# Yujia-Yan/Transkun

Hardware: AMD Instinct MI355X
Metric: semi-CRF logProb+backward steps/sec at T=1024, NBatch=352 (higher is better)
Workload: dtype f32; 1 GPU; NeuralSemiCRFInterval(score, noise).logProb(intervals) fwd+bwd through the public API (Python interval lists packed inside the timed region), T=1024, NBatch=352 per GPU, fp32, exact-hash randn-like scores resident in HBM; T=1024, NBatch=352, impl=0, parallelism=chains sharded, 1 rank(s) seen by the process group, no data-path collective

## Files before the change

### include/semicrf_hip.h

```cpp
#ifndef SEMICRF_HIP_H
#define SEMICRF_HIP_H

#include <stddef.h>
#include <stdint.h>

#ifdef __cplusplus
extern "C" {
#endif

#define SEMICRF_ABI_VERSION 2

#define SEMICRF_OK 0
#define SEMICRF_EINVAL 1
#define SEMICRF_EWORKSPACE 2
#define SEMICRF_ELAUNCH 3
#define SEMICRF_ETIMEOUT 4

#define SEMICRF_OP_LOGZ_FWD 0
#define SEMICRF_OP_LOGZ_BWD 1
#define SEMICRF_OP_VITERBI 2
#define SEMICRF_OP_EVAL_PATH 3
#define SEMICRF_OP_INTERVAL_SCORE 4
#define SEMICRF_OP_SAMPLE 5
#define SEMICRF_OP_VITERBI_NBEST 6
// ... 57 lines not shown
                       float* node, float* begin, float* end, float* single, float* noiseP, float* entropy, void* ws, size_t ws_bytes,
                       semicrf_stream_t stream);

int semicrf_interval_marginals(const float* score, const float* v, const float* q, const float* logZ, int T, int B,
                               const int32_t* pairs, int64_t K, const int32_t* offsets, float* out, semicrf_stream_t stream);

int semicrf_marginal_decode(const float* score, const float* noise, const float* v, const float* q, const float* logZ, int T, int B,
                            const float* tau, int tau_stride, int32_t* pairs, float* probs, int64_t cap, int32_t* offsets,
                            void* ws, size_t ws_bytes, semicrf_stream_t stream);

int semicrf_mbr_select(const int32_t* pairs, const float* weight, const int32_t* offsets, int64_t K, int T, int B, const float* tau,
                       int tau_stride, int32_t* pairs_out, float* probs_out, int64_t cap, int32_t* offsets_out, float* gain,
                       void* ws, size_t ws_bytes, semicrf_stream_t stream);

int semicrf_interval_marginals_tol(const float* score, const float* v, const float* q, const float* logZ, int T, int B,
                                   const int32_t* pairs, int64_t K, const int32_t* offsets, int tol_begin, int tol_end, float* out,
                                   semicrf_stream_t stream);
int semicrf_marginal_decode_tol(const float* score, const float* noise, const float* v, const float* q, const float* logZ, int T, int B,
                                const float* tau, int tau_stride, int tol_begin, int tol_end, int32_t* pairs, float* probs, int64_t cap,
                                int32_t* offsets, void* ws, size_t ws_bytes, semicrf_stream_t stream);

int semicrf_expectation(const float* score, const float* noise, const float* weight, const float* noiseWeight, const float* v,
                        const float* q, int T, int B, float* E, float* H, void* ws, size_t ws_bytes, semicrf_stream_t stream);
int semicrf_covariance(const float* score, const float* noise, const float* weight, const float* noiseWeight, const float* gout, int T,
                       int B, float* C, float* Cn, const void* ws, size_t ws_bytes, semicrf_stream_t stream);

int semicrf_alpha_from(const float* score, const float* noise, const int32_t* start, int T, int B, float* v, float* logZ, void* ws,
                       size_t ws_bytes, semicrf_stream_t stream);

int semicrf_compare_paths(const int32_t* est_pairs, const int32_t* est_offsets, const int32_t* ref_pairs, const int32_t* ref_offsets,
                          int T, int B, int tol_begin, int tol_end, int32_t* stats , semicrf_stream_t stream);

int semicrf_eval_path(const float* score, const float* noise, int T, int B,
                      const int32_t* pairs, int64_t K, const int32_t* offsets, float* out,
                      void* ws, size_t ws_bytes, semicrf_stream_t stream);

int semicrf_eval_path_bwd(const float* gout, int T, int B, const int32_t* pairs, int64_t K,
                          const int32_t* offsets, float* dScore, float* dNoise, semicrf_stream_t stream);

int semicrf_logprob_fwd(const float* score, const float* noise, int T, int B, const int32_t* pairs, int64_t K,
                        const int32_t* offsets, float* logProb, float* logZ, float* v, void* ws, size_t ws_bytes,
                        semicrf_stream_t stream);
int semicrf_logprob_bwd(const float* score, const float* noise, const float* v, const float* logZ, const float* gout,
                        int gout_stride, int T, int B, const int32_t* pairs, int64_t K, const int32_t* offsets,
                        float* dScore, float* dNoise, void* ws, size_t ws_bytes, semicrf_stream_t stream);

#define SEMICRF_GRAD_UPPER_IS_ZERO 1
int semicrf_logz_bwd_f(const float* score, const float* noise, const float* v, const float* logZ,
                       const float* gout, int T, int B, float* dScore, float* dNoise, float* q_out, int flags,
                       void* ws, size_t ws_bytes, semicrf_stream_t stream);
int semicrf_logprob_bwd_f(const float* score, const float* noise, const float* v, const float* logZ, const float* gout,
                          int gout_stride, int T, int B, const int32_t* pairs, int64_t K, const int32_t* offsets,
                          float* dScore, float* dNoise, int flags, void* ws, size_t ws_bytes, semicrf_stream_t stream);

int interval_score_fwd(const float* q, const float* k, const float* diag, int C, int T, int D,
                       int64_t ldq, int64_t ldk, int64_t ldd, float qscale, int length_scaling,
                       int full_square, float* S, float* noise_out, semicrf_stream_t stream);

int interval_score_bwd(const float* dS, const float* q, const float* k, int C, int T, int D, int64_t ldq,
                       int64_t ldk, float qscale, int length_scaling, float* dq, float* dk, float* ddiag,
                       int64_t lddq, int64_t lddk, int64_t lddd, semicrf_stream_t stream);

size_t interval_score_bwd_workspace_bytes(int C, int T, int D);
int interval_score_bwd_ws(const float* dS, const float* q, const float* k, int C, int T, int D, int64_t ldq,
                          int64_t ldk, float qscale, int length_scaling, float* dq, float* dk, float* ddiag,
                          int64_t lddq, int64_t lddk, int64_t lddd, void* ws, size_t ws_bytes, semicrf_stream_t stream);

int interval_score_fwd_p(const float* q, const float* k, const float* diag, int C, int T, int D,
                         int64_t ldq, int64_t ldk, int64_t ldd, float qscale, int length_scaling,
                         int full_square, int group, int pitch, float* S, float* noise_out, semicrf_stream_t stream);
int interval_score_bwd_ws_p(const float* dS, const float* q, const float* k, int C, int T, int D, int64_t ldq,
                            int64_t ldk, float qscale, int length_scaling, int group, int pitch, float* dq, float* dk,
                            float* ddiag, int64_t lddq, int64_t lddk, int64_t lddd, void* ws, size_t ws_bytes,
                            semicrf_stream_t stream);
int interval_score_bwd_fused_ws_p(const float* S, const float* alpha, const float* beta, const float* logZ,
                                  const float* gout, const float* q, const float* k, int C, int T, int D, int64_t ldq,
                                  int64_t ldk, float qscale, int length_scaling, int group, int pitch, float* dq, float* dk,
                                  float* ddiag, int64_t lddq, int64_t lddk, int64_t lddd, void* ws, size_t ws_bytes,
                                  semicrf_stream_t stream);
int interval_score_path_bwd_p(const float* gout, const int32_t* pairs, int64_t K, const int32_t* offsets, const float* q,
                              const float* k, int C, int T, int D, int64_t ldq, int64_t ldk, float qscale, int length_scaling,
                              int group, int pitch, float* dq, float* dk, float* ddiag, int64_t lddq, int64_t lddk,
                              int64_t lddd, semicrf_stream_t stream);

int interval_score_fwd_pc(const float* q, const float* k, const float* diag, const float* rowc, int C, int T, int D,
                          int64_t ldq, int64_t ldk, int64_t ldd, int64_t ldrc, float qscale, int length_scaling,
                          int full_square, int group, int pitch, float* S, float* noise_out, semicrf_stream_t stream);
int interval_score_bwd_ws_pc(const float* dS, const float* q, const float* k, int C, int T, int D, int64_t ldq,
                             int64_t ldk, float qscale, int length_scaling, int group, int pitch, float* dq, float* dk,
                             float* ddiag, float* drowc, int64_t lddq, int64_t lddk, int64_t lddd, int64_t lddrc, void* ws,
                             size_t ws_bytes, semicrf_stream_t stream);
int interval_score_bwd_fused_ws_pc(const float* S, const float* alpha, const float* beta, const float* logZ,
                                   const float* gout, const float* q, const float* k, int C, int T, int D, int64_t ldq,
                                   int64_t ldk, float qscale, int length_scaling, int group, int pitch, float* dq, float* dk,
                                   float* ddiag, float* drowc, int64_t lddq, int64_t lddk, int64_t lddd, int64_t lddrc,
                                   void* ws, size_t ws_bytes, semicrf_stream_t stream);
int interval_score_path_bwd_pc(const float* gout, const int32_t* pairs, int64_t K, const int32_t* offsets, const float* q,
                               const float* k, int C, int T, int D, int64_t ldq, int64_t ldk, float qscale,
                               int length_scaling, int group, int pitch, float* dq, float* dk, float* ddiag, float* drowc,
                               int64_t lddq, int64_t lddk, int64_t lddd, int64_t lddrc, semicrf_stream_t stream);

int scorer_proj_nn(const float* A, int64_t lda, int64_t M, int K, const float* B, int64_t ldb, int N, float* out, int64_t ldout,
                   const float* bias, const float* w2, const float* b2, int zero_cols, int accumulate, semicrf_stream_t stream);
size_t scorer_proj_nn3_workspace_bytes(int K, int N);
int scorer_proj_nn3(const float* A, int64_t lda, int64_t M, int K, const float* B, int64_t ldb, int N, float* out, int64_t ldout,
                    const float* bias, const float* w2, const float* b2, int zero_cols, int accumulate, void* ws, size_t ws_bytes,
// ... 113 lines not shown
```

### transkun_amd/CRF/NeuralSemiCRFInterval.py

```python
from __future__ import annotations

import os
from collections import namedtuple
from typing import List, Optional, Sequence, Tuple

import numpy as np
import torch

from .. import _lib

Intervals = List[List[Tuple[int, int]]]



def _check_inputs(score: torch.Tensor, noiseScore: torch.Tensor):
    assert len(score.shape) == 3
    assert score.shape[0] == score.shape[1]
    assert len(noiseScore.shape) == 2
    T, B = score.shape[0], score.shape[2]
    assert noiseScore.shape[0] == T - 1
    assert noiseScore.shape[1] == B
    _lib.require_device(score, "score")
    _lib.require_device(noiseScore, "noiseScore")
    assert score.device == noiseScore.device
    return T, B


def _prep(t: torch.Tensor) -> torch.Tensor:
    if t.dtype != torch.float32:
        t = t.float()
    return t if t.is_contiguous() else t.contiguous()


_SIDE = {}


def _side_stream(device):
    key = torch.device(device).index if torch.device(device).index is not None else torch.cuda.current_device()
    st = _SIDE.get(key)
    if st is None:
        st = _SIDE[key] = torch.cuda.Stream(device=device)
    return st


def _ready(pairs) -> None:
    ev = getattr(pairs, "_semicrf_ready", None)
    if ev is not None:
        torch.cuda.current_stream(pairs.device).wait_event(ev)
        pairs._semicrf_ready = None


def pack_intervals(intervals: Sequence[Sequence[Tuple[int, int]]], T: int, B: int, device, overlap: bool = False, ordered: bool = True):
    assert len(intervals) == B, f"expected {B} interval lists, got {len(intervals)}"
    mm = _lib.marshal()
    K = int(mm.count(intervals))
    pin = torch.device(device).type == "cuda"
    pairs_h = torch.empty(max(K, 1), 2, dtype=torch.int32, pin_memory=pin)
    offsets_h = torch.empty(B + 1, dtype=torch.int32, pin_memory=pin)
    if K == 0:
        pairs_h.zero_()
    k = mm.pack_into(intervals, pairs_h.data_ptr(), max(K, 1), offsets_h.data_ptr(), T, bool(ordered))
    assert k == K
    if overlap and pin:
        main = torch.cuda.current_stream(device)
        side = _side_stream(device)
        with torch.cuda.stream(side):
            pairs_d = pairs_h.to(device, non_blocking=True)
            offsets_d = offsets_h.to(device, non_blocking=True)
            ev = side.record_event()
        pairs_d.record_stream(main); offsets_d.record_stream(main)
        pairs_d._semicrf_ready = ev
    else:
        pairs_d = pairs_h.to(device, non_blocking=True)
        offsets_d = offsets_h.to(device, non_blocking=True)
    pairs_d._semicrf_K = K
    return pairs_d, offsets_d


def unpack_intervals(pairs_host: torch.Tensor, offsets_host: torch.Tensor, T: int = 1 << 30) -> Intervals:
    import gc
    pairs_host = pairs_host.contiguous()
    offsets_host = offsets_host.contiguous()
    assert pairs_host.dtype == torch.int32 and offsets_host.dtype == torch.int32
    B = offsets_host.numel() - 1
    total = int(offsets_host[-1]) if B >= 0 else 0
    assert pairs_host.numel() >= 2 * total
    if T >= 1 << 30:
        T = int(pairs_host[:total].max()) + 1 if total else 1
    was = gc.isenabled()
    gc.disable()
    try:
        return _lib.marshal().unpack(pairs_host.data_ptr(), offsets_host.data_ptr(), B, T)
    finally:
        if was:
            gc.enable()



_DEBUG_WS = []


def _odd_pad(score) -> bool:
    return score.is_cuda and score.shape[2] == 1 and score.shape[0] >= 2 and _lib.get_impl() == 0


def _pad1(t):
    return torch.nn.functional.pad(t, (0, 1))


def _logz_fwd_raw(score, noise, want_v: bool):
    if _odd_pad(score):
        logz, v = _logz_fwd_raw(_pad1(score), _pad1(noise), want_v)
        return logz[:-1].contiguous(), (v[:, :-1].contiguous() if v is not None else None)
    T, B = score.shape[0], score.shape[2]
    logz = torch.empty(B, dtype=torch.float32, device=score.device)
    v = torch.empty((T, B) if want_v else (0,), dtype=torch.float32, device=score.device)
    ws = _lib.leased_workspace(_lib.OP_LOGZ_FWD, T, B, score.device)
    _lib.ops().logz_fwd(score, noise, logz, v, want_v, ws)
    if os.environ.get("SEMICRF_DEBUG_KEEP_WS"):
        _DEBUG_WS[:] = [ws]
    return logz, (v if want_v else None)


GRAD_UPPER_IS_ZERO = 1


_USE_COUNT = getattr(torch._C, "_storage_Use_Count", None)
_WARNED = set()
# ... 76 lines not shown
            for i in same[:-self.PER_KEY]:
                self.entries[i] = None
            self.entries = [e for e in self.entries if e is not None]
            total = 0
            for i in range(len(self.entries) - 1, -1, -1):
                total += self.entries[i][1].numel() * 4
                if total > max(self.max_bytes, nbytes):
                    del self.entries[:i + 1]
                    break

    def rerecord(self, dscore: torch.Tensor) -> None:
        if dscore is None:
            return
        ptr = dscore.data_ptr()
        with self.lock:
            for e in self.entries:
                if e[1].data_ptr() == ptr:
                    e[2] = e[1]._version

    def clear(self) -> None:
        with self.lock:
            self.entries.clear()


_GRAD_POOL = _GradPool()


def grad_pool_bytes() -> int:
    from .. import scorer as _sc
    return _GRAD_POOL.held_bytes() + (_sc._SCORE_POOL.held_bytes() if _sc._SCORE_POOL is not None else 0)


def grad_pool_clear() -> None:
    _GRAD_POOL.clear()
    from .. import scorer as _sc
    if _sc._SCORE_POOL is not None:
        _sc._SCORE_POOL.clear()


def _logz_bwd_raw(score, noise, v, logz, gout, want_q: bool = False):
    if _odd_pad(score):
        ds, dn, q = _logz_bwd_raw(_pad1(score), _pad1(noise), _pad1(v), _pad1(logz), _pad1(gout), want_q)
        return ds[:, :, :-1].contiguous(), dn[:, :-1].contiguous(), (q[:, :-1].contiguous() if q is not None else None)
    T, B = score.shape[0], score.shape[2]
    dscore, flags, pkey = _GRAD_POOL.take(T, B, score.device)
    dnoise = torch.empty_like(noise)
    q = torch.empty((T, B) if want_q else (0,), dtype=torch.float32, device=score.device)
    ws = _lib.leased_workspace(_lib.OP_LOGZ_BWD, T, B, score.device)
    _lib.ops().logz_bwd(score, noise, v, logz, gout, dscore, dnoise, q, want_q, flags, ws)
    _GRAD_POOL.give(pkey, dscore)
    return dscore, dnoise, (q if want_q else None)


def _logprob_fwd_raw(score, noise, pairs, offsets, want_v: bool):
    K = getattr(pairs, "_semicrf_K", pairs.shape[0])
    if _odd_pad(score):
        logz, v = _logz_fwd_raw(score, noise, want_v)
        return _eval_path_raw(score, noise, pairs, offsets) - logz, logz, v
    T, B = score.shape[0], score.shape[2]
    dev = score.device
    lp = torch.empty(B, dtype=torch.float32, device=dev)
    logz = torch.empty(B, dtype=torch.float32, device=dev)
    v = torch.empty((T, B) if want_v else (0,), dtype=torch.float32, device=dev)
    ws = _lib.leased_workspace(_lib.OP_LOGZ_FWD, T, B, dev)
    _lib.ops().logprob_fwd(score, noise, pairs, int(K), offsets, lp, logz, v, want_v, ws)
    return lp, logz, (v if want_v else None)


def _eval_path_raw(score, noise, pairs, offsets):
    T, B = score.shape[0], score.shape[2]
    out = torch.empty(B, dtype=torch.float32, device=score.device)
    ws = _lib.workspace(_lib.OP_EVAL_PATH, T, B, score.device)
    K = getattr(pairs, "_semicrf_K", pairs.shape[0])
    _lib.ops().eval_path(score, noise, pairs, int(K), offsets, out, ws)
    return out


_EMPTY = {}


def _empty(device):
    e = _EMPTY.get(device)
    if e is None:
        e = _EMPTY[device] = torch.empty(0, dtype=torch.float32, device=device)
    return e


def _eval_path_bwd_raw(gout, T, B, pairs, offsets, dscore, dnoise, K: int, pooled: bool = False):
    e = _empty(gout.device)
    _lib.ops().eval_path_bwd(gout, T, B, pairs, int(K), offsets, dscore if dscore is not None else e, dscore is not None,
                             dnoise if dnoise is not None else e, dnoise is not None)
    if pooled:
        _GRAD_POOL.rerecord(dscore)


def _gout(grad_output: torch.Tensor, B: int) -> torch.Tensor:
    assert grad_output.shape[-1] == B
    g = grad_output.reshape(B)
    if g.dtype != torch.float32:
        g = g.float()
    return g.contiguous()





def _graph_task_id() -> int:
    fn = getattr(torch._C, "_current_graph_task_id", None)
    return int(fn()) if fn is not None else -1


class _HubState:

    def __init__(self):
        self.acc = {}

    def _slot(self, tid):
        a = self.acc.get(tid)
# ... 104 lines not shown
        return dscore.to(ctx.in_dtypes[0]), dnoise.to(ctx.in_dtypes[1]), None


def computeLogZFasterGrad(score, noiseScore):
    return ComputeLogZFasterGrad.apply(score, noiseScore)


class _EvalPath(torch.autograd.Function):
    @staticmethod
    def forward(ctx, score, noiseScore, pairs, offsets, hub=None):
        score_c, noise_c = _prep(score), _prep(noiseScore)
        ctx.save_for_backward(pairs, offsets)
        ctx.shape = (score_c.shape[0], score_c.shape[2])
        ctx.K = getattr(pairs, "_semicrf_K", pairs.shape[0])
        ctx.in_dtypes = (score.dtype, noiseScore.dtype)
        ctx.hub = hub
        return _eval_path_raw(score_c, noise_c, pairs, offsets).to(score.dtype)

    @staticmethod
    def backward(ctx, grad_output):
        pairs, offsets = ctx.saved_tensors
        T, B = ctx.shape
        g = _gout(grad_output, B)
        hub = _hub_of(ctx.hub)
        if hub is not None and ctx.needs_input_grad[0] and ctx.needs_input_grad[1]:
            hub.deposit_path(_graph_task_id(), g, pairs, offsets, ctx.K, T, B)
            return None, None, None, None, None
        dscore = torch.zeros(T, T, B, dtype=torch.float32, device=g.device) if ctx.needs_input_grad[0] else None
        dnoise = torch.zeros(max(T - 1, 0), B, dtype=torch.float32, device=g.device) if ctx.needs_input_grad[1] else None
        _eval_path_bwd_raw(g, T, B, pairs, offsets, dscore, dnoise, ctx.K)
        return (dscore.to(ctx.in_dtypes[0]) if dscore is not None else None,
                dnoise.to(ctx.in_dtypes[1]) if dnoise is not None else None, None, None, None)


def _gout_strided(grad_output: torch.Tensor, B: int):
    assert grad_output.shape[-1] == B
    g = grad_output.reshape(B) if grad_output.dim() != 1 else grad_output
    if g.dtype != torch.float32:
        g = g.float()
    if B > 1 and g.stride(0) == 0:
        return g.as_strided((1,), (1,)), 0
    return g.contiguous(), 1


class _LogProb(torch.autograd.Function):

    @staticmethod
    def forward(ctx, score, noiseScore, pairs, offsets):
        score_c, noise_c = _prep(score), _prep(noiseScore)
        need = ctx.needs_input_grad[0] or ctx.needs_input_grad[1]
        T, B = score_c.shape[0], score_c.shape[2]
        K = getattr(pairs, "_semicrf_K", pairs.shape[0])
        _ready(pairs)
        lp, logz, v = _logprob_fwd_raw(score_c, noise_c, pairs, offsets, need)
        if need:
            ctx.save_for_backward(score_c, noise_c, v, logz, pairs, offsets)
            ctx.K = K
        ctx.in_dtypes = (score.dtype, noiseScore.dtype)
        return lp.to(score.dtype)

    @staticmethod
    def backward(ctx, grad_output):
        score, noise, v, logz, pairs, offsets = ctx.saved_tensors
        T, B = score.shape[0], score.shape[2]
        if _odd_pad(score):
            g = _gout(grad_output, B)
            dscore, dnoise, _ = _logz_bwd_raw(score, noise, v, logz, -g)
            _eval_path_bwd_raw(g, T, B, pairs, offsets, dscore, dnoise, ctx.K)
        else:
            g, gstride = _gout_strided(grad_output, B)
            dscore, flags, pkey = _GRAD_POOL.take(T, B, score.device)
            dnoise = torch.empty_like(noise)
            ws = _lib.leased_workspace(_lib.OP_LOGZ_BWD, T, B, score.device)
            _lib.ops().logprob_bwd(score, noise, v, logz, g, gstride, pairs, int(ctx.K), offsets, dscore, dnoise, flags, ws)
            _GRAD_POOL.give(pkey, dscore)
        return dscore.to(ctx.in_dtypes[0]), dnoise.to(ctx.in_dtypes[1]), None, None



def _viterbi_raw(score_c, noise_c, start, forward: bool):
    if _odd_pad(score_c):
        st = _pad1(start) if start is not None else None
        pairs, offsets = _viterbi_raw(_pad1(score_c), _pad1(noise_c), st, forward)
        return pairs, offsets[:-1]
    T, B = score_c.shape[0], score_c.shape[2]
    dev = score_c.device
    cap = B * 2 * T
    pairs = torch.empty(cap, 2, dtype=torch.int32, device=dev)
    offsets = torch.empty(B + 1, dtype=torch.int32, device=dev)
    ws = _lib.leased_workspace(_lib.OP_VITERBI, T, B, dev)
    has = start is not None
    _lib.ops().viterbi(score_c, noise_c, start if has else offsets, has, bool(forward), pairs, offsets, ws)
    return pairs, offsets


def _start_tensor(forcedStartPos: Optional[Sequence[int]], T: int, B: int, device):
    if forcedStartPos is None:
        return None
    assert len(forcedStartPos) == B
    st = np.asarray(forcedStartPos, dtype=np.int64)
    if (st < 0).any() or (st > T - 1).any():
        raise IndexError(f"forcedStartPos out of range for T={T}")
    return torch.from_numpy(st.astype(np.int32)).to(device, non_blocking=True)


def _decode(score, noiseScore, forcedStartPos: Optional[Sequence[int]], forward: bool, packed: bool = False):
    assert len(score.shape) == 3
    assert score.shape[0] == score.shape[1]
    T, B = _check_inputs(score, noiseScore)
    with torch.no_grad():
        score_c, noise_c = _prep(score.detach()), _prep(noiseScore.detach())
        start = _start_tensor(forcedStartPos, T, B, score_c.device)
        pairs, offsets = _viterbi_raw(score_c, noise_c, start, forward)
        off_h = offsets.cpu()
        total = int(off_h[-1])
        if total < 0:
            _lib.async_error()
            raise RuntimeError("semicrf_viterbi: a bounded hand-off wait timed out on the device (GPU shared with work that "
                               "kept part of the persistent kernel from running?); the decode result is invalid")
        pairs_h = pairs[:total].cpu()
    if packed:
        return pairs_h.numpy(), off_h.numpy()
    return unpack_intervals(pairs_h, off_h, T)



_SAMPLE_CELLS = 1 << 24
# ... 751 lines not shown
```

### transkun_amd/_lib.py

```python
from __future__ import annotations

import collections
import ctypes
import os
from typing import Optional

import torch

_HERE = os.path.dirname(os.path.abspath(__file__))
LIB_PATH = os.environ.get("SEMICRF_LIB") or os.path.join(_HERE, "libsemicrf_hip.so")

OP_LOGZ_FWD, OP_LOGZ_BWD, OP_VITERBI, OP_EVAL_PATH, OP_INTERVAL_SCORE, OP_SAMPLE, OP_VITERBI_NBEST, OP_POSTERIORS = range(8)
OP_MARGINAL_DECODE = 8
OP_EXPECTATION = 9
OP_MBR_SELECT = 10
OP_MARGINAL_DECODE_TOL = 11
OP_ATTRIBUTE_HEADS = 12
OP_ATTRIBUTE_HEADS_BWD = 13
HEADS_ROW_TILE = 64
HEADS_SLICE = 64
HEADS_BWD_ROW_CHUNK = 512
TOL_MAX = 8
LEN_MODES = {"linear": 0, "sqrt": 1, "none": 2}

_vp = ctypes.c_void_p
_i = ctypes.c_int
_i64 = ctypes.c_int64
_sz = ctypes.c_size_t

OPTIM_MAX_GROUPS = 8
SQNORM_MAX_PARTIALS = 256
HISTORY_MAX = 16384


class AdaBeliefGroup(ctypes.Structure):
    _fields_ = [("end", ctypes.c_int64), ("decay", ctypes.c_float), ("b1", ctypes.c_float), ("omb1", ctypes.c_float),
                ("b2", ctypes.c_float), ("omb2", ctypes.c_float), ("eps", ctypes.c_float), ("sqrt_bc2", ctypes.c_float),
                ("step", ctypes.c_float), ("rectified", ctypes.c_int32), ("pad_", ctypes.c_int32)]


class AdaBeliefGroups(ctypes.Structure):
    _fields_ = [("n", ctypes.c_int32), ("pad_", ctypes.c_int32), ("g", AdaBeliefGroup * OPTIM_MAX_GROUPS)]


_SIGS = {
    "semicrf_abi_version": (ctypes.c_int, []),
    "semicrf_last_error": (ctypes.c_char_p, []),
    "semicrf_workspace_bytes": (_sz, [_i, _i, _i]),
    "semicrf_workspace_register": (_i, [_vp, _sz]),
    "semicrf_workspace_unregister": (_i, [_vp]),
    "semicrf_set_impl": (None, [_i]),
    "semicrf_get_impl": (ctypes.c_int, []),
    "semicrf_debug_device_status": (ctypes.c_int, []),
    "semicrf_async_error": (ctypes.c_int, []),
    "semicrf_logz_bwd_f": (_i, [_vp, _vp, _vp, _vp, _vp, _i, _i, _vp, _vp, _vp, _i, _vp, _sz, _vp]),
    "semicrf_logprob_bwd_f": (_i, [_vp, _vp, _vp, _vp, _vp, _i, _i, _i, _vp, _i64, _vp, _vp, _vp, _i, _vp, _sz, _vp]),
    "semicrf_debug_wg_ticket": (_i, [_i, _i, _i]),
    "semicrf_debug_score_variant": (None, [_i]),
    "semicrf_logz_fwd": (_i, [_vp, _vp, _i, _i, _vp, _vp, _vp, _sz, _vp]),
    "semicrf_logz_bwd": (_i, [_vp, _vp, _vp, _vp, _vp, _i, _i, _vp, _vp, _vp, _vp, _sz, _vp]),
    "semicrf_viterbi": (_i, [_vp, _vp, _i, _i, _vp, _i, _vp, _i64, _vp, _vp, _sz, _vp]),
    "semicrf_sample": (_i, [_vp, _vp, _vp, _i, _i, _i64, _i, ctypes.c_uint64, _vp, _vp, _i64, _vp, _vp, _sz, _vp]),
    "semicrf_viterbi_nbest": (_i, [_vp, _vp, _i, _i, _i, _vp, _i, _vp, _i64, _vp, _vp, _vp, _vp, _sz, _vp]),
    "semicrf_posteriors": (_i, [_vp, _vp, _vp, _vp, _vp, _i, _i, _vp, _vp, _vp, _vp, _vp, _vp, _vp, _sz, _vp]),
    "semicrf_interval_marginals": (_i, [_vp, _vp, _vp, _vp, _i, _i, _vp, _i64, _vp, _vp, _vp]),
    "semicrf_marginal_decode": (_i, [_vp, _vp, _vp, _vp, _vp, _i, _i, _vp, _i, _vp, _vp, _i64, _vp, _vp, _sz, _vp]),
    "semicrf_interval_marginals_tol": (_i, [_vp, _vp, _vp, _vp, _i, _i, _vp, _i64, _vp, _i, _i, _vp, _vp]),
    "semicrf_marginal_decode_tol": (_i, [_vp, _vp, _vp, _vp, _vp, _i, _i, _vp, _i, _i, _i, _vp, _vp, _i64, _vp, _vp, _sz, _vp]),
    "semicrf_mbr_select": (_i, [_vp, _vp, _vp, _i64, _i, _i, _vp, _i, _vp, _vp, _i64, _vp, _vp, _vp, _sz, _vp]),
    "semicrf_compare_paths": (_i, [_vp, _vp, _vp, _vp, _i, _i, _i, _i, _vp, _vp]),
    "semicrf_expectation": (_i, [_vp, _vp, _vp, _vp, _vp, _vp, _i, _i, _vp, _vp, _vp, _sz, _vp]),
    "semicrf_alpha_from": (_i, [_vp, _vp, _vp, _i, _i, _vp, _vp, _vp, _sz, _vp]),
    "semicrf_covariance": (_i, [_vp, _vp, _vp, _vp, _vp, _i, _i, _vp, _vp, _vp, _sz, _vp]),
    "semicrf_eval_path": (_i, [_vp, _vp, _i, _i, _vp, _i64, _vp, _vp, _vp, _sz, _vp]),
    "semicrf_eval_path_bwd": (_i, [_vp, _i, _i, _vp, _i64, _vp, _vp, _vp, _vp]),
    "semicrf_logprob_fwd": (_i, [_vp, _vp, _i, _i, _vp, _i64, _vp, _vp, _vp, _vp, _vp, _sz, _vp]),
    "semicrf_logprob_bwd": (_i, [_vp, _vp, _vp, _vp, _vp, _i, _i, _i, _vp, _i64, _vp, _vp, _vp, _vp, _sz, _vp]),
    "interval_score_fwd": (_i, [_vp, _vp, _vp, _i, _i, _i, _i64, _i64, _i64, ctypes.c_float, _i, _i, _vp, _vp, _vp]),
    "interval_score_fwd_p": (_i, [_vp, _vp, _vp, _i, _i, _i, _i64, _i64, _i64, ctypes.c_float, _i, _i, _i, _i, _vp, _vp, _vp]),
    "interval_score_bwd_ws_p": (_i, [_vp, _vp, _vp, _i, _i, _i, _i64, _i64, ctypes.c_float, _i, _i, _i, _vp, _vp, _vp, _i64, _i64, _i64, _vp, ctypes.c_size_t, _vp]),
    "interval_score_bwd_fused_ws_p": (_i, [_vp, _vp, _vp, _vp, _vp, _vp, _vp, _i, _i, _i, _i64, _i64, ctypes.c_float, _i, _i, _i, _vp, _vp, _vp, _i64, _i64, _i64, _vp, ctypes.c_size_t, _vp]),
    "interval_score_path_bwd_p": (_i, [_vp, _vp, _i64, _vp, _vp, _vp, _i, _i, _i, _i64, _i64, ctypes.c_float, _i, _i, _i, _vp, _vp, _vp, _i64, _i64, _i64, _vp]),
    "interval_score_fwd_pc": (_i, [_vp, _vp, _vp, _vp, _i, _i, _i, _i64, _i64, _i64, _i64, ctypes.c_float, _i, _i, _i, _i, _vp, _vp, _vp]),
    "interval_score_bwd_ws_pc": (_i, [_vp, _vp, _vp, _i, _i, _i, _i64, _i64, ctypes.c_float, _i, _i, _i, _vp, _vp, _vp, _vp, _i64, _i64, _i64, _i64, _vp, ctypes.c_size_t, _vp]),
    "interval_score_bwd_fused_ws_pc": (_i, [_vp, _vp, _vp, _vp, _vp, _vp, _vp, _i, _i, _i, _i64, _i64, ctypes.c_float, _i, _i, _i, _vp, _vp, _vp, _vp, _i64, _i64, _i64, _i64, _vp, ctypes.c_size_t, _vp]),
    "interval_score_path_bwd_pc": (_i, [_vp, _vp, _i64, _vp, _vp, _vp, _i, _i, _i, _i64, _i64, ctypes.c_float, _i, _i, _i, _vp, _vp, _vp, _vp, _i64, _i64, _i64, _i64, _vp]),
    "semicrf_beta": (_i, [_vp, _vp, _i, _i, _vp, _vp, _sz, _vp]),
    "scorer_proj_nn": (_i, [_vp, _i64, _i64, _i, _vp, _i64, _i, _vp, _i64, _vp, _vp, _vp, _i, _i, _vp]),
    "scorer_proj_nn3": (_i, [_vp, _i64, _i64, _i, _vp, _i64, _i, _vp, _i64, _vp, _vp, _vp, _i, _i, _vp, ctypes.c_size_t, _vp]),
    "scorer_proj_nn3_workspace_bytes": (ctypes.c_size_t, [_i, _i]),
    "scorer_proj_tn_workspace_bytes": (_sz, [_i64, _i, _i]),
    "scorer_merge_weights_fwd": (_i, [_vp, _vp, _i, _i, _i, _vp, _vp, _vp, _vp]),
    "scorer_stage_linear": (_i, [_vp, _vp, _i, _i, _i, _vp, _vp, _vp, _vp, _vp]),
    "scorer_merge_weights_bwd_workspace_bytes": (_sz, [_i]),
    "scorer_merge_weights_bwd": (_i, [_vp, _vp, _vp, _vp, _i, _i, _i, _vp, _vp, _vp, _sz, _vp]),
    "scorer_proj_tn": (_i, [_vp, _i64, _i64, _i, _i, _i, _vp, _i64, _i, _vp, _i64, _vp, _vp, _sz, _vp]),
    "interval_score_bwd_fused": (_i, [_vp, _vp, _vp, _vp, _vp, _vp, _vp, _i, _i, _i, _i64, _i64, ctypes.c_float, _i, _vp, _vp, _vp, _i64, _i64, _i64, _vp]),
    "interval_score_bwd": (_i, [_vp, _vp, _vp, _i, _i, _i, _i64, _i64, ctypes.c_float, _i, _vp, _vp, _vp, _i64, _i64, _i64, _vp]),
    "interval_score_bwd_fused_ws": (_i, [_vp, _vp, _vp, _vp, _vp, _vp, _vp, _i, _i, _i, _i64, _i64, ctypes.c_float, _i, _vp, _vp, _vp, _i64, _i64, _i64, _vp, ctypes.c_size_t, _vp]),
    "interval_score_path_bwd": (_i, [_vp, _vp, _i64, _vp, _vp, _vp, _i, _i, _i, _i64, _i64, ctypes.c_float, _i, _vp, _vp, _vp, _i64, _i64, _i64, _vp]),
    "interval_features_gather": (_i, [_vp, _i, _i, _i, _i64, _vp, _i64, _vp, _i, _vp, _vp, _vp, _vp]),
    "interval_features_gather_bwd": (_i, [_vp, _vp, _i, _i, _i, _i64, _vp, _i64, _vp, _vp, _i64, _vp]),
    "semicrf_attribute_loss_fwd": (_i, [_vp, _vp, _vp, _vp, _vp, _i64, _vp, _i, _vp, _vp, _vp, _vp]),
    "semicrf_attribute_loss_bwd": (_i, [_vp, _i, _vp, _vp, _vp, _vp, _vp, _i64, _vp, _i, _vp, _vp, _vp]),
    "semicrf_attribute_decode": (_i, [_vp, _vp, _i64, _i, _vp, _vp, _vp, _vp, _vp]),
    "semicrf_attribute_heads_workspace_bytes": (_sz, [_i64, _i, _i, _i, _i]),
    "semicrf_attribute_heads": (_i, [_vp, _i, _i, _i, _i64, _vp, _i64, _vp, _i, _vp, _vp, _vp, _vp, _i, _i, _i, _i, _vp, _vp, _vp, _vp, _vp, _sz, _vp]),
    "semicrf_attribute_heads_train_fwd_workspace_bytes": (_sz, [_i64, _i, _i, _i, _i]),
    "semicrf_attribute_heads_train_fwd": (_i, [_vp, _i, _i, _i, _i64, _vp, _i64, _vp, _i, _vp, _vp, _vp, _vp, _i, _i, _i, _i, ctypes.c_uint64,
# ... 167 lines not shown
```

### transkun_amd/csrc/api.hip

```cpp
#include <stdarg.h>
#include <string.h>
#include <stdlib.h>
#include <atomic>
#include <mutex>
#include <unordered_map>
#include "common.h"

namespace semicrf {

static thread_local char g_err[512] = "";
static std::atomic<int> g_impl{0};

void set_error(const char* fmt, ...)
{
    va_list ap;
    va_start(ap, fmt);
    vsnprintf(g_err, sizeof(g_err), fmt, ap);
    va_end(ap);
}

void launch_rowseq_sweep(int mode, int dir, const float* score, const float* noise, int T, int B, float* u,
                         int* code, float* out_last, hipStream_t stream);
void launch_marginals(const float* score, const float* noise, const float* v, const float* q,
                      const float* logZ, const float* gout, int T, int B, float* dScore, float* dNoise,
// ... 83 lines not shown
void launch_merge_weights_bwd(const float* W, const float* bias, const float* dWm, const float* dbm, int D, int size, float* dW, float* dbias,
                              float* ws, hipStream_t stream);
size_t merge_weights_bwd_workspace_bytes(int size);
void launch_stage_linear(const float* W, const float* bias, int D, int size, int rows_pad, float* BT, float* Wqd, float* w2, float* b2,
                         hipStream_t stream);
int launch_proj_tn(const float* A, long long lda, long long M, int R, int extra_col0, int total_rows, const float* X, long long ldx, int N,
                   float* dW, long long lddw, float* db, void* ws, size_t ws_bytes, hipStream_t stream);
size_t persist_workspace_bytes(int T, int B);
size_t sample_workspace_bytes(int T, int nB);
size_t posterior_workspace_bytes(int T, int B);
size_t expectation_workspace_bytes(int T, int B);
void launch_alpha_from(const float* score, const float* noise, const int* start, int T, int B, float* v, float* logZ, hipStream_t stream);
void launch_expectation(const float* score, const float* noise, const float* weight, const float* nweight, const float* v, const float* q,
                        int T, int B, float* E, float* H, void* ws, hipStream_t stream);
void launch_covariance(const float* score, const float* noise, const float* weight, const float* nweight, const float* gout, int T, int B,
                       float* C, float* Cn, const void* ws, hipStream_t stream);
void launch_posteriors(const float* score, const float* noise, const float* v, const float* q, const float* logZ, int T, int B,
                       float* node, float* begin, float* end, float* single, float* noiseP, float* entropy, void* ws,
                       hipStream_t stream);
void launch_interval_marginals(const float* score, const float* v, const float* q, const float* logZ, int T, int B, const int* pairs,
                               int K, const int* offsets, float* out, hipStream_t stream);
size_t marginal_decode_workspace_bytes(int T, int B);
void launch_marginal_decode(const float* score, const float* v, const float* q, const float* logZ, int T, int B, const float* tau,
                            int tau_stride, int* pairs, float* probs, long long cap, int* offsets, void* ws, hipStream_t stream);
size_t marginal_decode_tol_workspace_bytes(int T, int B);
void launch_interval_marginals_tol(const float* score, const float* v, const float* q, const float* logZ, int T, int B, const int* pairs,
                                   int K, const int* offsets, int db, int de, float* out, hipStream_t stream);
void launch_marginal_decode_tol(const float* score, const float* v, const float* q, const float* logZ, int T, int B, const float* tau,
                                int tau_stride, int db, int de, int* pairs, float* probs, long long cap, int* offsets, void* ws,
                                hipStream_t stream);
void launch_compare_paths(const int* est_pairs, const int* est_offsets, const int* ref_pairs, const int* ref_offsets, int T, int B,
                          int tb, int te, int* stats, hipStream_t stream);
size_t mbr_select_workspace_bytes(int T, int B);
void launch_mbr_select(const int* pairs, const float* weight, const int* offsets, long long K, int T, int B, const float* tau,
                       int tau_stride, int* pairs_out, float* probs_out, long long cap, int* offsets_out, float* gain, void* ws,
                       hipStream_t stream);
size_t nbest_workspace_bytes(int T, int nB);
void launch_viterbi_nbest(const float* score, const float* noise, int T, int B, int k, const int* start, int forward, int* pairs,
                          long long cap, int* offsets, float* scores, int* npaths, void* ws, hipStream_t stream);
void launch_sample(const float* score, const float* noise, const float* v, int T, int B, long long k0, int nSample,
                   unsigned long long key, const int* end, int* pairs, long long cap, int* offsets, void* ws, hipStream_t stream);
bool persist_supported(int T, int B);
int launch_persist_sweep(int mode, int dir, const float* score, const float* noise, int T, int B, float* u_out,
                         float* last_out, int* code, void* ws, hipStream_t stream, int lease, unsigned lease_tag);
int persist_set_host_abort_word(unsigned* devptr);
int persist_wg_ticket(int nSpine, int grid, int b);
void set_score_variant(int v);

int read_and_clear_device_status();

int launch_persist_logz_bwd(const float* score, const float* noise, const float* v, const float* logZ,
                            const float* gout, int T, int B, float* dScore, float* dNoise, float* q_out, void* ws,
                            hipStream_t stream, int lease, unsigned lease_tag, int gstride = 1, float gscale = 1.0f, int keep_upper = 0,
                            float noise_add = 0.0f);
int launch_persist_logprob_fwd(const float* score, const float* noise, int T, int B, float* u_out, float* logZ, const int* pairs,
                               int K, const int* offsets, float* logProb, void* ws, hipStream_t stream, int lease, unsigned lease_tag);

static bool use_persist(int T, int B) { return g_impl.load() == 0 && persist_supported(T, B); }

struct Carver {
    char* p;
    size_t left;
    bool ok = true;
    Carver(void* ws, size_t n) : p((char*)ws), left(n) {}
    template <typename U>
    U* take(size_t count)
    {
        size_t bytes = align_up(count * sizeof(U));
        if (bytes > left) { ok = false; return nullptr; }
        U* r = (U*)p;
        p += bytes;
        left -= bytes;
        return r;
    }
};

static size_t tb(int T, int B) { return align_up((size_t)T * (size_t)B * 4); }

struct Lease { size_t bytes; int op, T, B; bool clean; unsigned count; };
static std::mutex g_lease_mu;
static std::unordered_map<void*, Lease> g_leases;
static unsigned* g_abort_word = nullptr;
static std::atomic<bool> g_abort_on_device[64];

static int ensure_abort_word(hipStream_t stream)
{
    int dev = 0;
    if (hipGetDevice(&dev) != hipSuccess || dev < 0 || dev >= 64) dev = 0;
    if (g_abort_on_device[dev].load()) return 0;
    hipStreamCaptureStatus cs = hipStreamCaptureStatusNone;
    if (hipStreamIsCapturing(stream, &cs) == hipSuccess && cs != hipStreamCaptureStatusNone) return 0;
    {
        std::lock_guard<std::mutex> lk(g_lease_mu);
        if (!g_abort_word) {
            void* p = nullptr;
            if (hipHostMalloc(&p, 64, hipHostMallocMapped | hipHostMallocPortable) != hipSuccess) return 1;
            memset(p, 0, 64);
            g_abort_word = (unsigned*)p;
        }
    }
    void* dp = nullptr;
    if (hipHostGetDevicePointer(&dp, g_abort_word, 0) != hipSuccess || persist_set_host_abort_word((unsigned*)dp)) return 1;
    g_abort_on_device[dev].store(true);
    return 0;
}

static unsigned take_async_error()
{
    if (!g_abort_word) return 0u;
// ... 60 lines not shown
int semicrf_debug_wg_ticket(int n_spine, int grid, int block) { return persist_wg_ticket(n_spine, grid, block); }
void semicrf_debug_score_variant(int variant) { set_score_variant(variant); }

int semicrf_workspace_register(void* ws, size_t ws_bytes)
{
    SEMICRF_CHECK_ARG(ws != nullptr && ws_bytes > 0, "workspace is NULL or empty");
    if (ensure_abort_word(nullptr)) { set_error("could not hand the abort word to the device"); return SEMICRF_ELAUNCH; }
    std::lock_guard<std::mutex> lk(g_lease_mu);
    g_leases[ws] = Lease{ws_bytes, -1, 0, 0, false, 0u};
    return SEMICRF_OK;
}

int semicrf_workspace_unregister(void* ws)
{
    std::lock_guard<std::mutex> lk(g_lease_mu);
    g_leases.erase(ws);
    return SEMICRF_OK;
}

size_t semicrf_workspace_bytes(int op, int T, int B)
{
    if (T <= 0 || B <= 0) return 0;
    switch (op) {
        case SEMICRF_OP_LOGZ_FWD: return tb(T, B) + persist_workspace_bytes(T, B) + 4096;
        case SEMICRF_OP_LOGZ_BWD: return tb(T, B) + persist_workspace_bytes(T, B) + 4096;
        case SEMICRF_OP_VITERBI:
            return tb(T, B) * 2 + align_up((size_t)B * 2 * T * 2 * 4) + align_up((size_t)B * 4) +
                   persist_workspace_bytes(T, B) + 4096;
        case SEMICRF_OP_EVAL_PATH: return 4096;
        case SEMICRF_OP_INTERVAL_SCORE: return 4096;
        case SEMICRF_OP_SAMPLE: return sample_workspace_bytes(T, B);
        case SEMICRF_OP_POSTERIORS: return posterior_workspace_bytes(T, B);
        case SEMICRF_OP_VITERBI_NBEST: return nbest_workspace_bytes(T, B);
        case SEMICRF_OP_MARGINAL_DECODE: return marginal_decode_workspace_bytes(T, B);
        case SEMICRF_OP_EXPECTATION: return expectation_workspace_bytes(T, B);
        case SEMICRF_OP_MBR_SELECT: return mbr_select_workspace_bytes(T, B);
        case SEMICRF_OP_MARGINAL_DECODE_TOL: return marginal_decode_tol_workspace_bytes(T, B);
        case SEMICRF_OP_ATTRIBUTE_HEADS: return attr_heads_workspace_bytes(T, 64 * ((B + 63) / 64 + 1), 1, 128, 1);
        case SEMICRF_OP_ATTRIBUTE_HEADS_BWD: return attr_heads_bwd_workspace_bytes(T, (B + 2) / 3, B, 1, 128, 128);
        default: return 0;
    }
}

static int check_common(const float* score, const float* noise, int T, int B)
{
    SEMICRF_CHECK_ARG(T >= 1 && B >= 1, "T=%d, B=%d must be >= 1", T, B);
    SEMICRF_CHECK_ARG((long long)T * T * B < (1ll << 40), "T*T*B too large");
    SEMICRF_CHECK_ARG(T < (1 << 29), "T too large");
    SEMICRF_CHECK_ARG(score != nullptr, "score is NULL");
    SEMICRF_CHECK_ARG(noise != nullptr || T == 1, "noise is NULL");
    return SEMICRF_OK;
}

struct PathFold { const int32_t* pairs; int64_t K; const int32_t* offsets; float* logProb; int folded; };

static int logz_fwd_impl(const float* score, const float* noise, int T, int B, float* logZ, float* v, void* ws,
                         size_t ws_bytes, semicrf_stream_t stream, PathFold* pf)
{
    if (int rc = check_common(score, noise, T, B)) return rc;
    SEMICRF_CHECK_ARG(logZ != nullptr, "logZ is NULL");
    if (int rc = sweep_prologue("semicrf_logz_fwd", (hipStream_t)stream)) return rc;
    Carver cv(ws, ws_bytes);
    const bool fast = use_persist(T, B);
    void* pws = fast ? cv.take<char>(persist_workspace_bytes(T, B)) : nullptr;
    float* vv = v ? v : cv.take<float>((size_t)T * B);
    if (!cv.ok || !ws) { set_error("workspace too small for logz_fwd"); return SEMICRF_EWORKSPACE; }
    hipStream_t st = (hipStream_t)stream;
    if (fast) {
        unsigned ltag = 0;
        const int lease = lease_acquire(ws, SEMICRF_OP_LOGZ_FWD, T, B, &ltag, st);
        const int rc = pf ? launch_persist_logprob_fwd(score, noise, T, B, vv, logZ, pf->pairs, (int)pf->K, pf->offsets, pf->logProb, pws, st, lease, ltag)
                          : launch_persist_sweep(0, 0, score, noise, T, B, vv, logZ, nullptr, pws, st, lease, ltag);
        if (rc) {
            lease_failed(ws);
            set_error("persistent sweep could not be enqueued (too many chain chunks for this device)"); return SEMICRF_ELAUNCH;
        }
        if (pf) pf->folded = 1;
    } else {
        lease_failed(ws);
        launch_rowseq_sweep(0, 0, score, noise, T, B, vv, nullptr, logZ, st);
    }
    SEMICRF_CHECK_LAUNCH("semicrf_logz_fwd");
    return SEMICRF_OK;
}

int semicrf_logz_fwd(const float* score, const float* noise, int T, int B, float* logZ, float* v, void* ws,
                     size_t ws_bytes, semicrf_stream_t stream)
{
    return logz_fwd_impl(score, noise, T, B, logZ, v, ws, ws_bytes, stream, nullptr);
}

static int logz_bwd_impl(const float* score, const float* noise, const float* v, const float* logZ,
                         const float* gout, int gstride, float gscale, int T, int B, float* dScore, float* dNoise, float* q_out,
                         int flags, void* ws, size_t ws_bytes, semicrf_stream_t stream, float noise_add = 0.0f, int* noise_folded = nullptr)
{
    if (int rc = check_common(score, noise, T, B)) return rc;
    SEMICRF_CHECK_ARG((flags & ~SEMICRF_GRAD_UPPER_IS_ZERO) == 0, "unknown flags %d", flags);
    if (int rc = sweep_prologue("semicrf_logz_bwd", (hipStream_t)stream)) return rc;
    const int keep_upper = (flags & SEMICRF_GRAD_UPPER_IS_ZERO) ? 1 : 0;
    SEMICRF_CHECK_ARG(v && logZ && gout && dScore, "v/logZ/gout/dScore must be non-NULL");
    SEMICRF_CHECK_ARG(dNoise != nullptr || T == 1, "dNoise is NULL");
    SEMICRF_CHECK_ARG(gstride == 0 || gstride == 1, "gout stride must be 0 (one value for all chains) or 1");
    Carver cv(ws, ws_bytes);
    const bool fast = use_persist(T, B);
    void* pws = fast ? cv.take<char>(persist_workspace_bytes(T, B)) : nullptr;
    float* q = q_out ? q_out : cv.take<float>((size_t)T * B);
    if (!cv.ok || !ws) { set_error("workspace too small for logz_bwd"); return SEMICRF_EWORKSPACE; }
    hipStream_t st = (hipStream_t)stream;
    if (fast) {
        unsigned ltag = 0;
        const int lease = lease_acquire(ws, SEMICRF_OP_LOGZ_BWD, T, B, &ltag, st);
        if (launch_persist_logz_bwd(score, noise, v, logZ, gout, T, B, dScore, dNoise, q, pws, st, lease, ltag, gstride, gscale, keep_upper, noise_add)) {
            lease_failed(ws);
            set_error("persistent sweep could not be enqueued (too many chain chunks for this device)"); return SEMICRF_ELAUNCH;
        }
        if (noise_folded) *noise_folded = 1;
    } else {
        lease_failed(ws);
        launch_rowseq_sweep(0, 1, score, noise, T, B, q, nullptr, nullptr, st);
        launch_marginals(score, noise, v, q, logZ, gout, T, B, dScore, dNoise, st, gstride, gscale);
    }
    return SEMICRF_OK;
}

int semicrf_logz_bwd_f(const float* score, const float* noise, const float* v, const float* logZ,
                       const float* gout, int T, int B, float* dScore, float* dNoise, float* q_out, int flags, void* ws,
                       size_t ws_bytes, semicrf_stream_t stream)
{
    if (int rc = logz_bwd_impl(score, noise, v, logZ, gout, 1, 1.0f, T, B, dScore, dNoise, q_out, flags, ws, ws_bytes, stream)) return rc;
    SEMICRF_CHECK_LAUNCH("semicrf_logz_bwd");
    return SEMICRF_OK;
}

int semicrf_logz_bwd(const float* score, const float* noise, const float* v, const float* logZ,
                     const float* gout, int T, int B, float* dScore, float* dNoise, float* q_out, void* ws,
                     size_t ws_bytes, semicrf_stream_t stream)
{
    return semicrf_logz_bwd_f(score, noise, v, logZ, gout, T, B, dScore, dNoise, q_out, 0, ws, ws_bytes, stream);
}

int semicrf_logprob_fwd(const float* score, const float* noise, int T, int B, const int32_t* pairs, int64_t K,
                        const int32_t* offsets, float* logProb, float* logZ, float* v, void* ws, size_t ws_bytes,
                        semicrf_stream_t stream)
{
    SEMICRF_CHECK_ARG(offsets && logProb && logZ, "offsets/logProb/logZ must be non-NULL");
    SEMICRF_CHECK_ARG(K >= 0 && K < (1ll << 31) && (K == 0 || pairs), "bad interval count");
    PathFold pf{pairs, K, offsets, logProb, 0};
    if (int rc = logz_fwd_impl(score, noise, T, B, logZ, v, ws, ws_bytes, stream, &pf)) return rc;
    if (!pf.folded) launch_eval_path(score, noise, T, B, (int)K, pairs, offsets, logProb, (hipStream_t)stream, logZ);
    SEMICRF_CHECK_LAUNCH("semicrf_logprob_fwd");
    return SEMICRF_OK;
}

int semicrf_logprob_bwd(const float* score, const float* noise, const float* v, const float* logZ, const float* gout,
                        int gout_stride, int T, int B, const int32_t* pairs, int64_t K, const int32_t* offsets, float* dScore,
                        float* dNoise, void* ws, size_t ws_bytes, semicrf_stream_t stream)
{
    return semicrf_logprob_bwd_f(score, noise, v, logZ, gout, gout_stride, T, B, pairs, K, offsets, dScore, dNoise, 0, ws, ws_bytes, stream);
}

int semicrf_logprob_bwd_f(const float* score, const float* noise, const float* v, const float* logZ, const float* gout,
                          int gout_stride, int T, int B, const int32_t* pairs, int64_t K, const int32_t* offsets, float* dScore,
                          float* dNoise, int flags, void* ws, size_t ws_bytes, semicrf_stream_t stream)
{
    SEMICRF_CHECK_ARG(offsets, "offsets must be non-NULL");
    SEMICRF_CHECK_ARG(K >= 0 && K < (1ll << 31) && (K == 0 || pairs), "bad interval count");
    int noise_folded = 0;
    if (int rc = logz_bwd_impl(score, noise, v, logZ, gout, gout_stride, -1.0f, T, B, dScore, dNoise, nullptr, flags, ws, ws_bytes, stream,
                               1.0f, &noise_folded)) return rc;
    launch_eval_path_bwd(gout, T, B, (int)K, pairs, offsets, dScore, dNoise, (hipStream_t)stream, gout_stride, 1.0f, noise_folded);
    SEMICRF_CHECK_LAUNCH("semicrf_logprob_bwd");
    return SEMICRF_OK;
}

int semicrf_beta(const float* score, const float* noise, int T, int B, float* beta, void* ws, size_t ws_bytes,
                 semicrf_stream_t stream)
{
    if (int rc = check_common(score, noise, T, B)) return rc;
    SEMICRF_CHECK_ARG(beta, "beta must be non-NULL");
    if (int rc = sweep_prologue("semicrf_beta", (hipStream_t)stream)) return rc;
    Carver cv(ws, ws_bytes);
    const bool fast = use_persist(T, B);
    void* pws = fast ? cv.take<char>(persist_workspace_bytes(T, B)) : nullptr;
    if (!cv.ok || (fast && !ws)) { set_error("workspace too small for beta"); return SEMICRF_EWORKSPACE; }
    hipStream_t st = (hipStream_t)stream;
    if (fast) {
        unsigned ltag = 0;
        const int lease = lease_acquire(ws, SEMICRF_OP_LOGZ_FWD + 100, T, B, &ltag, st);
        if (launch_persist_sweep(0, 1, score, noise, T, B, beta, nullptr, nullptr, pws, st, lease, ltag)) {
            lease_failed(ws);
            set_error("persistent sweep could not be enqueued (too many chain chunks for this device)"); return SEMICRF_ELAUNCH;
        }
    } else {
        lease_failed(ws);
        launch_rowseq_sweep(0, 1, score, noise, T, B, beta, nullptr, nullptr, st);
    }
    SEMICRF_CHECK_LAUNCH("semicrf_beta");
    return SEMICRF_OK;
}

int semicrf_viterbi(const float* score, const float* noise, int T, int B, const int32_t* start, int forward,
                    int32_t* pairs, int64_t cap, int32_t* offsets, void* ws, size_t ws_bytes,
                    semicrf_stream_t stream)
{
    if (int rc = check_common(score, noise, T, B)) return rc;
    SEMICRF_CHECK_ARG(pairs && offsets && cap >= 0, "pairs/offsets must be non-NULL");
    SEMICRF_CHECK_ARG((long long)B * 2 * T < (1ll << 31), "B*2T exceeds int32 offsets");
    if (int rc = sweep_prologue("semicrf_viterbi", (hipStream_t)stream)) return rc;
    Carver cv(ws, ws_bytes);
    float* u = cv.take<float>((size_t)T * B);
    int* code = cv.take<int>((size_t)T * B);
    int* region = cv.take<int>((size_t)B * 2 * T * 2);
    int* counts = cv.take<int>((size_t)B);
    const bool fast = use_persist(T, B);
    void* pws = fast ? cv.take<char>(persist_workspace_bytes(T, B)) : nullptr;
    if (!cv.ok || !ws) { set_error("workspace too small for viterbi"); return SEMICRF_EWORKSPACE; }
    hipStream_t st = (hipStream_t)stream;
    if (fast) {
        unsigned ltag = 0;
        const int lease = lease_acquire(ws, SEMICRF_OP_VITERBI, T, B, &ltag, st);
        if (launch_persist_sweep(1, forward ? 0 : 1, score, noise, T, B, nullptr, nullptr, code, pws, st, lease, ltag)) {
            lease_failed(ws);
            set_error("persistent sweep could not be enqueued (too many chain chunks for this device)"); return SEMICRF_ELAUNCH;
// ... 830 lines not shown
```

### transkun_amd/csrc/pathscore.h

```cpp
#pragma once
#include "common.h"

namespace semicrf {

__device__ __forceinline__ double path_score_wave(const float* __restrict__ score, const float* __restrict__ noise, int T, int B, int K,
                                                  const int* __restrict__ pairs, const int* __restrict__ offsets, int c)
{
    const int lane = threadIdx.x & 63;
    double acc = 0.0;
    for (int t = lane; t < T - 1; t += 64) acc += (double)noise[(size_t)t * B + c];
    const int k0 = offsets[c], k1 = offsets[c + 1];
    for (int k = k0 + lane; k < k1 && k < K; k += 64) {
        const int b = pairs[2 * k], e = pairs[2 * k + 1];
        double covered = 0.0;
        for (int t = b; t < e; ++t) covered += (double)noise[(size_t)t * B + c];
        acc += (double)score[((size_t)e * T + b) * B + c] - covered;
    }
#pragma unroll
    for (int d = 32; d >= 1; d >>= 1) acc += __shfl_xor(acc, d, 64);
    return acc;
}

}
```

### transkun_amd/csrc/persist.hip

```cpp
#include <atomic>
#include <stdlib.h>
#include "common.h"
#include "pathscore.h"

#ifndef SEMICRF_PANEL_PROBES
#define SEMICRF_PANEL_PROBES 0
#endif

#ifndef SEMICRF_PROBE_TASKS
#define SEMICRF_PROBE_TASKS 0
#endif
#ifndef SEMICRF_PROBE_HIST
#define SEMICRF_PROBE_HIST 0
#endif

#ifndef SEMICRF_CT_DBG
#define SEMICRF_CT_DBG -1
#endif

namespace semicrf {

constexpr int PB = 16;
#ifndef SEMICRF_RING
#define SEMICRF_RING 4
// ... 57 lines not shown
constexpr size_t CTRL_WORDS = 256;
constexpr int CTRL_EXIT = 64;
constexpr int CTRL_COPYQ = 192;
constexpr int CTRL_PATHQ = 160;
constexpr int CTRL_GEN = 96;

typedef unsigned long long u64;
typedef unsigned v4u __attribute__((ext_vector_type(4)));
typedef unsigned v4u_a4 __attribute__((ext_vector_type(4), aligned(4)));
template <int V>
struct IC { static constexpr int value = V; };

#define DBGF(P) (SEMICRF_CT_DBG >= 0 ? (unsigned)SEMICRF_CT_DBG : (P).dbg)
struct SweepParams {
    const float* score;
    const float* noise;
    int T, B, K;
    int c0, c1;
    int nSpine, nPanelGroups;
    int nTasks;
    int taskBase;
    int panelWaves;
    int hybridPanelWaves;
    int hybridStart;
    int zeroWaves;
    unsigned tag;
    int selfclean;
    unsigned expect_gen;
    unsigned dbg;
    unsigned* ctrl;
    u64* ts;
    unsigned* ug;
    unsigned* ug_other;
    int gradLazyShort;
    int bandWaves;
    u64* farg;
    float* u_out;
    float* last_out;
    int* code;
    const float* vfwd;
    const float* logZ;
    const float* gout;
    int gstride;
    float gscale;
    float* dScore;
    float* dNoise;
    const int* pathPairs;
    const int* pathOffsets;
    int pathK;
    int pathSpine;
    float* pathOut;
    u64* pathg;
    float noiseAdd;
    float* band;
    unsigned* bandFlags;
    int bandSpines;
    int bandGroups;
    int bandK0;
    int copyWaves;
    int cellNT;
    int gradNT;
    int nfarw;
};

__device__ __forceinline__ float fexp2(float x) { return __builtin_amdgcn_exp2f(x); }
__device__ __forceinline__ float flog2(float x) { return __builtin_amdgcn_logf(x); }

__device__ __forceinline__ u64 make_granule(unsigned tag, float v)
{
    return ((u64)tag << 32) | (u64)__float_as_uint(v);
}
__device__ __forceinline__ u64 make_granule_key(unsigned tag, float v, int key)
{
    return ((u64)(((tag & 0xffffu) << 16) | ((unsigned)key & 0xffffu)) << 32) | (u64)__float_as_uint(v);
}
__device__ __forceinline__ void store_granule(u64* p, u64 g)
{
    __hip_atomic_store(p, g, __ATOMIC_RELAXED, __HIP_MEMORY_SCOPE_AGENT);
}
__device__ __forceinline__ u64 load_granule(const u64* p)
{
    return __hip_atomic_load(p, __ATOMIC_RELAXED, __HIP_MEMORY_SCOPE_AGENT);
}

template <int DIR>
__device__ __forceinline__ int frame_of(int p, int T) { return DIR == 0 ? p : T - 1 - p; }

template <int DIR>
__device__ __forceinline__ size_t cell_index(int pi, int pj, int T)
{
    return DIR == 0 ? (size_t)pi * T + pj : (size_t)(T - 1 - pj) * T + (T - 1 - pi);
}
template <int DIR>
__device__ __forceinline__ int gap_of(int p, int T) { return DIR == 0 ? p - 1 : T - 1 - p; }

__device__ __forceinline__ void acc_push1(float& M, float& S, float t)
{
    const float d = t - M;
    const float e = fexp2(-fabsf(d));
    S = d > 0.0f ? fmaf(S, e, 1.0f) : S + e;
    M = fmaxf(M, t);
}
__device__ __forceinline__ void acc_merge(float& M, float& S, float M2, float S2)
{
    if (S2 == 0.0f) return;
    if (M2 > M) {
        S = S * fexp2(M - M2) + S2;
        M = M2;
    } else {
        S += S2 * fexp2(M2 - M);
    }
}
template <int DIR>
__device__ __forceinline__ void max_push_seq(float& best, int& key, float t, int k)
{
    const bool take = DIR == 0 ? t > best : t >= best;
    best = take ? t : best;
    key = take ? k : key;
}
__device__ __forceinline__ float softplus2(float x)
{
    const float x2 = x * LOG2E;
    return x > 20.0f ? x2 : flog2(1.0f + fexp2(x2));
}

__device__ unsigned g_dev_status = 0;
__shared__ int s_abort;

__device__ unsigned* g_host_abort = nullptr;

__device__ __forceinline__ void set_error(unsigned* ctrl, unsigned code)
{
    __hip_atomic_store(ctrl + 1, code, __ATOMIC_RELAXED, __HIP_MEMORY_SCOPE_AGENT);
    __hip_atomic_store(&g_dev_status, code, __ATOMIC_RELAXED, __HIP_MEMORY_SCOPE_AGENT);
    unsigned* const h = g_host_abort;
    if (h) __hip_atomic_store(h, code, __ATOMIC_RELAXED, __HIP_MEMORY_SCOPE_SYSTEM);
}

__device__ __forceinline__ bool spin_abort(unsigned* ctrl, int& spins, int limit, unsigned code)
{
    ++spins;
    if (spins > limit) { set_error(ctrl, code); s_abort = 1; return true; }
    if ((spins & 255) == 0 &&
        __hip_atomic_load(ctrl + 1, __ATOMIC_RELAXED, __HIP_MEMORY_SCOPE_AGENT) != CTRL_INIT) { s_abort = 1; return true; }
    return false;
}

#ifndef SEMICRF_NLOADER
#define SEMICRF_NLOADER 1
#endif
constexpr int NLOADER = SEMICRF_NLOADER;
#ifndef SEMICRF_NRBUF
#define SEMICRF_NRBUF 4
#endif
constexpr int NRBUF = SEMICRF_NRBUF;
constexpr int TILE_BYTES = PB * PB * RS * 4;
constexpr int NCONST = 3;
constexpr int LDS_TILES = 0;
constexpr int LDS_CONST = LDS_TILES + NRBUF * RING * TILE_BYTES;
constexpr int LDS_FAR = LDS_CONST + NRBUF * NCONST * 256;
constexpr int NFAR = 8;
constexpr int NPOS = 128;
static_assert(NFAR >= RING && NPOS >= RING * PB, "ring geometry");
constexpr int LDS_RING = LDS_FAR + NFAR * 64 * 16;
#ifndef SEMICRF_STAGGER
#define SEMICRF_STAGGER 32
#endif
#ifndef SEMICRF_GRAD_LAZY
#define SEMICRF_GRAD_LAZY 127
#endif
#ifndef SEMICRF_GRAD_HSTART
#define SEMICRF_GRAD_HSTART 12
#endif
#ifndef SEMICRF_LOADER_PACE
#define SEMICRF_LOADER_PACE 0
#endif
#ifndef SEMICRF_LOADER_AUX
#define SEMICRF_LOADER_AUX 0
#endif
#ifndef SEMICRF_SPH
#define SEMICRF_SPH 1
#endif
#ifndef SEMICRF_FAR_EARLY
#define SEMICRF_FAR_EARLY 0
#endif
#ifndef SEMICRF_FAR_PRIO
#define SEMICRF_FAR_PRIO 0
#endif
#ifndef SEMICRF_NFARW
#define SEMICRF_NFARW 2
#endif
constexpr int NFARW = SEMICRF_NFARW;
constexpr int NNSLOT = 8;
constexpr int NEAR_SLOT_BYTES = NNEAR * TILE_BYTES + 256;
constexpr int LDS_NEAR = LDS_RING + NPOS * RS * 8;
constexpr int LDS_CTL = LDS_NEAR + (NNEAR > 0 ? NNSLOT * NEAR_SLOT_BYTES : 0);
static_assert(NPOS >= (FAR0 + 1) * PB && NNSLOT >= FAR0 + 1 && NRBUF + RING + NNSLOT + NFARW <= 64 && NNSLOT % NFARW == 0, "near geometry");
constexpr int LDS_DUMMY = LDS_CTL + 256;
constexpr int LDS_SPINE_BYTES = LDS_DUMMY + (64 * 2 + PB * 8) * 4;

typedef __attribute__((address_space(3))) void lds_void_t;
typedef __attribute__((address_space(1))) const void gbl_void_t;

struct SpineBlk { float v[PB]; };

__device__ __forceinline__ int spine_row(int lane) { return lane & 15; }
__device__ __forceinline__ int spine_chain(int lane) { return lane >> 4; }

template <int N>
__device__ __forceinline__ void wait_vmcnt() { asm volatile("s_waitcnt vmcnt(%0)" ::"n"(N)); }

__device__ __forceinline__ int lds_flag_load(const int* p) { return __hip_atomic_load(p, __ATOMIC_RELAXED, __HIP_MEMORY_SCOPE_WORKGROUP); }
__device__ __forceinline__ void lds_flag_store(int* p, int v) { __hip_atomic_store(p, v, __ATOMIC_RELAXED, __HIP_MEMORY_SCOPE_WORKGROUP); }
__device__ __forceinline__ unsigned lds_addr(const void* p)
{
    return (unsigned)(uintptr_t)(__attribute__((address_space(3))) const void*)p;
}
__device__ __forceinline__ int lds_flag_load_asm(const int* p)
{
    int v;
    asm volatile("ds_read_b32 %0, %1\n\ts_waitcnt lgkmcnt(0)" : "=v"(v) : "v"(lds_addr(p)) : "memory");
    return v;
}
__device__ __forceinline__ void lds_flag_store_asm(int* p, int v)
{
    asm volatile("ds_write_b32 %0, %1" ::"v"(lds_addr(p)), "v"(v) : "memory");
}
__device__ __forceinline__ u64 lds_load64(const void* p)
{
    return __hip_atomic_load((const u64*)p, __ATOMIC_RELAXED, __HIP_MEMORY_SCOPE_WORKGROUP);
}
__device__ __forceinline__ void lds_store64(void* p, float value, int seq)
{
    __hip_atomic_store((u64*)p, ((u64)(unsigned)seq << 32) | (u64)__float_as_uint(value), __ATOMIC_RELAXED, __HIP_MEMORY_SCOPE_WORKGROUP);
}
typedef float f32x4_t __attribute__((ext_vector_type(4)));
__device__ __forceinline__ void lds_store128(void* p, float4 v)
{
    const f32x4_t w = {v.x, v.y, v.z, v.w};
    asm volatile("ds_write_b128 %0, %1" ::"v"(lds_addr(p)), "v"(w) : "memory");
}
__device__ __forceinline__ float4 lds_load128(const void* p)
{
    f32x4_t w;
    asm volatile("ds_read_b128 %0, %1\n\ts_waitcnt lgkmcnt(0)" : "=v"(w) : "v"(lds_addr(p)) : "memory");
    return make_float4(w.x, w.y, w.z, w.w);
}

template <int DIR, bool GRAD>
__device__ __forceinline__ void loader_role(const SweepParams& P, int sg, char* lds, int lid)
{
    const int T = P.T, B = P.B, K = P.K;
    unsigned* const ctrl = P.ctrl;
    const size_t Bs = (size_t)B;
    const float* const score = P.score;
    const float* const noise = P.noise;
    const float* const vfwd = P.vfwd;
    const int lane = threadIdx.x & 63;
    const int cbase = P.c0 + sg * GS;
    const size_t last4 = (size_t)T * T * Bs - 4;
    const int tu = lane >> 4, tr = lane & 15;
    const int cr = spine_row(lane), cch = spine_chain(lane);
    const int cc = cbase + cch < P.c1 ? cbase + cch : cbase;
    int* const ready = (int*)(lds + LDS_CTL);
    int* const cons = ready + NRBUF;
    int* const nready = cons + RING;
    const int* const fcons = nready + NNSLOT;
    constexpr int NL = RING * 4 + 2 + (GRAD ? 1 : 0) + NNEAR * 4 + ((GRAD && NNEAR > 0) ? 1 : 0);
    constexpr int LDEPTH = 3 * NL <= 63 ? 3 : 2;
    static_assert(2 * NL <= 63, "loader pipeline");

    const bool useband = SEMICRF_BANDX && P.band != nullptr;
    const float* const bandp = useband ? P.band + (size_t)(cbase / GS) * NBT * (TILE_BYTES / 4) + lane * 4 : nullptr;
    const size_t band_kr = (size_t)P.bandSpines * NBT * (TILE_BYTES / 4);
    typedef unsigned v16u __attribute__((ext_vector_type(16)));
    const int bKpad = K + 2;
    const unsigned* const bflags = useband ? P.bandFlags + (size_t)(cbase / GP) * bKpad * 8 : nullptr;
    const unsigned btag = P.tag;
    int ready_upto = -1;
    auto band_ready = [&](int kr) -> bool {
        const uintptr_t fa = (uintptr_t)(bflags + (size_t)kr * 8);
        const u64 fp = (u64)(unsigned)__builtin_amdgcn_readfirstlane((int)(unsigned)fa) |
                       ((u64)(unsigned)__builtin_amdgcn_readfirstlane((int)(unsigned)(fa >> 32)) << 32);
        v16u f;
        asm volatile("s_load_dwordx16 %0, %1, 0x0 glc\n\ts_waitcnt lgkmcnt(0)" : "=&s"(f) : "s"(fp) : "memory");
        const unsigned want0 = ((btag & 0xffffu) << 16) | (unsigned)kr, want1 = want0 + 1u;
        bool ok0 = true, ok1 = true;
#pragma unroll
        for (int i = 0; i < NBT; ++i) { ok0 = ok0 && f[i] == want0; ok1 = ok1 && f[8 + i] == want1; }
        if (ok0) ready_upto = ok1 ? kr + 1 : kr;
        return ok0;
    };
    auto issue = [&](int kr) {
        const int slot = kr % NRBUF;
        const int prow_t = kr * PB + tr < T ? kr * PB + tr : T - 1;
        const bool fromband = useband && kr >= P.bandK0;
        if (fromband) {
            const float* const bk = bandp + (size_t)kr * band_kr;
#pragma unroll
            for (int i = 0; i < RING; ++i)
#pragma unroll
                for (int q = 0; q < 4; ++q)
                    __builtin_amdgcn_global_load_lds((gbl_void_t*)(bk + i * (TILE_BYTES / 4) + q * 256),
                                                     (lds_void_t*)(lds + LDS_TILES + (slot * RING + i) * TILE_BYTES + q * 1024), 16, 0, SEMICRF_BAND_LOAD_AUX);
        } else
#pragma unroll
        for (int i = 0; i < RING; ++i) {
            const int kc = kr - (RING - 1) + i > 0 ? kr - (RING - 1) + i : 0;
#pragma unroll
            for (int q = 0; q < 4; ++q) {
                int pj = kc * PB + 4 * q + tu;
                pj = pj < prow_t ? pj : (prow_t > 0 ? prow_t - 1 : 0);
                size_t off = cell_index<DIR>(prow_t, pj, T) * Bs + cbase;
                off = off < last4 ? off : last4;
                __builtin_amdgcn_global_load_lds((gbl_void_t*)(score + off),
                                                 (lds_void_t*)(lds + LDS_TILES + (slot * RING + i) * TILE_BYTES + q * 1024), 16, 0, SEMICRF_LOADER_AUX);
                if (SEMICRF_LOADER_PACE > 0) __builtin_amdgcn_s_sleep(SEMICRF_LOADER_PACE);
            }
        }
        const int prow_c = kr * PB + cr < T ? kr * PB + cr : T - 1;
        const int frow = frame_of<DIR>(prow_c, T);
        char* cb = lds + LDS_CONST + slot * NCONST * 256;
        __builtin_amdgcn_global_load_lds((gbl_void_t*)(score + ((size_t)frow * T + frow) * Bs + cc), (lds_void_t*)cb, 4, 0, 0);
        __builtin_amdgcn_global_load_lds((gbl_void_t*)(noise + (size_t)gap_of<DIR>(prow_c >= 1 ? prow_c : 1, T) * Bs + cc),
                                         (lds_void_t*)(cb + 256), 4, 0, 0);
        if (GRAD)
            __builtin_amdgcn_global_load_lds((gbl_void_t*)(vfwd + (size_t)frow * Bs + cc), (lds_void_t*)(cb + 512), 4, 0, 0);
        if (NNEAR > 0) {
            char* const nb = lds + LDS_NEAR + (kr % NNSLOT) * NEAR_SLOT_BYTES;
            if (fromband) {
                const float* const bk = bandp + (size_t)kr * band_kr;
#pragma unroll
                for (int n = 0; n < NNEAR; ++n)
#pragma unroll
                    for (int q = 0; q < 4; ++q)
                        __builtin_amdgcn_global_load_lds((gbl_void_t*)(bk + (RING + n) * (TILE_BYTES / 4) + q * 256),
                                                         (lds_void_t*)(nb + n * TILE_BYTES + q * 1024), 16, 0, 16);
            } else
#pragma unroll
            for (int n = 0; n < NNEAR; ++n) {
                const int kc = kr - RING - n > 0 ? kr - RING - n : 0;
#pragma unroll
                for (int q = 0; q < 4; ++q) {
                    int pj = kc * PB + 4 * q + tu;
                    pj = pj < prow_t ? pj : (prow_t > 0 ? prow_t - 1 : 0);
                    size_t off = cell_index<DIR>(prow_t, pj, T) * Bs + cbase;
                    off = off < last4 ? off : last4;
                    __builtin_amdgcn_global_load_lds((gbl_void_t*)(score + off), (lds_void_t*)(nb + n * TILE_BYTES + q * 1024), 16, 0, SEMICRF_LOADER_AUX);
                }
            }
            if (GRAD)
                __builtin_amdgcn_global_load_lds((gbl_void_t*)(vfwd + (size_t)frow * Bs + cc), (lds_void_t*)(nb + NNEAR * TILE_BYTES), 4, 0, 0);
        }
    };
    auto publish = [&](int kr) {
        if (lane == 0) {
            lds_flag_store_asm(ready + kr % NRBUF, kr + 1);
            if (NNEAR > 0) lds_flag_store_asm(nready + kr % NNSLOT, kr + 1);
        }
    };

    int prev2 = -1, prev1 = -1;
    for (int kr = lid; kr < K; kr += NLOADER) {
        if (kr >= NRBUF) {
            const int w = (kr - NRBUF) % RING;
            int spins = 0;
            while (lds_flag_load_asm(cons + w) < kr - NRBUF + 1) {
                __builtin_amdgcn_s_sleep(2);
                if (spin_abort(ctrl, spins, SPIN_LIMIT_LDS, 6)) return;
            }
        }
        if (NNEAR > 0 && kr >= NNSLOT && !(SEMICRF_PANEL_PROBES && (DBGF(P) & 9u))) {
            int spins = 0;
            while (lds_flag_load_asm(fcons + (kr - NNSLOT - RING + NFARW * NNSLOT) % NFARW) < kr - NNSLOT + 1 && kr - NNSLOT >= RING) {
                __builtin_amdgcn_s_sleep(2);
                if (spin_abort(ctrl, spins, SPIN_LIMIT_LDS, 6)) return;
            }
        }
        if (useband && kr >= P.bandK0 && kr > ready_upto) {
            int spins = 0;
// ... 165 lines not shown
                    }
            }
        }
        if (fprobe && k < 64) P.ts[896 + k] = __builtin_amdgcn_s_memrealtime();
        const float val = MODE == 0 ? aM + flog2(aS) : aM;
        lds_store128(far + (k % NFAR) * 64 + lane, make_float4(val, __int_as_float(aK), __int_as_float(k + 1), 0.0f));
        if (SEMICRF_PANEL_PROBES && (DBGF(P) & 16u) && cbase_is_first && lane == 0) P.ts[128 + k] = __builtin_amdgcn_s_memrealtime();
    }
}


template <int J>
__device__ __forceinline__ float row_bcast(float x)
{
    return __int_as_float(__builtin_amdgcn_update_dpp(0, __float_as_int(x), 0x150 + J, 0xf, 0xf, false));
}
template <int J, int N, typename F>
__device__ __forceinline__ void static_for(F&& f)
{
    if constexpr (J < N) { f(IC<J>{}); static_for<J + 1, N>(f); }
}

template <int MODE, int DIR, bool GRAD, bool RINGBAND>
__device__ __forceinline__ void spine_role(const SweepParams& P, int sg, int ring_pos, char* lds)
{
    const int T = P.T, B = P.B, K = P.K;
    const unsigned dbg = DBGF(P);
    unsigned* const ctrl = P.ctrl;
    u64* const ts = P.ts;
    unsigned* const ug = P.ug;
    float* const u_out = P.u_out;
    float* const last_out = P.last_out;
    int* const code = P.code;
    float* const dScore = P.dScore;
    float* const dNoise = P.dNoise;
    const u64* const pathg = P.pathg;
    float* const pathOut = P.pathOut;
    const unsigned ptag = P.tag;
    const int rw = __builtin_amdgcn_readfirstlane(ring_pos);
    const int lane = threadIdx.x & 63;
    const int r = spine_row(lane), ch = spine_chain(lane);
    const int c = P.c0 + sg * GS + ch;
    const bool cvalid = c < P.c1;
    const int cc = cvalid ? c : P.c0;
    const size_t Bs = (size_t)B;
    const bool trace = (dbg & 16u) && sg == 0 && lane == 0;
    float* const ring = (float*)(lds + LDS_RING);
    const float* rd_base = ring + ch * 2;
    const int* const ready = (const int*)(lds + LDS_CTL);
    int* const cons = (int*)(lds + LDS_CTL) + NRBUF;
    const float4* const far = (const float4*)(lds + LDS_FAR);
    float gz = 0.f, lzc = 0.f;
    float nadd = 0.f;
    if (GRAD && cvalid) {
        const float go = P.gout[(size_t)c * P.gstride];
        gz = go * P.gscale; lzc = P.logZ[c]; nadd = P.noiseAdd * go;
    }
    constexpr int ringBand = GRAD && RINGBAND ? 1 : 0;
    __builtin_amdgcn_s_setprio(1);

    for (int k = rw; k < K; k += RING) {
        u64* ev = ts + T + (size_t)k * 8;
        if (trace) ev[0] = __builtin_readcyclecounter();
        const int prow = k * PB + r;
        const bool rvalid = cvalid && prow < T;
        const int prow_c = prow < T ? prow : T - 1;
        const int frow = frame_of<DIR>(prow_c, T);
        const int own0 = k * PB;
        const int slot = k % NRBUF;

        {
            int spins = 0;
            while (lds_flag_load(ready + slot) != k + 1) {
                __builtin_amdgcn_s_sleep(1);
                if (spin_abort(ctrl, spins, SPIN_LIMIT_LDS, 7)) break;
            }
        }
        const char* tb = lds + LDS_TILES + slot * RING * TILE_BYTES + (r * RS + ch) * 4;
        auto read_tile = [&](int i) -> SpineBlk {
            SpineBlk o;
#pragma unroll
            for (int u = 0; u < PB; ++u) o.v[u] = *(const float*)(tb + i * TILE_BYTES + u * (PB * RS * 4));
            return o;
        };
        SpineBlk X[RING];
#pragma unroll
        for (int i = 0; i < RING; ++i) X[i] = read_tile(i);
        const float* cst = (const float*)(lds + LDS_CONST + slot * NCONST * 256) + lane;
        const float dcell = cst[0], nzl = cst[64], vfl = cst[128];
        const float s1own = *(const float*)(lds + LDS_TILES + (slot * RING + RING - 1) * TILE_BYTES +
                                            ((((r > 0 ? r - 1 : 0) * PB) + r) * RS + ch) * 4);
        const float s1 = r == 0 ? X[RING - 2].v[PB - 1] : s1own;
        if (lane == 0) lds_flag_store(cons + rw, k + 1);

        const unsigned bvoff = DIR == 0 ? (unsigned)(((size_t)(prow_c - own0) * T * Bs + cc) * 4)
                                        : (unsigned)(((size_t)(T - 1 - prow_c) * Bs + cc) * 4);
        auto col_off = [&](int j) -> size_t {
            return DIR == 0 ? ((size_t)own0 * T + (size_t)j) * Bs : (size_t)(T - 1 - j) * T * Bs;
        };
        auto grad_store = [&](int j, float v) {
#ifdef SEMICRF_NO_BAND_GSTORE
            (void)j; asm volatile("" ::"v"(v)); return;
#endif
            const auto rs = __builtin_amdgcn_make_buffer_rsrc((void*)(dScore + col_off(j)), 0, 0x7fffffff, 0x00020000);
            __builtin_amdgcn_raw_buffer_store_b32(__float_as_uint(v), rs, bvoff, 0, 0);
        };

        float sp = 0.f;
        float nz = 0.f;
        float wl = 0.f;
        float draw = 0.f;
        if (rvalid) {
            draw = dcell * LOG2E;
            sp = MODE == 0 ? softplus2(dcell) : dcell;
            if (prow >= 1) {
                nz = nzl;
                if (MODE == 0) {
                    const float a0 = s1 * LOG2E, b0 = nz * LOG2E;
                    wl = fmaxf(a0, b0) + flog2(1.0f + fexp2(-fabsf(a0 - b0)));
                }
            }
        }
        const float arow = (GRAD && rvalid) ? (vfl - lzc) * LOG2E : 0.f;
        float d[PB - 1];
        if (MODE == 0) {
            static_for<0, PB - 1>([&](auto jc) {
                constexpr int j = decltype(jc)::value;
                const float cj = r > j + 1 ? X[RING - 1].v[j] * LOG2E : (r == j + 1 ? wl : SEMICRF_NEG_INF);
                d[j] = (rvalid ? cj : SEMICRF_NEG_INF) + row_bcast<j>(sp);
            });
        }
        if (trace) ev[1] = __builtin_readcyclecounter();

        float aM = SEMICRF_NEG_INF, aS = 0.f;
        int aK = 0x7fffffff;

        auto ring_get4 = [&](int j, float (&uo)[4]) {
            const float* e = rd_base + (j % NPOS) * 8;
            u64 w0, w1, w2, w3;
            auto fetch = [&]() { w0 = lds_load64(e); w1 = lds_load64(e + 2 * RS); w2 = lds_load64(e + 4 * RS); w3 = lds_load64(e + 6 * RS); };
            auto ok = [&]() {
                return (int)(w0 >> 32) == j + 1 && (int)(w1 >> 32) == j + 2 && (int)(w2 >> 32) == j + 3 && (int)(w3 >> 32) == j + 4;
            };
            fetch();
            if (!__all(ok())) {
                int spins = 0;
                while (true) {
                    __builtin_amdgcn_s_sleep(1);
                    fetch();
                    if (__all(ok())) break;
                    if (spin_abort(ctrl, spins, SPIN_LIMIT_LDS, 2)) break;
                }
            }
            uo[0] = __uint_as_float((unsigned)w0); uo[1] = __uint_as_float((unsigned)w1);
            uo[2] = __uint_as_float((unsigned)w2); uo[3] = __uint_as_float((unsigned)w3);
        };

        auto shadow = [&](const SpineBlk& X, int b, bool last) {
            if (trace && b >= k - 3) ev[3 + (b - (k - 3))] = __builtin_readcyclecounter();
            if (MODE == 0) {
                float t[PB];
#pragma unroll
                for (int u4 = 0; u4 < PB; u4 += 4) {
                    float uq[4];
                    ring_get4(b * PB + u4, uq);
#pragma unroll
                    for (int q = 0; q < 4; ++q) {
                        const int u = u4 + q;
                        const int j = b * PB + u;
                        float p = fmaf(X.v[u], LOG2E, uq[q]);
                        if (GRAD && ringBand && rvalid && j < prow) grad_store(j, gz * fexp2(p + arow));
                        if (last && u == PB - 1 && r == 0) {
                            if (GRAD && rvalid)
                                dNoise[(size_t)gap_of<DIR>(prow, T) * Bs + c] = gz * fexp2(uq[q] + nz * LOG2E + arow) + nadd;
                            p = uq[q] + wl;
                        }
                        t[u] = p;
                    }
                }
                float mx = aM;
#pragma unroll
                for (int u = 0; u < PB; u += 2) mx = fmaxf(mx, fmaxf(t[u], t[u + 1]));
                float sum = aS * fexp2(aM - mx);
#pragma unroll
                for (int u = 0; u < PB; ++u) sum += fexp2(t[u] - mx);
                aM = mx; aS = sum;
            } else {
#pragma unroll
                for (int u4 = 0; u4 < PB; u4 += 4) {
                    float uq[4];
                    ring_get4(b * PB + u4, uq);
#pragma unroll
                    for (int q = 0; q < 4; ++q) {
                        const int u = u4 + q;
                        const int j = b * PB + u;
                        const float uv = uq[q];
                        const int key = frame_of<DIR>(j, T);
                        if (last && u == PB - 1 && r == 0) max_push_sel(aM, aK, uv + nz, -1);
                        max_push_sel(aM, aK, uv + X.v[u], key);
                    }
                }
            }
        };

#pragma unroll
        for (int i = 0; i < RING - 1; ++i)
            if (k - (RING - 1) + i >= 0) shadow(X[i], k - (RING - 1) + i, i == RING - 2);

        __builtin_amdgcn_s_setprio(3);
        if (trace) ev[6] = __builtin_readcyclecounter();
        if (k >= RING && !(dbg & 1u)) {
            const float4* fe = far + (k % NFAR) * 64 + lane;
            float4 f = lds_load128(fe);
            if (!__all(__float_as_int(f.z) == k + 1)) {
                int spins = 0;
                while (true) {
                    __builtin_amdgcn_s_sleep(1);
                    f = lds_load128(fe);
                    if (__all(__float_as_int(f.z) == k + 1)) break;
                    if (spin_abort(ctrl, spins, SPIN_LIMIT_LDS, 8)) break;
                }
            }
            if (rvalid) {
                if (MODE == 0) acc_push1(aM, aS, f.x);
                else max_push_sel(aM, aK, f.x, __float_as_int(f.y));
            }
        }

        if (SEMICRF_PANEL_PROBES && trace) { ts[64 + k] = __builtin_amdgcn_s_memrealtime(); ev[2] = __builtin_readcyclecounter(); }
        int mykey = -1;
        float mine = 0.f;
        if (MODE == 0) {
            float mx = aM, S = aS;
            if (prow == 0 || !rvalid) { mx = 0.0f; S = 1.0f; }
            float e = mx;
            static_for<0, PB - 1>([&](auto jc) {
                constexpr int j = decltype(jc)::value;
                e = fmaxf(e, row_bcast<j>(e) + d[j]);
            });
            float acc = S * fexp2(mx - e);
            static_for<0, PB - 1>([&](auto jc) {
                constexpr int j = decltype(jc)::value;
                acc = fmaf(row_bcast<j>(acc), fexp2((row_bcast<j>(e) - e) + d[j]), acc);
            });
            mine = e + flog2(acc) + sp;
            lds_store64(ring + ch * 2 + ((own0 + r) % NPOS) * 8, mine, own0 + r + 1);
            __builtin_amdgcn_s_setprio(1);
            if (GRAD) {
                if (ringBand) {
                    static_for<0, PB - 1>([&](auto jc) {
                        constexpr int j = decltype(jc)::value;
                        const float uj = row_bcast<j>(mine);
                        if (rvalid && r > j) grad_store(own0 + j, gz * fexp2(fmaf(X[RING - 1].v[j], LOG2E, uj) + arow));
                    });
                }
                const float um1 = __int_as_float(__builtin_amdgcn_update_dpp(0, __float_as_int(mine), 0x111, 0xf, 0xf, false));
                if (rvalid && r >= 1) dNoise[(size_t)gap_of<DIR>(prow, T) * Bs + c] = gz * fexp2(um1 + nz * LOG2E + arow) + nadd;
            }
        } else {
            float best = aM;
            int key = aK;
            if (prow == 0 || !rvalid) { best = 0.0f; key = -1; }
            const float spr = sp > 0.0f ? sp : 0.0f;
            static_for<0, PB - 1>([&](auto jc) {
                constexpr int j = decltype(jc)::value;
                const float uj = row_bcast<j>(best + spr);
                const int keyj = frame_of<DIR>(own0 + j < T ? own0 + j : T - 1, T);
                const float ts = uj + nz;
                const bool c1 = (r == j + 1) & ((ts > best) | ((ts == best) & (key > -1)));
                best = c1 ? ts : best;
                key = c1 ? -1 : key;
                const float tc = uj + (r > j ? X[RING - 1].v[j] : SEMICRF_NEG_INF);
                const bool c2 = (tc > best) | ((tc == best) & (keyj < key));
                best = c2 ? tc : best;
                key = c2 ? keyj : key;
            });
            mine = best + spr;
            mykey = key;
            lds_store64(ring + ch * 2 + ((own0 + r) % NPOS) * 8, mine, own0 + r + 1);
            __builtin_amdgcn_s_setprio(1);
        }
        if (trace) ev[7] = __builtin_readcyclecounter();

        if (rvalid) {
            if (k == K - 1 && lds_flag_load(&s_abort) != 0) mine = __uint_as_float(0x7fc00000u);
            if (k < K - FAR0 || (GRAD && ringBand == 0)) {
                unsigned ub = __float_as_uint(mine);
                if (ub == U_EMPTY) ub = 0x7fc00000u;
                __hip_atomic_store(ug + (size_t)prow * Bs + c, ub, __ATOMIC_RELAXED, __HIP_MEMORY_SCOPE_AGENT);
            }
            const float sc = MODE == 0 ? LN2 : 1.0f;
            if (u_out) u_out[(size_t)frow * Bs + c] = mine * sc;
            if (last_out && prow == T - 1) last_out[c] = mine * sc;
            if (MODE == 0 && DIR == 0 && !GRAD && pathg && prow == T - 1) {
                u64 gr;
                int spins = 0;
                bool ok = true;
                while (true) {
                    gr = load_granule(pathg + c);
                    if ((unsigned)(gr >> 32) == ptag) break;
                    __builtin_amdgcn_s_sleep(8);
                    if (spin_abort(ctrl, spins, SPIN_LIMIT, 15)) { ok = false; break; }
                }
                pathOut[c] = ok ? __uint_as_float((unsigned)gr) - mine * sc : __uint_as_float(0x7fc00000u);
            }
            if (GRAD)
                dScore[((size_t)frow * T + frow) * Bs + c] = gz * fexp2(arow + mine + draw - 2.0f * sp);
            if (MODE == 1) code[(size_t)c * T + frow] = (mykey + 1) | (sp > 0.0f ? 0x40000000 : 0);
        }
        if (SEMICRF_PANEL_PROBES && trace) ts[k] = __builtin_amdgcn_s_memrealtime();
    }
}

#ifndef SEMICRF_GRAD_AUX
#define SEMICRF_GRAD_AUX 2
#endif
constexpr int GRAD_AUX = SEMICRF_GRAD_AUX;
#ifndef SEMICRF_CELL_AUX
#define SEMICRF_CELL_AUX 2
#endif
constexpr int CELL_AUX = SEMICRF_CELL_AUX;
#ifndef SEMICRF_PNS
#define SEMICRF_PNS 3
#endif
constexpr int PNS = SEMICRF_PNS;
constexpr int PSTAGE_BYTES = 10240;
#ifndef SEMICRF_PW_MAX
#define SEMICRF_PW_MAX 5
#endif
constexpr int PW_MAX = SEMICRF_PW_MAX;
constexpr int LDS_PANEL_BYTES = PW_MAX * PNS * PSTAGE_BYTES;
constexpr int SPH = SEMICRF_SPH;
constexpr int HWAVES = SPH == 1 ? RING + NLOADER + 1 : RING + NLOADER + NFARW;
constexpr int LDS_HALF = (LDS_SPINE_BYTES + 1023) / 1024 * 1024;
constexpr int LDS_HYBRID_PANEL = SPH * LDS_HALF;
constexpr int HPW_MAX = (160 * 1024 - 512 - LDS_HYBRID_PANEL) / (PNS * PSTAGE_BYTES) < NT / 64 - SPH * HWAVES
                            ? (160 * 1024 - 512 - LDS_HYBRID_PANEL) / (PNS * PSTAGE_BYTES) : NT / 64 - SPH * HWAVES;
static_assert(SPH * HWAVES <= NT / 64 && SPH * LDS_HALF <= 160 * 1024 - 512 && (GP / GS) % SPH == 0, "wave roles");
constexpr int LDS_HYBRID_BYTES = LDS_HYBRID_PANEL + (HPW_MAX > 0 ? HPW_MAX : 0) * PNS * PSTAGE_BYTES;
constexpr int LDS_DYN_MAX2 = SPH * LDS_HALF > LDS_PANEL_BYTES ? SPH * LDS_HALF : LDS_PANEL_BYTES;
constexpr int LDS_DYN_BYTES = LDS_HYBRID_BYTES > LDS_DYN_MAX2 ? LDS_HYBRID_BYTES : LDS_DYN_MAX2;
__device__ __forceinline__ void acc_lift(float& M, float& S, float tm)
{
    const bool need = tm > M + (RESC_HI - RESC_EARLY);
    const float newM = need ? floorf(tm) + RESC_LIFT : M;
    const int sh = (int)fmaxf(M - newM, -4096.0f);
    S = __builtin_ldexpf(S, sh);
    M = newM;
}

struct PanelGeom {
    int pirow[4];
    unsigned voff;
    unsigned fvoff;
    unsigned gvoff;
};

template <int DIR>
__device__ __forceinline__ size_t panel_tile_off(const PanelGeom& G, int m, int T, size_t Bs)
{
// ... 57 lines not shown
__device__ __forceinline__ void panel_wait_younger(int y)
{
    if (y >= 44) wait_vmcnt<44>();
    else if (y >= 36) wait_vmcnt<36>();
    else if (y >= 28) wait_vmcnt<28>();
    else if (y >= 20) wait_vmcnt<20>();
    else if (y >= 10) wait_vmcnt<10>();
    else wait_vmcnt<0>();
}

struct PanelTask { int k, part, g, q4; };

__device__ __forceinline__ void panel_tt_decode(int tt, PanelTask& t)
{
    if (tt < LEADT - 1) { t.part = 0; t.k = FAR0 + tt; return; }
    tt -= LEADT - 1;
    int a = 0;
    while (tt >= TPT * (a + 1) * (a + 2) / 2) ++a;
    tt -= TPT * a * (a + 1) / 2;
    const int q = a * TPT + tt / (a + 1) + LEADT - 1;
    t.part = tt % (a + 1);
    t.k = FAR0 + q;
}
__device__ __forceinline__ void panel_task_decode(const SweepParams& P, int task, PanelTask& t)
{
    t.q4 = task & 3;
    const int t2 = task >> 2;
    t.g = t2 % P.nPanelGroups;
    panel_tt_decode(t2 / P.nPanelGroups, t);
}

__device__ __forceinline__ bool panel_next_task(const SweepParams& P, PanelTask& t)
{
    int task = 0;
    if ((threadIdx.x & 63) == 0) task = (int)(atomicAdd(P.ctrl + 2, 1u) + 1u);
    task = __builtin_amdgcn_readfirstlane(task) + P.taskBase;
    if (task >= P.nTasks) return false;
    panel_task_decode(P, task, t);
    return true;
}

template <int MODE, int DIR, bool GRAD>
__device__ __forceinline__ void panel_role(const SweepParams& P, char* lds, int wslot, int hist_role = 0, int first_task = -1)
{
    const int T = P.T, B = P.B;
    const int c0 = P.c0, c1 = P.c1;
    const unsigned dbg = DBGF(P);
    unsigned* const ctrl = P.ctrl;
    u64* const farg = P.farg;
    const float* const vfwd = P.vfwd;
    const float* const logZp = P.logZ;
    const float* const goutp = P.gout;
    float* const dScore = P.dScore;
    const int lane = threadIdx.x & 63;
    const int slot = lane >> 3, q8 = lane & 7;
    const size_t Bs = (size_t)B;
    const float* __restrict__ score = P.score;
    const unsigned tag = P.tag;
    const auto ursrc = __builtin_amdgcn_make_buffer_rsrc((void*)P.ug, 0, (int)((size_t)T * Bs * 4), 0x00020000);
    const bool cell_nt = __builtin_amdgcn_readfirstlane(P.cellNT) != 0, grad_nt = __builtin_amdgcn_readfirstlane(P.gradNT) != 0;

    auto geom_of = [&](const PanelTask& t, PanelGeom& G) {
        const int pb = t.k * PB + t.q4 * 4;
        const int cc = c0 + t.g * GP + q8 * 4;
        const int ccl = cc < c1 ? cc : c0;
#pragma unroll
        for (int rr = 0; rr < 4; ++rr) G.pirow[rr] = pb + rr < T ? pb + rr : T - 1;
        G.voff = DIR == 0 ? (unsigned)((slot * B + ccl) * 4) : (unsigned)(((size_t)(7 - slot) * T * Bs + ccl) * 4);
        const int f_pisub = lane >> 4, f_pjsub = (lane >> 3) & 1;
        const int f_pirow = pb + f_pisub < T ? pb + f_pisub : T - 1;
        G.fvoff = DIR == 0 ? G.voff : (unsigned)((((size_t)(1 - f_pjsub) * T + (G.pirow[3] - f_pirow)) * Bs + ccl) * 4);
        G.gvoff = (unsigned)((slot * B + ccl) * 4);
    };
    int issued = 0, mark0 = 0, mark1 = 0, mark2 = 0;
    bool tracer = false;
    int tn = 0;

    while (true) {
        PanelTask tk;
        if (first_task >= 0 && first_task < P.nTasks) {
            panel_task_decode(P, first_task, tk);
#if SEMICRF_STAGGER > 0
            for (int i = 0, n = tk.k - FAR0 < 48 ? tk.k - FAR0 : 48; i < n; ++i) __builtin_amdgcn_s_sleep(SEMICRF_STAGGER);
#endif
        } else if (!panel_next_task(P, tk)) break;
        first_task = -1;
        if (SEMICRF_PROBE_TASKS && (dbg & 256u) && tk.k == RING && tk.part == 0 && tk.g == 0 && tk.q4 == 0) tracer = true;
        u64* const tsp = P.ts + (3 * T) / 2 + 5 * tn;
        const bool tr = SEMICRF_PROBE_TASKS && tracer && lane == 0 && 5 * tn + 5 <= T / 2;
        if (tr) tsp[0] = __builtin_amdgcn_s_memrealtime();
        const int q = tk.k - FAR0;
        int m0, m1;
        part_tiles(q, tk.part, m0, m1);
        const int k = tk.k, part = tk.part, g = tk.g, q4 = tk.q4;
        const int pbase = k * PB + q4 * 4;
        if (pbase >= T) continue;
        const int c = c0 + g * GP + q8 * 4;
        const bool cvalid = c < c1;
        const int cl = cvalid ? c : c0;

        float aM[4][4], aS[4][4];
        int aK[4][4];
#pragma unroll
        for (int rr = 0; rr < 4; ++rr)
#pragma unroll
            for (int i = 0; i < 4; ++i) { aM[rr][i] = SEMICRF_NEG_INF; aS[rr][i] = 0.f; aK[rr][i] = 0x7fffffff; }

        float arow[4][4], gz[4];
        if (GRAD) {
            float lz[4];
#pragma unroll
            for (int i = 0; i < 4; ++i) {
                const bool ok = c + i < c1;
                lz[i] = ok ? logZp[c + i] : 0.f;
                gz[i] = ok ? goutp[(size_t)(c + i) * P.gstride] * P.gscale : 0.f;
            }
#pragma unroll
            for (int rr = 0; rr < 4; ++rr) {
                const int pi = pbase + rr;
#pragma unroll
                for (int i = 0; i < 4; ++i) {
                    const float vv = (c + i < c1 && pi < T) ? vfwd[(size_t)frame_of<DIR>(pi, T) * Bs + c + i] : 0.f;
                    arow[rr][i] = (vv - lz[i]) * LOG2E;
                }
            }
        }
        PanelGeom G;
        geom_of(tk, G);
        char* const stage0 = lds + wslot * (PNS * PSTAGE_BYTES);
        const unsigned rdbase = lds_addr(stage0) + (DIR == 0 ? (unsigned)lane * 16u
                                                             : (unsigned)((slot >> 1) * 1024 + (slot & 1) * 128 + q8 * 16));
        const unsigned grbase = lds_addr(stage0) + 8192u + (unsigned)lane * 16u;
        const bool probe_stream = SEMICRF_PANEL_PROBES && (dbg & 32u);
        const bool probe_nowait = SEMICRF_PANEL_PROBES && (dbg & 4u);
        const bool probe_nou = SEMICRF_PANEL_PROBES && (dbg & 64u);
        const int nst = GRAD ? 2 * (T - pbase < 4 ? T - pbase : 4) : 0;

        bool frontier = false;
#pragma unroll
        for (int i = 0; i < PNS; ++i)
            if (m0 + i < m1) {
                panel_fetch_cells<DIR>(score, G, stage0 + i * PSTAGE_BYTES, m0 + i, T, Bs, cell_nt);
                if (!probe_stream && !probe_nou) panel_fetch_gran<false>(ursrc, stage0 + i * PSTAGE_BYTES, G.gvoff, m0 + i, B);
                issued += 10;
                if (i == 0) mark0 = issued; else if (i == 1) mark1 = issued; else mark2 = issued;
            }

        for (int m = m0, s = 0; m < m1; ++m, s = (s + 1 == PNS ? 0 : s + 1)) {
            char* const stage = stage0 + s * PSTAGE_BYTES;
            const bool tprobe = SEMICRF_PANEL_PROBES && (dbg & 16u) && g == 0 && q4 == 0 && m == q && lane == 0 && k < 64 && T >= 1024;
            if (tprobe) P.ts[1536 + k] = __builtin_amdgcn_s_memrealtime();
            panel_wait_younger(issued - (s == 0 ? mark0 : (s == 1 ? mark1 : mark2)));
            if (tprobe) P.ts[1600 + k] = __builtin_amdgcn_s_memrealtime();
            int npoll = 0;
            if (tr && m == m0) tsp[1] = __builtin_amdgcn_s_memrealtime();
            if (SEMICRF_PROBE_HIST && (dbg & 1024u) && lane == 0) {
                u64* const hb = P.ts + (3 * T) / 2;
                const u64 now = __builtin_amdgcn_s_memrealtime();
                const u64 t0 = __hip_atomic_load(hb + 129 + (__builtin_amdgcn_s_getreg(6164) & 7), __ATOMIC_RELAXED, __HIP_MEMORY_SCOPE_AGENT);
                u64 b = now > t0 ? (now - t0) / 400 : 0;
                if (b > 63) b = 63;
                atomicAdd((unsigned long long*)(hb + 1 + 64 * hist_role + b), 1ull);
            }
            v4u xo[8];
            panel_read_cells<DIR>(rdbase + (unsigned)(s * PSTAGE_BYTES), xo);
            const bool refill = m + PNS < m1;
            if (probe_stream) {
#pragma unroll
                for (int e = 0; e < 8; ++e)
                    aS[0][0] += __uint_as_float(xo[e].x) + __uint_as_float(xo[e].y) + __uint_as_float(xo[e].z) + __uint_as_float(xo[e].w);
            } else {
                v4u g0, g1;
                panel_read_gran(grbase + (unsigned)(s * PSTAGE_BYTES), g0, g1);
                if (!probe_nowait) {
                    const bool v0 = c < c1, v1 = c + 1 < c1, v2 = c + 2 < c1, v3 = c + 3 < c1;
                    int spins = 0;
                    while (true) {
                        const bool ok = (g0.x != U_EMPTY || !v0) && (g0.y != U_EMPTY || !v1) && (g0.z != U_EMPTY || !v2) &&
                                        (g0.w != U_EMPTY || !v3) && (g1.x != U_EMPTY || !v0) && (g1.y != U_EMPTY || !v1) &&
                                        (g1.z != U_EMPTY || !v2) && (g1.w != U_EMPTY || !v3);
                        if (__all(ok)) break;
                        frontier = true;
                        if (m == q) __builtin_amdgcn_s_sleep(2);
                        else if (GRAD) {
                            if (P.gradLazyShort) __builtin_amdgcn_s_sleep(16);
                            else __builtin_amdgcn_s_sleep(SEMICRF_GRAD_LAZY);
                        }
                        else __builtin_amdgcn_s_sleep(16);
                        if (spin_abort(ctrl, spins, SPIN_LIMIT, 5)) break;
                        ++npoll;
                        if (m == q) panel_fetch_gran<true>(ursrc, stage, G.gvoff, m, B);
                        const unsigned pw = __builtin_amdgcn_raw_buffer_load_b32(ursrc, (unsigned)(cl * 4), (unsigned)((m * PB + PB - 1) * B * 4), 16);
                        if (!__all(pw != U_EMPTY || !cvalid)) continue;
                        if (m != q) panel_fetch_gran<true>(ursrc, stage, G.gvoff, m, B);
                        wait_vmcnt<0>();
                        panel_read_gran(grbase + (unsigned)(s * PSTAGE_BYTES), g0, g1);
                    }
                }
                if (frontier && m + 1 < m1) {
// ... 109 lines not shown
                if (!probe_stream && !probe_nou) panel_fetch_gran<false>(ursrc, stage, G.gvoff, m + PNS, B);
                issued += 10;
                if (s == 0) mark0 = issued; else if (s == 1) mark1 = issued; else mark2 = issued;
            }
        }
        if (tr) { tsp[2] = __builtin_amdgcn_s_memrealtime(); tsp[4] = (u64)(m1 - m0) | ((u64)k << 8) | ((u64)(frontier ? 1 : 0) << 16) | ((u64)part << 20); }
        if (!(GRAD && MODE == 0)) wait_vmcnt<0>();
        (void)frontier;
        if (SEMICRF_PANEL_PROBES && (dbg & 16u) && g == 0 && q4 == 0 && m1 == q + 1 && lane == 0 && k < 64 && T >= 1024)
            P.ts[1728 + k] = __builtin_amdgcn_s_memrealtime();

        const bool b5 = (lane & 32) != 0, b4 = (lane & 16) != 0, b3 = (lane & 8) != 0;
        u64* fbase = farg + (size_t)part * T * Bs;
        const int pi = pbase + (b5 ? 2 : 0) + (b4 ? 1 : 0);
        {
            constexpr int RSTR = 65 * 8;
            char* const rb = stage0;
#pragma unroll
            for (int rr = 0; rr < 4; ++rr)
#pragma unroll
                for (int i = 0; i < 4; ++i)
                    *(float2*)(rb + (rr * 4 + i) * RSTR + lane * 8) =
                        make_float2(aM[rr][i], MODE == 0 ? aS[rr][i] : __int_as_float(aK[rr][i]));
            const int orow = (b5 ? 2 : 0) + (b4 ? 1 : 0);
#pragma unroll
            for (int e = 0; e < 2; ++e) {
                const int oi = (b3 ? 2 : 0) + e;
                const char* src = rb + (orow * 4 + oi) * RSTR + q8 * 8;
                float2 v[8];
#pragma unroll
                for (int j = 0; j < 8; ++j) v[j] = *(const float2*)(src + j * 64);
                const int cc = c + oi;
                u64 gr;
                if (MODE == 0) {
                    float mx = v[0].x;
#pragma unroll
                    for (int j = 1; j < 8; ++j) mx = fmaxf(mx, v[j].x);
                    float sum = 0.f;
#pragma unroll
                    for (int j = 0; j < 8; ++j) sum += v[j].y == 0.0f ? 0.0f : v[j].y * fexp2(v[j].x - mx);
                    gr = make_granule(tag, mx + flog2(sum));
                } else {
                    float bm = v[0].x;
                    int bk = __float_as_int(v[0].y);
#pragma unroll
                    for (int j = 1; j < 8; ++j) max_push(bm, bk, v[j].x, __float_as_int(v[j].y));
                    gr = make_granule_key(tag, bm, bk);
                }
                if (pi < T && cc < c1 && !(SEMICRF_PANEL_PROBES && (dbg & 32u))) store_granule(fbase + (size_t)pi * Bs + cc, gr);
            }
        }
        if (SEMICRF_PANEL_PROBES && (dbg & 16u) && g == 0 && m1 == q + 1 && lane == 0 && k < 64)
            P.ts[256 + 64 * q4 + k] = __builtin_amdgcn_s_memrealtime();
        if (tr) tsp[3] = __builtin_amdgcn_s_memrealtime();
        ++tn;
    }
}

__device__ __forceinline__ void zero_row(float* __restrict__ dScore, int e, int T, int B, int lane)
{
    const size_t n = (size_t)(T - 1 - e) * B;
    float* rowp = dScore + ((size_t)e * T + e + 1) * B;
    const size_t lead = (4 - (((uintptr_t)rowp >> 2) & 3)) & 3;
    const size_t head = lead < n ? lead : n;
    const size_t n4 = (n - head) / 4;
    typedef float f32x4 __attribute__((ext_vector_type(4)));
    f32x4* v = (f32x4*)(rowp + head);
    const f32x4 z = {0.f, 0.f, 0.f, 0.f};
    for (size_t i = lane; i < n4; i += 64) __builtin_nontemporal_store(z, v + i);
    if ((size_t)lane < head) rowp[lane] = 0.f;
    const size_t tail0 = head + n4 * 4;
    if (tail0 + lane < n) rowp[tail0 + lane] = 0.f;
}
__device__ __forceinline__ void zero_role(const SweepParams& P)
{
    const int T = P.T, B = P.B;
    float* const dScore = P.dScore;
    unsigned* const ctrl = P.ctrl;
    const int lane = threadIdx.x & 63;
    const int npairs = T / 2;
    while (true) {
        int p = 0;
        if (lane == 0) p = (int)(atomicAdd(ctrl + 3, 1u) + 1u);
        p = __builtin_amdgcn_readfirstlane(p);
        if (p >= npairs) break;
        const int e2 = T - 2 - p;
        if (p <= e2) zero_row(dScore, p, T, B, lane);
        if (p < e2) zero_row(dScore, e2, T, B, lane);
    }
}

constexpr int CTRL_BANDQ = 32;

template <int DIR>
__device__ __forceinline__ void band_role(const SweepParams& P)
{
    const int T = P.T, B = P.B, K = P.K, c0 = P.c0, c1 = P.c1;
    const size_t Bs = (size_t)B;
    unsigned* const ctrl = P.ctrl;
    const float* __restrict__ score = P.score;
    float* const dScore = P.dScore;
    const int lane = threadIdx.x & 63;
    const int q8 = lane & 7, pjsub = (lane >> 3) & 1, pisub = lane >> 4;
    const int nG = P.nPanelGroups;
    const int nTasks = K * FAR0 * nG * 4;
    const size_t last4 = (size_t)T * T * Bs - 4;
    const auto ursrc = __builtin_amdgcn_make_buffer_rsrc((void*)P.ug, 0, (int)((size_t)T * Bs * 4), 0x00020000);
    const bool grad_nt = __builtin_amdgcn_readfirstlane(P.gradNT) != 0;
    while (true) {
        int task = 0;
        if (lane == 0) task = (int)(atomicAdd(ctrl + CTRL_BANDQ, 1u) + 1u);
        task = __builtin_amdgcn_readfirstlane(task);
        if (task >= nTasks) break;
        const int q4 = task & 3, t2 = task >> 2;
        const int g = t2 % nG, t3 = t2 / nG;
        const int dk = t3 % FAR0, m = t3 / FAR0, k = m + dk;
        const int pbase = k * PB + q4 * 4;
        if (k >= K || pbase >= T) continue;
#if defined(SEMICRF_BAND_ABL) && SEMICRF_BAND_ABL == 2
        continue;
#endif
        const int pi = pbase + pisub;
        const bool rowok = pi < T;
        const int pic = rowok ? pi : T - 1;
        const int c = c0 + g * GP + q8 * 4;
        const int cl = c < c1 ? c : c0;
        const bool v0 = c < c1, v1 = c + 1 < c1, v2 = c + 2 < c1, v3 = c + 3 < c1;
        float gz[4], ar[4];
        {
            const int fr = frame_of<DIR>(pic, T);
#pragma unroll
            for (int i = 0; i < 4; ++i) {
                const bool ok = c + i < c1;
                const float lz = ok ? P.logZ[c + i] : 0.f;
                gz[i] = ok ? P.gout[(size_t)(c + i) * P.gstride] * P.gscale : 0.f;
                ar[i] = ok ? (P.vfwd[(size_t)fr * Bs + c + i] - lz) * LOG2E : 0.f;
            }
        }
        v4u x[8], uu[8];
        size_t off[8];
        unsigned uoff[8];
        bool use[8];
#pragma unroll
        for (int e = 0; e < 8; ++e) {
            const int pj = m * PB + 2 * e + pjsub;
            use[e] = rowok && pj < pi;
            const int pjc = pj < pic ? pj : (pic > 0 ? pic - 1 : 0);
            off[e] = cell_index<DIR>(pic, pjc, T) * Bs + cl;
            uoff[e] = (unsigned)(((size_t)pjc * Bs + cl) * 4);
            const v4u_a4 t = *(const v4u_a4*)(score + (off[e] < last4 ? off[e] : last4));
            x[e] = t;
            uu[e] = __builtin_amdgcn_raw_buffer_load_b128(ursrc, uoff[e], 0, 0);
        }
        {
            int spins = 0;
            while (true) {
                bool ok = true;
#pragma unroll
                for (int e = 0; e < 8; ++e)
                    ok = ok && (uu[e].x != U_EMPTY || !v0) && (uu[e].y != U_EMPTY || !v1) && (uu[e].z != U_EMPTY || !v2) && (uu[e].w != U_EMPTY || !v3);
                if (__all(ok)) break;
                __builtin_amdgcn_s_sleep(64);
                if (spin_abort(ctrl, spins, SPIN_LIMIT, 14)) break;
#pragma unroll
                for (int e = 0; e < 8; ++e) uu[e] = __builtin_amdgcn_raw_buffer_load_b128(ursrc, uoff[e], 0, 16);
            }
        }
#pragma unroll
        for (int e = 0; e < 8; ++e) {
            if (!use[e] || !v0) continue;
            v4u gv;
            gv.x = __float_as_uint(gz[0] * fexp2(fmaf(__uint_as_float(x[e].x), LOG2E, __uint_as_float(uu[e].x)) + ar[0]));
            gv.y = __float_as_uint(gz[1] * fexp2(fmaf(__uint_as_float(x[e].y), LOG2E, __uint_as_float(uu[e].y)) + ar[1]));
            gv.z = __float_as_uint(gz[2] * fexp2(fmaf(__uint_as_float(x[e].z), LOG2E, __uint_as_float(uu[e].z)) + ar[2]));
            gv.w = __float_as_uint(gz[3] * fexp2(fmaf(__uint_as_float(x[e].w), LOG2E, __uint_as_float(uu[e].w)) + ar[3]));
            float* const dst = dScore + off[e];
#if defined(SEMICRF_BAND_ABL) && SEMICRF_BAND_ABL == 1
            asm volatile("" ::"v"(gv));
            continue;
#endif
            if (v3) {
                const v4u_a4 ga = gv;
                if (grad_nt) __builtin_nontemporal_store(ga, (v4u_a4*)dst);
                else *(v4u_a4*)dst = ga;
            }
            else {
                dst[0] = __uint_as_float(gv.x);
                if (v1) dst[1] = __uint_as_float(gv.y);
                if (v2) dst[2] = __uint_as_float(gv.z);
            }
        }
    }
}

__device__ __forceinline__ void path_role(const SweepParams& P)
{
    const int nb = P.c1 - P.c0;
    while (true) {
        int i = 0;
        if ((threadIdx.x & 63) == 0) i = (int)(atomicAdd(P.ctrl + CTRL_PATHQ, 1u) + 1u);
        i = __builtin_amdgcn_readfirstlane(i);
        if (i >= nb) break;
        const int c = P.c0 + i;
        const double r = path_score_wave(P.score, P.noise, P.T, P.B, P.pathK, P.pathPairs, P.pathOffsets, c);
        __builtin_amdgcn_wave_barrier();
        store_granule(P.pathg + c, make_granule(P.tag, (float)r));
    }
}

__host__ __device__ __forceinline__ int wg_ticket(int nSpine, int grid, int b)
{
    constexpr int X = 8, SPG = GP / GS / SPH;
    const int ngroups = (nSpine + SPG - 1) / SPG;
    int S[X], W[X];
    bool fits = true;
#pragma unroll
    for (int x = 0; x < X; ++x) {
        W[x] = x < grid ? (grid - x + X - 1) / X : 0;
        int sx = 0;
        for (int g = x; g < ngroups; g += X) sx += nSpine - g * SPG < SPG ? nSpine - g * SPG : SPG;
        S[x] = sx;
        fits = fits && sx <= W[x];
    }
    if (!fits) return b;
    const int x = b % X, slot = b / X;
    int Sx = 0, Px = 0;
#pragma unroll
    for (int i = 0; i < X; ++i) if (i == x) { Sx = S[i]; Px = W[i] - S[i]; }
    (void)Px;
    if (slot < Sx) return (x + X * (slot / SPG)) * SPG + slot % SPG;
    const int ps = slot - Sx;
    int rank = 0;
#pragma unroll
    for (int i = 0; i < X; ++i) {
        const int pn = W[i] - S[i];
        rank += ps < pn ? ps : pn;
        if (i < x && pn > ps) ++rank;
    }
    return nSpine + rank;
}

template <int MODE, int DIR, bool GRAD>
__global__ __launch_bounds__(NT) void persist_sweep_kernel(SweepParams P)
{
    extern __shared__ __attribute__((aligned(16))) char s_dyn[];
    __shared__ int s_exit;
    if (threadIdx.x == 0) {
        const unsigned e1 = __hip_atomic_load(P.ctrl + 1, __ATOMIC_RELAXED, __HIP_MEMORY_SCOPE_AGENT);
        const unsigned gen = P.selfclean ? __hip_atomic_load(P.ctrl + CTRL_GEN, __ATOMIC_RELAXED, __HIP_MEMORY_SCOPE_AGENT) : P.expect_gen;
        s_abort = e1 != CTRL_INIT ? 1 : 0;
        if (gen != P.expect_gen) { set_error(P.ctrl, 13u); s_abort = 1; }
        s_exit = 0;
    }
    for (int h = 0; h < SPH; ++h)
        for (int i = threadIdx.x; i < (LDS_DUMMY - LDS_FAR) / 4; i += NT) ((int*)(s_dyn + h * LDS_HALF + LDS_FAR))[i] = 0;
    __syncthreads();
    const int nSpineWG = (P.nSpine + SPH - 1) / SPH;
    const int ticket = wg_ticket(nSpineWG, (int)gridDim.x, (int)blockIdx.x);
    const int wave = (int)(threadIdx.x >> 6);
// ... 218 lines not shown
    return dev;
}
static int device_cus()
{
    static std::atomic<int> ncu[MAX_DEVICES];
    const int dev = current_device();
    int n = ncu[dev].load();
    if (n == 0) {
        int v = 0;
        n = 256;
        if (hipDeviceGetAttribute(&v, hipDeviceAttributeMultiprocessorCount, dev) == hipSuccess && v > 0) n = v;
        ncu[dev].store(n);
    }
    return n;
}

size_t persist_workspace_bytes(int T, int B)
{
    return CTRL_BYTES + align_up((size_t)2 * T * sizeof(u64)) + (size_t)max_parts(T) * align_up((size_t)T * B * sizeof(u64)) +
           2 * align_up((size_t)T * B * sizeof(unsigned)) +
           align_up((size_t)B * sizeof(u64)) +
           band_flag_bytes(T, B) + band_copy_bytes(T, B);
}

bool persist_supported(int T, int B)
{
    return B >= 2 && T >= 2 && T < 65535 && (long long)T * B * 64 < (1ll << 31) &&
           (B + GS - 1) / GS <= MAX_CHUNKS * (device_cus() / 2 > 0 ? device_cus() / 2 : 1);
}

static unsigned next_tag()
{
    static std::atomic<unsigned> counter{0};
    const unsigned lo = (counter.fetch_add(1) % 65534u) + 1u;
    return (lo << 16) | lo;
}

struct Knobs { int hybrid_waves, hybrid_start, panel_waves, zero_waves, band_waves, nfarw; };
static Knobs read_knobs()
{
#if defined(SEMICRF_DEBUG_BUILD) && SEMICRF_DEBUG_BUILD
    auto get = [](const char* name) { const char* e = getenv(name); return e ? atoi(e) : -1; };
    return Knobs{get("SEMICRF_HYBRID_PANEL_WAVES"), get("SEMICRF_HYBRID_START"), get("SEMICRF_PANEL_WAVES"), get("SEMICRF_ZERO_WAVES"),
                 get("SEMICRF_BAND_WAVES"), get("SEMICRF_NFARW_RT")};
#else
    return Knobs{-1, -1, -1, -1, -1, -1};
#endif
}

struct GradArgs {
    const float* vfwd; const float* logZ; const float* gout; float* dScore; float* dNoise; int gstride; float gscale;
    int keep_upper;
    float noise_add;
};
struct PathArgs { const int* pairs; const int* offsets; int K; float* out; };

template <int MODE, int DIR, bool GRAD>
static void launch_one(const SweepParams& P, int grid, hipStream_t stream)
{
    static std::atomic<bool> attr_set[MAX_DEVICES];
    const int dev = current_device();
    if (!attr_set[dev].load()) {
        (void)hipFuncSetAttribute((const void*)persist_sweep_kernel<MODE, DIR, GRAD>,
                                  hipFuncAttributeMaxDynamicSharedMemorySize, LDS_DYN_BYTES);
        attr_set[dev].store(true);
    }
    hipLaunchKernelGGL((persist_sweep_kernel<MODE, DIR, GRAD>), dim3(grid), dim3(NT), LDS_DYN_BYTES, stream, P);
}

static int launch_persist_sweep_impl(int mode, int dir, const float* score, const float* noise, int T, int B,
                                     float* u_out, float* last_out, int* code, void* ws, hipStream_t stream,
                                     const GradArgs* grad, int lease, unsigned lease_tag, const PathArgs* path = nullptr)
{
    SweepParams P;
    P.pathPairs = nullptr; P.pathOffsets = nullptr; P.pathK = 0; P.pathOut = nullptr; P.pathg = nullptr; P.pathSpine = 0; P.noiseAdd = 0.0f;
    P.vfwd = nullptr; P.logZ = nullptr; P.gout = nullptr; P.dScore = nullptr; P.dNoise = nullptr; P.gstride = 1; P.gscale = 1.0f;
    if (grad) {
        P.vfwd = grad->vfwd; P.logZ = grad->logZ; P.gout = grad->gout; P.dScore = grad->dScore; P.dNoise = grad->dNoise;
        P.gstride = grad->gstride; P.gscale = grad->gscale; P.noiseAdd = grad->noise_add;
    }
    P.score = score; P.noise = noise; P.T = T; P.B = B; P.K = (T + PB - 1) / PB;
    P.band = nullptr; P.bandFlags = nullptr; P.bandSpines = (B + GS - 1) / GS; P.bandGroups = (B + GP - 1) / GP; P.bandK0 = 0; P.copyWaves = 0;
    P.tag = lease_tag ? (lease_tag % 65534u) + 1u : next_tag();
    P.dbg = 0u;
    P.selfclean = 0;
#if SEMICRF_PANEL_PROBES
    if (const char* dbg = getenv("SEMICRF_DEBUG_FLAGS")) P.dbg = (unsigned)atoi(dbg);
    if (SEMICRF_CT_DBG >= 0) P.dbg = (unsigned)SEMICRF_CT_DBG;
#endif
    char* w = (char*)ws;
    P.ts = (u64*)(w + CTRL_BYTES);
    const size_t ts_bytes = align_up((size_t)2 * T * sizeof(u64));
    P.farg = (u64*)(w + CTRL_BYTES + ts_bytes);
    const size_t ug_off = CTRL_BYTES + ts_bytes + (size_t)max_parts(T) * align_up((size_t)T * B * sizeof(u64));
    const size_t ug_bytes = align_up((size_t)T * B * sizeof(unsigned));
    const unsigned upar = lease != 0 ? (lease_tag & 1u) : 0u;
    P.ug = (unsigned*)(w + ug_off + upar * ug_bytes);
    P.ug_other = nullptr;
    const size_t band_off = ug_off + 2 * ug_bytes + align_up((size_t)B * sizeof(u64));
    const bool band_ok = band_in_sweep(T, B);
    if (path && mode == 0 && dir == 0 && !grad) {
        P.pathPairs = path->pairs ? path->pairs : path->offsets; P.pathOffsets = path->offsets; P.pathK = path->K; P.pathOut = path->out;
        P.pathg = (u64*)(w + ug_off + 2 * ug_bytes);
    }
    P.u_out = u_out; P.last_out = last_out; P.code = code;
    const size_t fill_bytes = (SEMICRF_PANEL_PROBES && (P.dbg & 512u)) ? ug_off : persist_workspace_bytes(T, B) - band_copy_bytes(T, B);
    if (P.dbg != 0u) lease = lease ? 1 : 0;
    if (lease != 2) hipLaunchKernelGGL(fill_ff_kernel, dim3(1024), dim3(256), 0, stream, (v4u*)ws, (fill_bytes + 15) / 16);
    P.selfclean = lease != 0 && P.dbg == 0u;
    if (P.selfclean) P.ug_other = (unsigned*)(w + ug_off + (1u - upar) * ug_bytes);
    P.expect_gen = (lease == 2 && P.selfclean) ? ((lease_tag - 1u) % 65534u) + 1u : CTRL_INIT;
    static const Knobs knobs = read_knobs();

    const int ncu = device_cus();
    const int nSpineTotal = (B + GS - 1) / GS;
    const int maxSpine = ncu / 2 > 0 ? ncu / 2 : 1;
    const int nchunks = (nSpineTotal + maxSpine - 1) / maxSpine;
    if (nchunks > MAX_CHUNKS) return 1;
    int perChunk = (nSpineTotal + nchunks - 1) / nchunks;
    perChunk = (perChunk + GP / GS - 1) / (GP / GS) * (GP / GS);
    if (perChunk > maxSpine) perChunk = maxSpine / (GP / GS) * (GP / GS) > 0 ? maxSpine / (GP / GS) * (GP / GS) : maxSpine;
    for (int ci = 0; ci < nchunks; ++ci) {
        P.c0 = ci * perChunk * GS;
        P.c1 = P.c0 + perChunk * GS < B ? P.c0 + perChunk * GS : B;
        if (P.c0 >= P.c1) break;
        const int nb = P.c1 - P.c0;
        P.nSpine = (nb + GS - 1) / GS;
        P.nPanelGroups = (nb + GP - 1) / GP;
        long long ntask = 0;
        for (int q = 0; q < P.K - FAR0; ++q) ntask += nparts_of(q);
        ntask *= 4;
        P.nTasks = (int)(ntask * P.nPanelGroups);
        P.ctrl = (unsigned*)w + (size_t)ci * CTRL_WORDS;
        const int nSpineWG = (P.nSpine + SPH - 1) / SPH;
        int nPanelWG = ncu - nSpineWG;
        if (nPanelWG < 0) nPanelWG = 0;
        int hpw = HPW_MAX > 0 ? HPW_MAX : 0;
        if (knobs.hybrid_waves >= 0 && knobs.hybrid_waves <= HPW_MAX) hpw = knobs.hybrid_waves;
        int hstart = grad ? SEMICRF_GRAD_HSTART : P.K * 5 / 8;
        hstart = hstart < 8 ? 8 : (hstart > 40 ? 40 : hstart);
        if (knobs.hybrid_start >= 0) hstart = knobs.hybrid_start;
        P.hybridStart = hstart;
        P.hybridPanelWaves = hpw;
        int pw = (T >= 1024 && nb >= 256) ? PW_MAX : (PW_MAX < 4 ? PW_MAX : 4);
        if (knobs.panel_waves > 0) pw = knobs.panel_waves;
        if (pw < 1) pw = 1;
        if (pw > PW_MAX) pw = PW_MAX;
        P.panelWaves = pw;
        int zw = 0;
        if (grad && ci == 0 && !grad->keep_upper) {
            zw = 2;
            if (knobs.zero_waves >= 0) zw = knobs.zero_waves;
            if (zw > NT / 64 - pw) zw = NT / 64 - pw;
            if (nPanelWG <= 0 || P.nTasks == 0) zw = 0;
            if (zw == 0 && T > 1) {
                launch_zero_upper(grad->dScore, T, B, stream);
            }
        }
        P.zeroWaves = zw;
        int bw = 0;
        if (grad && nPanelWG > 0 && P.nTasks > 0) {
            bw = 3;
            if (knobs.band_waves >= 0) bw = knobs.band_waves;
            if (bw > NT / 64 - pw - zw) bw = NT / 64 - pw - zw;
        }
        P.bandWaves = bw;
        P.gradLazyShort = nb < 256 ? 1 : 0;
        P.nfarw = (!grad && nb <= SEMICRF_NFARW2_MAXB && T >= SEMICRF_NFARW2_MINT && NFARW >= 2) ? 2 : 1;
        if (knobs.nfarw >= 1 && knobs.nfarw <= NFARW) P.nfarw = knobs.nfarw;
        P.cellNT = cell_policy_nt(T, B, SEMICRF_NT_MIN_MB) ? 1 : 0;
        if (!SEMICRF_NT_MISALIGNED && grad && B % 32 != 0) P.cellNT = 0;
        P.gradNT = cell_policy_nt(T, B, SEMICRF_GRAD_NT_MIN_MB) ? 1 : 0;
        if (P.nTasks == 0) nPanelWG = 0;
        P.pathSpine = nPanelWG == 0 ? 1 : 0;
        P.band = nullptr; P.copyWaves = 0;
        if (band_ok && !grad && nchunks == 1 && nPanelWG > 0 && NT / 64 - pw - zw - bw - 1 >= SEMICRF_BANDX_WAVES) {
            P.bandFlags = (unsigned*)(w + band_off);
            P.band = (float*)(w + band_off + band_flag_bytes(T, B));
            P.bandK0 = SEMICRF_BANDX_K0;
            P.copyWaves = SEMICRF_BANDX_WAVES;
        }
        const int grid = nSpineWG + nPanelWG;
        P.taskBase = nPanelWG * P.panelWaves;
        if (P.taskBase > P.nTasks) P.taskBase = P.nTasks;
        if (grad) launch_one<0, 1, true>(P, grid, stream);
        else if (mode == 0 && dir == 0) launch_one<0, 0, false>(P, grid, stream);
        else if (mode == 0 && dir == 1) launch_one<0, 1, false>(P, grid, stream);
        else if (mode == 1 && dir == 0) launch_one<1, 0, false>(P, grid, stream);
        else launch_one<1, 1, false>(P, grid, stream);
    }
    return 0;
}

int launch_persist_sweep(int mode, int dir, const float* score, const float* noise, int T, int B, float* u_out,
                         float* last_out, int* code, void* ws, hipStream_t stream, int lease, unsigned lease_tag)
{
    return launch_persist_sweep_impl(mode, dir, score, noise, T, B, u_out, last_out, code, ws, stream, nullptr, lease, lease_tag);
}

int launch_persist_logprob_fwd(const float* score, const float* noise, int T, int B, float* u_out, float* logZ, const int* pairs,
                               int K, const int* offsets, float* logProb, void* ws, hipStream_t stream, int lease, unsigned lease_tag)
{
    const PathArgs pa{pairs, offsets, K, logProb};
    return launch_persist_sweep_impl(0, 0, score, noise, T, B, u_out, logZ, nullptr, ws, stream, nullptr, lease, lease_tag, &pa);
}

int launch_persist_logz_bwd(const float* score, const float* noise, const float* v, const float* logZ,
                            const float* gout, int T, int B, float* dScore, float* dNoise, float* q_out, void* ws,
                            hipStream_t stream, int lease, unsigned lease_tag, int gstride, float gscale, int keep_upper, float noise_add)
{
    GradArgs ga{v, logZ, gout, dScore, dNoise, gstride, gscale, keep_upper, noise_add};
    return launch_persist_sweep_impl(0, 1, score, noise, T, B, q_out, nullptr, nullptr, ws, stream, &ga, lease, lease_tag);
}

int persist_wg_ticket(int nSpine, int grid, int b) { return wg_ticket(nSpine, grid, b); }
int persist_spine_wgs_per_group() { return GP / GS / SPH; }

const unsigned* persist_error_words(void* pws, int* n, int* stride)
{
    *n = MAX_CHUNKS; *stride = (int)CTRL_WORDS;
    return (const unsigned*)pws + 1;
}

int persist_set_host_abort_word(unsigned* devptr)
{
    static std::atomic<bool> done[MAX_DEVICES];
    const int dev = current_device();
    if (done[dev].load()) return 0;
    if (hipMemcpyToSymbol(HIP_SYMBOL(g_host_abort), &devptr, sizeof(devptr)) != hipSuccess) return 1;
    done[dev].store(true);
    return 0;
}

int read_and_clear_device_status()
{
    unsigned v = 0, z = 0;
    if (hipDeviceSynchronize() != hipSuccess) return -1;
    if (hipMemcpyFromSymbol(&v, HIP_SYMBOL(g_dev_status), sizeof(v)) != hipSuccess) return -1;
    if (v != 0 && hipMemcpyToSymbol(HIP_SYMBOL(g_dev_status), &z, sizeof(z)) != hipSuccess) return -1;
    return (int)v;
}

}
```

### transkun_amd/csrc/pymarshal.c

```c
#define PY_SSIZE_T_CLEAN
#include <Python.h>
#include <stdint.h>

static PyObject* m_unpack(PyObject* self, PyObject* args)
{
    unsigned long long pa, oa;
    long B, T;
    if (!PyArg_ParseTuple(args, "KKll", &pa, &oa, &B, &T)) return NULL;
    const int32_t* pairs = (const int32_t*)(uintptr_t)pa;
    const int32_t* off = (const int32_t*)(uintptr_t)oa;
    if (B < 0 || T < 1) { PyErr_SetString(PyExc_ValueError, "bad B/T"); return NULL; }
    PyObject** ints = (PyObject**)PyMem_Malloc(sizeof(PyObject*) * (size_t)T);
    if (!ints) return PyErr_NoMemory();
    for (long i = 0; i < T; ++i) {
        ints[i] = PyLong_FromLong(i);
        if (!ints[i]) { for (long j = 0; j < i; ++j) Py_DECREF(ints[j]); PyMem_Free(ints); return NULL; }
    }
    PyObject* out = PyList_New(B);
    int ok = out != NULL;
    for (long c = 0; ok && c < B; ++c) {
        const long n0 = off[c], n1 = off[c + 1];
        if (n1 < n0) { PyErr_SetString(PyExc_ValueError, "offsets not ascending"); ok = 0; break; }
        PyObject* lst = PyList_New(n1 - n0);
        if (!lst) { ok = 0; break; }
// ... 51 lines not shown
    int ordered = 0;
    if (!PyArg_ParseTuple(args, "OKLKl|p", &iv, &pa, &cap, &oa, &T, &ordered)) return NULL;
    int32_t* pairs = (int32_t*)(uintptr_t)pa;
    int32_t* off = (int32_t*)(uintptr_t)oa;
    PyObject* seq = PySequence_Fast(iv, "intervals must be a sequence of sequences");
    if (!seq) return NULL;
    const Py_ssize_t B = PySequence_Fast_GET_SIZE(seq);
    long long k = 0;
    off[0] = 0;
    for (Py_ssize_t c = 0; c < B; ++c) {
        PyObject* lst = PySequence_Fast(PySequence_Fast_GET_ITEM(seq, c), "each chain must hold a sequence of (begin, end)");
        if (!lst) { Py_DECREF(seq); return NULL; }
        const Py_ssize_t n = PySequence_Fast_GET_SIZE(lst);
        for (Py_ssize_t i = 0; i < n; ++i) {
            PyObject* p = PySequence_Fast_GET_ITEM(lst, i);
            long b, e;
            if (PyTuple_CheckExact(p) && PyTuple_GET_SIZE(p) == 2) {
                b = PyLong_AsLong(PyTuple_GET_ITEM(p, 0));
                e = PyLong_AsLong(PyTuple_GET_ITEM(p, 1));
            } else {
                PyObject* ps = PySequence_Fast(p, "an interval must be a (begin, end) pair");
                if (!ps) { Py_DECREF(lst); Py_DECREF(seq); return NULL; }
                if (PySequence_Fast_GET_SIZE(ps) != 2) {
                    Py_DECREF(ps); Py_DECREF(lst); Py_DECREF(seq);
                    PyErr_SetString(PyExc_ValueError, "an interval must be a (begin, end) pair");
                    return NULL;
                }
                b = PyLong_AsLong(PySequence_Fast_GET_ITEM(ps, 0));
                e = PyLong_AsLong(PySequence_Fast_GET_ITEM(ps, 1));
                Py_DECREF(ps);
            }
            if ((b == -1 || e == -1) && PyErr_Occurred()) { Py_DECREF(lst); Py_DECREF(seq); return NULL; }
            if (b < 0 || b >= T || e < 0 || e >= T) {
                Py_DECREF(lst); Py_DECREF(seq);
                PyErr_Format(PyExc_IndexError, "interval index out of range for T=%ld", T);
                return NULL;
            }
            if (ordered && b > e) {
                Py_DECREF(lst); Py_DECREF(seq);
                PyErr_Format(PyExc_ValueError, "interval (%ld, %ld) of chain %zd has begin > end", b, e, c);
                return NULL;
            }
            if (k >= cap) { Py_DECREF(lst); Py_DECREF(seq); PyErr_SetString(PyExc_ValueError, "pairs buffer too small"); return NULL; }
            pairs[2 * k] = (int32_t)b; pairs[2 * k + 1] = (int32_t)e;
            ++k;
        }
        Py_DECREF(lst);
        off[c + 1] = (int32_t)k;
    }
    Py_DECREF(seq);
    return PyLong_FromLongLong(k);
}


#include <descrobject.h>
#include <structmember.h>
#include <stdlib.h>
#include <string.h>

typedef struct { double start, end, vel; char on, off, settled; } TmEv;
typedef struct { double start, end; PyObject* obj; } TmFin;
typedef struct { TmEv* v; long n, cap; int seen; long first_step; double first_start, first_end;
                 long nfin; TmFin* f; long nf, fcap; } TmTrack;
typedef struct { long n_files, P; int merge; TmTrack* tracks;
                 int eager;
                 PyObject* cls; PyObject* pseq; Py_ssize_t so[6]; int vel_float; } TmMerger;

static void tm_free(PyObject* cap)
{
    TmMerger* m = (TmMerger*)PyCapsule_GetPointer(cap, "semicrf.tm");
    if (!m) return;
    if (m->tracks) {
        for (long i = 0; i < m->n_files * m->P; ++i) {
            free(m->tracks[i].v);
            for (long k = 0; k < m->tracks[i].nf; ++k) Py_XDECREF(m->tracks[i].f[k].obj);
            free(m->tracks[i].f);
        }
        free(m->tracks);
    }
    Py_XDECREF(m->cls); Py_XDECREF(m->pseq);
    free(m);
}

static PyObject* m_tm_new(PyObject* self, PyObject* args)
{
    long n_files, P; int merge;
    if (!PyArg_ParseTuple(args, "llp", &n_files, &P, &merge)) return NULL;
    if (n_files < 1 || P < 1) { PyErr_SetString(PyExc_ValueError, "bad sizes"); return NULL; }
    TmMerger* m = (TmMerger*)calloc(1, sizeof(TmMerger));
    if (!m) return PyErr_NoMemory();
    m->n_files = n_files; m->P = P; m->merge = merge;
    m->tracks = (TmTrack*)calloc((size_t)(n_files * P), sizeof(TmTrack));
    if (!m->tracks) { free(m); return PyErr_NoMemory(); }
    return PyCapsule_New(m, "semicrf.tm", tm_free);
}

static int tm_push(TmTrack* t, const TmEv* e)
{
    if (t->n == t->cap) {
        const long nc = t->cap ? 2 * t->cap : 16;
        TmEv* nv = (TmEv*)realloc(t->v, (size_t)nc * sizeof(TmEv));
        if (!nv) return -1;
        t->v = nv; t->cap = nc;
    }
    t->v[t->n++] = *e;
    return 0;
// ... 311 lines not shown
    for (long k = 0; k < nk; ++k) {
        const long s = keys[k].sym;
        for (long i = 0; i < tr[s].n; ++i)
            if (tr[s].v[i].off) {
                TmOut* o = &ev[n];
                o->start = tr[s].v[i].start; o->end = tr[s].v[i].end; o->vel = tr[s].v[i].vel; o->sym = s; o->pitch = keys[k].pitch;
                o->on = tr[s].v[i].on; o->off = 1; o->idx = n; ++n;
            }
    }
    if (resolve) {
        qsort(ev, (size_t)n, sizeof(TmOut), tm_cmp_time);
        for (long s = 0; s < m->P; ++s) lastp[s] = -1;
        for (long i = 0; i < n; ++i) {
            const long j = lastp[ev[i].sym];
            if (j >= 0 && ev[j].end > ev[i].start) ev[j].end = ev[i].start;
            lastp[ev[i].sym] = i;
        }
        long w = 0;
        for (long i = 0; i < n; ++i) if (ev[i].start < ev[i].end) { ev[w] = ev[i]; ev[w].idx = w; ++w; }
        n = w;
        qsort(ev, (size_t)n, sizeof(TmOut), tm_cmp_time);
    }
    PyObject* out = PyList_New(n);
    PyTypeObject* tp = (PyTypeObject*)cls;
    int ok = out != NULL;
    for (long i = 0; ok && i < n; ++i) {
        PyObject* o = tp->tp_alloc(tp, 0);
        if (!o) { ok = 0; break; }
        PyObject* vals[6];
        vals[0] = PyFloat_FromDouble(ev[i].start);
        vals[1] = PyFloat_FromDouble(ev[i].end);
        vals[2] = PySequence_Fast_GET_ITEM(pseq, ev[i].sym); Py_INCREF(vals[2]);
        vals[3] = vel_float ? PyFloat_FromDouble(ev[i].vel) : PyLong_FromLong((long)ev[i].vel);
        vals[4] = ev[i].on ? Py_True : Py_False; Py_INCREF(vals[4]);
        vals[5] = ev[i].off ? Py_True : Py_False; Py_INCREF(vals[5]);
        for (int k = 0; k < 6; ++k) {
            if (!vals[k]) { ok = 0; continue; }
            *(PyObject**)((char*)o + so[k]) = vals[k];
        }
        PyList_SET_ITEM(out, i, o);
    }
    free(ev); free(keys); free(lastp); Py_DECREF(pseq);
    if (!ok) {
        if (out) { for (long i = 0; i < n; ++i) if (!PyList_GET_ITEM(out, i)) { Py_INCREF(Py_None); PyList_SET_ITEM(out, i, Py_None); } Py_DECREF(out); }
        return PyErr_Occurred() ? NULL : PyErr_NoMemory();
    }
    return out;
}

static PyMethodDef methods[] = {
    {"unpack", m_unpack, METH_VARARGS, "packed int32 pairs/offsets (host addresses) -> list of lists of (begin, end)"},
    {"pack_into", m_pack_into, METH_VARARGS, "list of lists of (begin, end) -> packed int32 buffers; returns K (ordered: begin <= end required)"},
    {"count", m_count, METH_O, "total number of intervals"},
    {"tm_new", m_tm_new, METH_VARARGS, "event merger for n_files recordings of P symbols"},
    {"tm_add", m_tm_add, METH_VARARGS, "merge the packed events of one step (rows of 7 doubles at a host address)"},
    {"tm_finish", m_tm_finish, METH_VARARGS, "the final Note list of one recording"},
    {"tm_eager", m_tm_eager, METH_VARARGS, "make the Notes as events settle (merge on): tm_eager(capsule, NoteClass, pitches, resolve)"},
    {NULL, NULL, 0, NULL}};

static struct PyModuleDef moddef = {PyModuleDef_HEAD_INIT, "_semicrf_marshal", "interval-list marshalling", -1, methods};

PyMODINIT_FUNC PyInit__semicrf_marshal(void) { return PyModule_Create(&moddef); }
```

### transkun_amd/csrc/torch_ops.cpp

```cpp
#define USE_ROCM 1
#include <torch/csrc/stable/accelerator.h>
#include <torch/csrc/stable/library.h>
#include <torch/csrc/stable/tensor.h>

#include "../../include/semicrf_hip.h"
#include "cpu_ops.h"

#include <vector>

using torch::stable::Tensor;
using torch::headeronly::ScalarType;

namespace {

inline void want(const Tensor& t, ScalarType st, int64_t min_numel, const char* name)
{
    STD_TORCH_CHECK(t.defined(), "semicrf: `", name, "` is undefined");
    STD_TORCH_CHECK(t.scalar_type() == st, "semicrf: `", name, "` has the wrong dtype");
    STD_TORCH_CHECK(t.is_contiguous(), "semicrf: `", name, "` must be contiguous");
    STD_TORCH_CHECK(t.numel() >= min_numel, "semicrf: `", name, "` holds ", t.numel(), " elements, the call needs ", min_numel);
}
inline const float* f32(const Tensor& t, int64_t n, const char* name) { want(t, ScalarType::Float, n, name); return n > 0 || t.numel() > 0 ? (const float*)t.data_ptr() : nullptr; }
inline float* f32w(const Tensor& t, int64_t n, const char* name) { return (float*)f32(t, n, name); }
inline int32_t* i32(const Tensor& t, int64_t n, const char* name) { want(t, ScalarType::Int, n, name); return n > 0 || t.numel() > 0 ? (int32_t*)t.data_ptr() : nullptr; }
// ... 255 lines not shown
    check(semicrf_mbr_select(ip(pairs), cfp(weight), ip(offsets), d.K, (int)T, d.B, cfp(tau), tau_stride_of(tau, d.B), ip(pairs_out),
                             fp(probs_out), d.cap, ip(offsets_out), fp(gain), bytes(ws, "ws"), (size_t)ws.numel(), c.stream),
          "semicrf_mbr_select");
}
inline int cmp_dims(const Tensor& est_pairs, const Tensor& est_offsets, const Tensor& ref_pairs, const Tensor& ref_offsets, int64_t T,
                    int64_t tol_begin, int64_t tol_end, const Tensor& stats)
{
    STD_TORCH_CHECK(est_pairs.dim() == 2 && est_pairs.size(1) == 2 && ref_pairs.dim() == 2 && ref_pairs.size(1) == 2,
                    "semicrf: pairs must be [K, 2]");
    const int64_t B = est_offsets.numel() - 1;
    STD_TORCH_CHECK(T >= 1 && B >= 1 && T < (1 << 29) && 7 * B < (1ll << 31), "semicrf: bad T / offsets size");
    STD_TORCH_CHECK(ref_offsets.numel() == B + 1, "semicrf: est_offsets and ref_offsets must have the same length");
    want(est_pairs, ScalarType::Int, 0, "est_pairs");
    want(ref_pairs, ScalarType::Int, 0, "ref_pairs");
    want(est_offsets, ScalarType::Int, B + 1, "est_offsets");
    want(ref_offsets, ScalarType::Int, B + 1, "ref_offsets");
    want(stats, ScalarType::Int, 7 * B, "stats");
    check_tol(tol_begin, tol_end);
    STD_TORCH_CHECK((((uintptr_t)ip(est_pairs) | (uintptr_t)ip(ref_pairs)) & 7) == 0, "semicrf: pairs must be 8-byte aligned");
    return (int)B;
}
void compare_paths(Tensor est_pairs, Tensor est_offsets, Tensor ref_pairs, Tensor ref_offsets, int64_t T, int64_t tol_begin,
                   int64_t tol_end, Tensor stats)
{
    Ctx c(est_offsets); c.same(est_offsets, est_pairs, ref_pairs, ref_offsets, stats);
    const int B = cmp_dims(est_pairs, est_offsets, ref_pairs, ref_offsets, T, tol_begin, tol_end, stats);
    check(semicrf_compare_paths(ip(est_pairs), ip(est_offsets), ip(ref_pairs), ip(ref_offsets), (int)T, B, (int)tol_begin, (int)tol_end,
                                ip(stats), c.stream),
          "semicrf_compare_paths");
}
void eval_path(Tensor score, Tensor noise, Tensor pairs, int64_t K, Tensor offsets, Tensor out, Tensor ws)
{
    Ctx c(score); c.same(score, noise, pairs, offsets, out);
    const Dims d = crf_dims(score, noise);
    STD_TORCH_CHECK(K >= 0, "semicrf: negative interval count");
    check(semicrf_eval_path(cfp(score), cfp(noise), d.T, d.B, i32(pairs, 2 * K, "pairs"), K, i32(offsets, d.B + 1, "offsets"),
                            f32w(out, d.B, "out"), ws.numel() > 0 ? ws.data_ptr() : nullptr, (size_t)ws.numel(), c.stream),
          "semicrf_eval_path");
}
void eval_path_bwd(Tensor gout, int64_t T, int64_t B, Tensor pairs, int64_t K, Tensor offsets, Tensor dScore, bool has_ds, Tensor dNoise,
                   bool has_dn)
{
    Ctx c(gout); c.same(gout, pairs, offsets);
    if (has_ds) c.same(gout, dScore);
    if (has_dn) c.same(gout, dNoise);
    STD_TORCH_CHECK(T >= 1 && B >= 1 && K >= 0 && T < (1 << 29) && B < (1ll << 31), "semicrf: bad sizes");
    check(semicrf_eval_path_bwd(f32(gout, B, "gout"), (int)T, (int)B, i32(pairs, 2 * K, "pairs"), K, i32(offsets, B + 1, "offsets"),
                                has_ds ? f32w(dScore, T * T * B, "dScore") : nullptr, has_dn ? f32w(dNoise, (T - 1) * B, "dNoise") : nullptr,
                                c.stream),
          "semicrf_eval_path_bwd");
}

void logprob_fwd(Tensor score, Tensor noise, Tensor pairs, int64_t K, Tensor offsets, Tensor logProb, Tensor logZ, Tensor v, bool want_v,
                 Tensor ws)
{
    Ctx c(score); c.same(score, noise, pairs, offsets, logProb, logZ, v, ws);
    const Dims d = crf_dims(score, noise);
    STD_TORCH_CHECK(K >= 0, "semicrf: negative interval count");
    check(semicrf_logprob_fwd(cfp(score), cfp(noise), d.T, d.B, i32(pairs, 2 * K, "pairs"), K, i32(offsets, d.B + 1, "offsets"),
                              f32w(logProb, d.B, "logProb"), f32w(logZ, d.B, "logZ"), want_v ? f32w(v, (int64_t)d.T * d.B, "v") : nullptr,
                              bytes(ws, "ws"), (size_t)ws.numel(), c.stream),
          "semicrf_logprob_fwd");
}
void logprob_bwd(Tensor score, Tensor noise, Tensor v, Tensor logZ, Tensor gout, int64_t gstride, Tensor pairs, int64_t K, Tensor offsets,
                 Tensor dScore, Tensor dNoise, int64_t flags, Tensor ws)
{
    Ctx c(score); c.same(score, noise, v, logZ, gout, pairs, offsets, dScore, dNoise, ws);
    const Dims d = crf_dims(score, noise);
    const int64_t TB = (int64_t)d.T * d.B;
    STD_TORCH_CHECK(K >= 0 && (gstride == 0 || gstride == 1), "semicrf: bad interval count / gout stride");
    check(semicrf_logprob_bwd_f(cfp(score), cfp(noise), f32(v, TB, "v"), f32(logZ, d.B, "logZ"), f32(gout, gstride ? d.B : 1, "gout"),
                                (int)gstride, d.T, d.B, i32(pairs, 2 * K, "pairs"), K, i32(offsets, d.B + 1, "offsets"),
                                f32w(dScore, TB * d.T, "dScore"), f32w(dNoise, TB - d.B, "dNoise"), (int)flags, bytes(ws, "ws"),
                                (size_t)ws.numel(), c.stream),
          "semicrf_logprob_bwd");
}

void logz_fwd_cpu(Tensor score, Tensor noise, Tensor logZ, Tensor v, bool want_v, Tensor ws)
{
    all_cpu(score, noise, logZ, v);
    const Dims d = crf_dims(score, noise);
    const int64_t TB = (int64_t)d.T * d.B;
    std::vector<float> scratch;
    float* vv;
    if (want_v) vv = f32w(v, TB, "v");
    else { scratch.resize((size_t)TB); vv = scratch.data(); }
    semicrf_cpu::logz_fwd(cfp(score), cfp(noise), d.T, d.B, f32w(logZ, d.B, "logZ"), vv);
}
void logz_bwd_cpu(Tensor score, Tensor noise, Tensor v, Tensor logZ, Tensor gout, Tensor dScore, Tensor dNoise, Tensor q, bool want_q,
                  int64_t flags, Tensor ws)
{
    all_cpu(score, noise, v, logZ, gout, dScore, dNoise, q);
    const Dims d = crf_dims(score, noise);
    const int64_t TB = (int64_t)d.T * d.B;
    std::vector<float> scratch;
    float* qq;
    if (want_q) qq = f32w(q, TB, "q");
    else { scratch.resize((size_t)TB); qq = scratch.data(); }
    semicrf_cpu::logz_bwd(cfp(score), cfp(noise), f32(v, TB, "v"), f32(logZ, d.B, "logZ"), f32(gout, d.B, "gout"), d.T, d.B,
                          f32w(dScore, TB * d.T, "dScore"), f32w(dNoise, TB - d.B, "dNoise"), qq);
}
void beta_cpu(Tensor score, Tensor noise, Tensor out, Tensor ws)
{
    all_cpu(score, noise, out);
    const Dims d = crf_dims(score, noise);
    semicrf_cpu::logz_bwd(cfp(score), cfp(noise), nullptr, nullptr, nullptr, d.T, d.B, nullptr, nullptr, f32w(out, (int64_t)d.T * d.B, "beta"));
}
void alpha_from_cpu(Tensor score, Tensor noise, Tensor start, Tensor v, Tensor logZ, Tensor ws)
{
    all_cpu(score, noise, start, v, logZ);
    const Dims d = crf_dims(score, noise);
    semicrf_cpu::alpha_from(cfp(score), cfp(noise), i32(start, d.B, "start"), d.T, d.B, f32w(v, (int64_t)d.T * d.B, "v"),
                            f32w(logZ, d.B, "logZ"));
}
void viterbi_cpu(Tensor score, Tensor noise, Tensor start, bool has_start, bool forward, Tensor pairs, Tensor offsets, Tensor ws)
{
    all_cpu(score, noise, pairs, offsets);
    if (has_start) all_cpu(start);
    const Dims d = crf_dims(score, noise);
    STD_TORCH_CHECK(pairs.dim() == 2 && pairs.size(1) == 2, "semicrf: pairs must be [cap, 2]");
    const int32_t* st = has_start ? i32(start, d.B, "start") : nullptr;
    if (st)
        for (int c = 0; c < d.B; ++c) STD_TORCH_CHECK(st[c] >= 0 && st[c] < d.T, "semicrf: forcedStartPos out of range");
    semicrf_cpu::viterbi(cfp(score), cfp(noise), d.T, d.B, st, forward ? 1 : 0, i32(pairs, 0, "pairs"), (int64_t)pairs.size(0),
                         i32(offsets, d.B + 1, "offsets"));
}
void sample_cpu(Tensor score, Tensor noise, Tensor v, int64_t k0, int64_t nSample, int64_t key, Tensor end, bool has_end, Tensor pairs,
// ... 120 lines not shown
    STD_TORCH_CHECK(pairs.dim() == 2 && pairs.size(1) == 2 && pairs.size(0) >= 1, "semicrf: pairs must be [cap, 2], cap >= 1");
    check_tol(tol_begin, tol_end);
    const int64_t cap = pairs.size(0);
    const int ts = tau_stride_of(tau, d.B);
    if (tol_begin == 0 && tol_end == 0)
        semicrf_cpu::marginal_decode(cfp(score), f32(v, TB, "v"), f32(q, TB, "q"), f32(logZ, d.B, "logZ"), d.T, d.B, cfp(tau), ts,
                                     i32(pairs, 2 * cap, "pairs"), f32w(probs, cap, "probs"), cap, i32(offsets, d.B + 1, "offsets"));
    else
        semicrf_cpu::marginal_decode_tol(cfp(score), f32(v, TB, "v"), f32(q, TB, "q"), f32(logZ, d.B, "logZ"), d.T, d.B, cfp(tau), ts,
                                         (int)tol_begin, (int)tol_end, i32(pairs, 2 * cap, "pairs"), f32w(probs, cap, "probs"), cap,
                                         i32(offsets, d.B + 1, "offsets"));
}
void mbr_select_cpu(Tensor pairs, Tensor weight, Tensor offsets, int64_t T, Tensor tau, Tensor pairs_out, Tensor probs_out,
                    Tensor offsets_out, Tensor gain, Tensor ws)
{
    all_cpu(pairs, weight, offsets, tau, pairs_out, probs_out, offsets_out, gain);
    const MbrDims d = mbr_dims(pairs, weight, offsets, T, pairs_out, probs_out, offsets_out, gain);
    const int ts = tau_stride_of(tau, d.B);
    semicrf_cpu::mbr_select(ip(pairs), cfp(weight), ip(offsets), d.K, (int)T, d.B, cfp(tau), ts, ip(pairs_out), fp(probs_out), d.cap,
                            ip(offsets_out), fp(gain));
}
void compare_paths_cpu(Tensor est_pairs, Tensor est_offsets, Tensor ref_pairs, Tensor ref_offsets, int64_t T, int64_t tol_begin,
                       int64_t tol_end, Tensor stats)
{
    all_cpu(est_pairs, est_offsets, ref_pairs, ref_offsets, stats);
    const int B = cmp_dims(est_pairs, est_offsets, ref_pairs, ref_offsets, T, tol_begin, tol_end, stats);
    const int32_t *eo = ip(est_offsets), *ro = ip(ref_offsets);
    STD_TORCH_CHECK(eo[B] <= est_pairs.size(0) && ro[B] <= ref_pairs.size(0), "semicrf: offsets[B] exceeds the pairs buffer");
    semicrf_cpu::compare_paths(ip(est_pairs), eo, ip(ref_pairs), ro, (int)T, B, (int)tol_begin, (int)tol_end, ip(stats));
}
void eval_path_cpu(Tensor score, Tensor noise, Tensor pairs, int64_t K, Tensor offsets, Tensor out, Tensor ws)
{
    all_cpu(score, noise, pairs, offsets, out);
    const Dims d = crf_dims(score, noise);
    STD_TORCH_CHECK(K >= 0, "semicrf: negative interval count");
    const int32_t* pp = i32(pairs, 2 * K, "pairs");
    const int32_t* oo = i32(offsets, d.B + 1, "offsets");
    check_path(pp, K, oo, d.T, d.B);
    semicrf_cpu::eval_path(cfp(score), cfp(noise), d.T, d.B, pp, oo, f32w(out, d.B, "out"));
}
void eval_path_bwd_cpu(Tensor gout, int64_t T, int64_t B, Tensor pairs, int64_t K, Tensor offsets, Tensor dScore, bool has_ds, Tensor dNoise,
                       bool has_dn)
{
    all_cpu(gout, pairs, offsets);
    STD_TORCH_CHECK(T >= 1 && B >= 1 && K >= 0 && T < (1 << 29) && B < (1ll << 31), "semicrf: bad sizes");
    const int32_t* pp = i32(pairs, 2 * K, "pairs");
    const int32_t* oo = i32(offsets, B + 1, "offsets");
    check_path(pp, K, oo, (int)T, (int)B);
    semicrf_cpu::eval_path_bwd(f32(gout, B, "gout"), (int)T, (int)B, pp, oo, has_ds ? f32w(dScore, T * T * B, "dScore") : nullptr,
                               has_dn ? f32w(dNoise, (T - 1) * B, "dNoise") : nullptr);
}

void logprob_fwd_cpu(Tensor score, Tensor noise, Tensor pairs, int64_t K, Tensor offsets, Tensor logProb, Tensor logZ, Tensor v, bool want_v,
                     Tensor ws)
{
    logz_fwd_cpu(score, noise, logZ, v, want_v, ws);
    eval_path_cpu(score, noise, pairs, K, offsets, logProb, ws);
    float* lp = (float*)logProb.data_ptr();
    const float* lz = (const float*)logZ.data_ptr();
    for (int64_t c = 0; c < score.size(2); ++c) lp[c] -= lz[c];
}
void logprob_bwd_cpu(Tensor score, Tensor noise, Tensor v, Tensor logZ, Tensor gout, int64_t gstride, Tensor pairs, int64_t K, Tensor offsets,
                     Tensor dScore, Tensor dNoise, int64_t flags, Tensor ws)
{
    all_cpu(score, noise, v, logZ, gout, pairs, offsets, dScore, dNoise);
    const Dims d = crf_dims(score, noise);
    const int64_t TB = (int64_t)d.T * d.B;
    STD_TORCH_CHECK(K >= 0 && (gstride == 0 || gstride == 1), "semicrf: bad interval count / gout stride");
    const float* g = f32(gout, gstride ? d.B : 1, "gout");
    std::vector<float> gp((size_t)d.B), gn((size_t)d.B), q((size_t)TB);
    for (int c = 0; c < d.B; ++c) { gp[(size_t)c] = g[(size_t)c * gstride]; gn[(size_t)c] = -gp[(size_t)c]; }
    const int32_t* pp = i32(pairs, 2 * K, "pairs");
    const int32_t* oo = i32(offsets, d.B + 1, "offsets");
    check_path(pp, K, oo, d.T, d.B);
    semicrf_cpu::logz_bwd(cfp(score), cfp(noise), f32(v, TB, "v"), f32(logZ, d.B, "logZ"), gn.data(), d.T, d.B, f32w(dScore, TB * d.T, "dScore"),
                          f32w(dNoise, TB - d.B, "dNoise"), q.data());
    semicrf_cpu::eval_path_bwd(gp.data(), d.T, d.B, pp, oo, fp(dScore), fp(dNoise));
}

inline const float* f32s(const Tensor& t, const char* name)
{
    STD_TORCH_CHECK(t.defined() && t.scalar_type() == ScalarType::Float, "semicrf: `", name, "` must be a float32 tensor");
    return t.numel() > 0 ? (const float*)t.data_ptr() : nullptr;
}
inline float* f32so(const Tensor& t, const char* name) { return t.defined() && t.numel() > 0 ? (float*)f32s(t, name) : nullptr; }
inline void score_dims(int64_t C, int64_t T, int64_t D)
{
    STD_TORCH_CHECK(C >= 1 && T >= 1 && D >= 1 && C < (1ll << 31) && T < (1 << 29) && D < (1 << 20), "semicrf: bad C / T / D");
}
inline int64_t slots_of(int64_t C, int64_t group, int64_t pitch)
{
    STD_TORCH_CHECK(group >= 1 && pitch >= group && C % group == 0 && group < (1ll << 31) && pitch < (1ll << 31), "semicrf: bad slot layout");
    return C / group * pitch;
}
void interval_score_fwd_op(Tensor q, Tensor k, Tensor diag, Tensor rowc, int64_t C, int64_t T, int64_t D, int64_t ldq, int64_t ldk,
                           int64_t ldd, int64_t ldrc, double qscale, int64_t mode, int64_t full, int64_t group, int64_t pitch, Tensor S,
                           Tensor noise)
{
    Ctx c(q); c.same(q, k, diag, rowc, S, noise);
    score_dims(C, T, D);
    const int64_t Cs = slots_of(C, group, pitch);
    check(interval_score_fwd_pc(f32s(q, "q"), f32s(k, "k"), f32s(diag, "diag"), ldrc > 0 ? f32s(rowc, "rowc") : nullptr, (int)C, (int)T, (int)D,
                                ldq, ldk, ldd, ldrc > 0 ? ldrc : 1, (float)qscale, (int)mode, (int)full, (int)group, (int)pitch,
                                f32w(S, T * T * Cs, "S"), noise.numel() > 0 ? f32w(noise, (T - 1) * Cs, "noise") : nullptr, c.stream),
          "interval_score_fwd");
}
void interval_score_bwd_ws_op(Tensor dS, Tensor q, Tensor k, int64_t C, int64_t T, int64_t D, int64_t ldq, int64_t ldk, double qscale,
                              int64_t mode, int64_t group, int64_t pitch, Tensor dq, Tensor dk, Tensor ddiag, Tensor drowc, int64_t lddq,
                              int64_t lddk, int64_t lddd, int64_t lddrc, Tensor ws)
{
    Ctx c(dS); c.same(dS, q, k, dq, dk, ddiag, drowc, ws);
    score_dims(C, T, D);
    const int64_t Cs = slots_of(C, group, pitch);
    check(interval_score_bwd_ws_pc(f32(dS, T * T * Cs, "dS"), f32s(q, "q"), f32s(k, "k"), (int)C, (int)T, (int)D, ldq, ldk, (float)qscale,
                                   (int)mode, (int)group, (int)pitch, f32so(dq, "dq"), f32so(dk, "dk"), f32so(ddiag, "ddiag"),
                                   lddrc > 0 ? f32so(drowc, "drowc") : nullptr, lddq, lddk, lddd, lddrc > 0 ? lddrc : 1, bytes(ws, "ws"),
                                   (size_t)ws.numel(), c.stream),
// ... 446 lines not shown
          "segment_onset_filter");
}
void segment_events_op(Tensor pairs, int64_t K, Tensor offsets, int64_t B, int64_t nSym, Tensor ofValue, Tensor ofPresence,
                       int64_t lastFrameIdx, double frameDur, Tensor beginTime, int64_t stepFrames, Tensor times, Tensor flags, Tensor lastP,
                       Tensor nextStart)
{
    Ctx c(offsets); c.same(offsets, pairs, ofValue, ofPresence, beginTime, times, flags, lastP, nextStart);
    STD_TORCH_CHECK(B >= 1 && B < (1ll << 31) && nSym >= 1 && K >= 0, "semicrf: bad B / nSym / K");
    want(ofPresence, ScalarType::Byte, 2 * K, "ofPresence"); want(flags, ScalarType::Byte, 2 * K, "flags");
    want(beginTime, ScalarType::Double, B / nSym, "beginTime"); want(times, ScalarType::Double, 2 * K, "times");
    check(segment_events(i32(pairs, 2 * K, "pairs"), K, i32(offsets, B + 1, "offsets"), (int)B, (int)nSym, f32(ofValue, 2 * K, "ofValue"),
                         K > 0 ? (const unsigned char*)ofPresence.data_ptr() : nullptr, (int)lastFrameIdx, frameDur,
                         (const double*)beginTime.data_ptr(), (int)stepFrames, K > 0 ? (double*)times.data_ptr() : nullptr,
                         K > 0 ? (unsigned char*)flags.data_ptr() : nullptr, i32(lastP, B, "lastP"), i32(nextStart, B, "nextStart"), c.stream),
          "segment_events");
}

}

STABLE_TORCH_LIBRARY(semicrf, m)
{
    m.def("logz_fwd(Tensor score, Tensor noise, Tensor(a!) logZ, Tensor(b!) v, bool want_v, Tensor(c!) ws) -> ()");
    m.def("logz_bwd(Tensor score, Tensor noise, Tensor v, Tensor logZ, Tensor gout, Tensor(a!) dScore, Tensor(b!) dNoise, Tensor(c!) q, "
          "bool want_q, int flags, Tensor(d!) ws) -> ()");
    m.def("beta(Tensor score, Tensor noise, Tensor(a!) out, Tensor(b!) ws) -> ()");
    m.def("alpha_from(Tensor score, Tensor noise, Tensor start, Tensor(a!) v, Tensor(b!) logz, Tensor(c!) ws) -> ()");
    m.def("viterbi(Tensor score, Tensor noise, Tensor start, bool has_start, bool forward, Tensor(a!) pairs, Tensor(b!) offsets, "
          "Tensor(c!) ws) -> ()");
    m.def("sample(Tensor score, Tensor noise, Tensor v, int k0, int nSample, int key, Tensor end, bool has_end, Tensor(a!) pairs, "
          "Tensor(b!) offsets, Tensor(c!) ws) -> ()");
    m.def("viterbi_nbest(Tensor score, Tensor noise, int k, Tensor start, bool has_start, bool forward, Tensor(a!) pairs, "
          "Tensor(b!) offsets, Tensor(c!) scores, Tensor(d!) npaths, Tensor(e!) ws) -> ()");
    m.def("posteriors(Tensor score, Tensor noise, Tensor v, Tensor q, Tensor logZ, Tensor(a!) node, Tensor(b!) begin, Tensor(c!) end, "
          "Tensor(d!) single, Tensor(e!) noiseP, Tensor(f!) entropy, Tensor(g!) ws) -> ()");
    m.def("expectation(Tensor score, Tensor noise, Tensor weight, Tensor nweight, bool has_nw, Tensor v, Tensor q, Tensor(a!) E, Tensor(b!) H, "
          "Tensor(c!) ws) -> ()");
    m.def("covariance(Tensor score, Tensor noise, Tensor weight, Tensor nweight, bool has_nw, Tensor gout, Tensor(a!) C, Tensor(b!) Cn, "
          "Tensor ws) -> ()");
    m.def("interval_marginals(Tensor score, Tensor v, Tensor q, Tensor logZ, Tensor pairs, int K, Tensor offsets, Tensor(a!) out) -> ()");
    m.def("marginal_decode(Tensor score, Tensor noise, Tensor v, Tensor q, Tensor logZ, Tensor tau, Tensor(a!) pairs, Tensor(b!) probs, "
          "Tensor(c!) offsets, Tensor(d!) ws) -> ()");
    m.def("interval_marginals_tol(Tensor score, Tensor v, Tensor q, Tensor logZ, Tensor pairs, int K, Tensor offsets, int tol_begin, "
          "int tol_end, Tensor(a!) out) -> ()");
    m.def("marginal_decode_tol(Tensor score, Tensor noise, Tensor v, Tensor q, Tensor logZ, Tensor tau, int tol_begin, int tol_end, "
          "Tensor(a!) pairs, Tensor(b!) probs, Tensor(c!) offsets, Tensor(d!) ws) -> ()");
    m.def("mbr_select(Tensor pairs, Tensor weight, Tensor offsets, int T, Tensor tau, Tensor(a!) pairs_out, Tensor(b!) probs_out, "
          "Tensor(c!) offsets_out, Tensor(d!) gain, Tensor(e!) ws) -> ()");
    m.def("compare_paths(Tensor est_pairs, Tensor est_offsets, Tensor ref_pairs, Tensor ref_offsets, int T, int tol_begin, int tol_end, "
          "Tensor(a!) stats) -> ()");
    m.def("eval_path(Tensor score, Tensor noise, Tensor pairs, int K, Tensor offsets, Tensor(a!) out, Tensor(b!) ws) -> ()");
    m.def("eval_path_bwd(Tensor gout, int T, int B, Tensor pairs, int K, Tensor offsets, Tensor(a!) dScore, bool has_ds, Tensor(b!) dNoise, "
          "bool has_dn) -> ()");
    m.def("logprob_fwd(Tensor score, Tensor noise, Tensor pairs, int K, Tensor offsets, Tensor(a!) logProb, Tensor(b!) logZ, Tensor(c!) v, "
          "bool want_v, Tensor(d!) ws) -> ()");
    m.def("logprob_bwd(Tensor score, Tensor noise, Tensor v, Tensor logZ, Tensor gout, int gstride, Tensor pairs, int K, Tensor offsets, "
          "Tensor(a!) dScore, Tensor(b!) dNoise, int flags, Tensor(c!) ws) -> ()");
    m.def("interval_score_fwd(Tensor q, Tensor k, Tensor diag, Tensor rowc, int C, int T, int D, int ldq, int ldk, int ldd, int ldrc, "
          "float qscale, int mode, int full, int group, int pitch, Tensor(a!) S, Tensor(b!) noise) -> ()");
    m.def("interval_score_bwd_ws(Tensor dS, Tensor q, Tensor k, int C, int T, int D, int ldq, int ldk, float qscale, int mode, int group, "
          "int pitch, Tensor(a!) dq, Tensor(b!) dk, Tensor(c!) ddiag, Tensor(d!) drowc, int lddq, int lddk, int lddd, int lddrc, "
          "Tensor(e!) ws) -> ()");
    m.def("interval_score_bwd_fused_ws(Tensor S, Tensor alpha, Tensor beta, Tensor logZ, Tensor gout, Tensor q, Tensor k, int C, int T, int D, "
          "int ldq, int ldk, float qscale, int mode, int group, int pitch, Tensor(a!) dq, Tensor(b!) dk, Tensor(c!) ddiag, Tensor(d!) drowc, "
          "int lddq, int lddk, int lddd, int lddrc, Tensor(e!) ws) -> ()");
    m.def("interval_score_path_bwd(Tensor gout, Tensor pairs, int K, Tensor offsets, Tensor q, Tensor k, int C, int T, int D, int ldq, int ldk, "
          "float qscale, int mode, int group, int pitch, Tensor(a!) dq, Tensor(b!) dk, Tensor(c!) ddiag, Tensor(d!) drowc, int lddq, int lddk, "
          "int lddd, int lddrc) -> ()");
    m.def("proj_nn(Tensor A, int lda, int M, int K, Tensor B, int ldb, int N, Tensor(a!) out, int ldout, Tensor bias, bool has_bias, Tensor w2, "
          "Tensor b2, bool has_w2, int zero_cols, bool accumulate) -> ()");
    m.def("proj_nn3(Tensor A, int lda, int M, int K, Tensor B, int ldb, int N, Tensor(a!) out, int ldout, Tensor bias, bool has_bias, Tensor w2, "
          "Tensor b2, bool has_w2, int zero_cols, bool accumulate, Tensor(b!) ws) -> ()");
    m.def("stage_linear(Tensor W, Tensor bias, int D, int size, int rows_pad, Tensor(a!) BT, Tensor(b!) Wqd, Tensor(c!) w2, Tensor(d!) b2) -> ()");
    m.def("merge_weights_fwd(Tensor W, Tensor bias, int D, int size, int rows, Tensor(a!) Wm, Tensor(b!) bm, Tensor(c!) WmT, bool has_t) -> ()");
    m.def("merge_weights_bwd(Tensor W, Tensor bias, Tensor dWm, Tensor dbm, int D, int size, int rows, Tensor(a!) dW, Tensor(b!) dbias, Tensor(c!) ws) -> ()");
    m.def("proj_tn(Tensor dy, int lddy, int M, int R, int extra_col0, int total_rows, Tensor x, int ldx, int N, Tensor(a!) dW, int lddw, "
          "Tensor(b!) db, Tensor(c!) ws) -> ()");
    m.def("interval_features_gather(Tensor ctx, int C, int T, int D, int ldc, Tensor pairs, int K, Tensor offsets, int nSym, Tensor(a!) out, "
          "Tensor(b!) symIdx, Tensor(c!) scatterIdx) -> ()");
    m.def("interval_features_gather_bwd(Tensor gout, Tensor ctx, int C, int T, int D, int ldc, Tensor pairs, int K, Tensor offsets, "
          "Tensor(a!) dctx, int lddc) -> ()");
    m.def("attribute_loss_fwd(Tensor logitsVelocity, Tensor ofLogits, Tensor velocity, Tensor ofRefined, Tensor ofPresence, int K, "
          "Tensor offsets, int C, Tensor base, bool has_base, Tensor(a!) rowLogProb, Tensor(b!) out) -> ()");
    m.def("attribute_loss_bwd(Tensor gout, int gstride, Tensor logitsVelocity, Tensor ofLogits, Tensor velocity, Tensor ofRefined, "
          "Tensor ofPresence, int K, Tensor offsets, int C, Tensor(a!) dLogitsVelocity, Tensor(b!) dOfLogits) -> ()");
    m.def("attribute_decode(Tensor logitsVelocity, Tensor ofLogits, int K, int criterion, Tensor(a!) velocityClass, Tensor(b!) velocityMean, "
          "Tensor(c!) ofValue, Tensor(d!) ofPresence) -> ()");
    m.def("attribute_heads(Tensor ctx, int C, int T, int D, int ldc, Tensor pairs, int K, Tensor offsets, int nSym, Tensor W1, Tensor b1, "
          "Tensor W2, Tensor b2, int Hv, int Ho, int Nv, int No, Tensor(a!) logitsVelocity, Tensor(b!) ofLogits, Tensor(c!) symIdx, "
          "Tensor(d!) scatterIdx, Tensor(e!) ws) -> ()");
    m.def("attribute_heads_train_fwd(Tensor ctx, int C, int T, int D, int ldc, Tensor pairs, int K, Tensor offsets, int nSym, Tensor W1, "
          "Tensor b1, Tensor W2, Tensor b2, int Hv, int Ho, int Nv, int No, int seed, float pv, float po, Tensor(a!) logitsVelocity, "
          "Tensor(b!) ofLogits, Tensor(c!) z, Tensor(d!) symIdx, Tensor(e!) scatterIdx, Tensor(f!) ws) -> ()");
    m.def("attribute_heads_bwd(Tensor dLogitsVelocity, Tensor dOfLogits, Tensor z, Tensor ctx, int C, int T, int D, int ldc, Tensor pairs, "
          "int K, Tensor offsets, Tensor W1, Tensor W2, int Hv, int Ho, int Nv, int No, int seed, float pv, float po, Tensor(a!) dctx, "
          "Tensor(b!) dW1, Tensor(c!) db1, Tensor(d!) dW2, Tensor(e!) db2, Tensor(f!) ws) -> ()");
    m.def("attribute_heads_dropout_mask(Tensor(a!) mask, int seed, int K, int Hv, int Ho, float pv, float po) -> ()");
    m.def("grad_sqnorm(Tensor flat, int numel, Tensor(a!) partials) -> ()");
    m.def("clip_from_history(Tensor partials, bool has_partials, int numel, Tensor norm_in, bool has_norm, float q, Tensor(a!) ring, "
          "int capacity, Tensor(b!) state, bool append, Tensor(c!) stats) -> ()");
    m.def("adabelief_step(Tensor(a!) p, Tensor g, Tensor(b!) m, Tensor(c!) s, int numel, Tensor coef, bool has_coef, Tensor table) -> ()");
    m.def("segment_onset_filter(Tensor pairs, Tensor offsets, int B, int bound, Tensor(a!) pairs_out, Tensor(b!) offsets_out, "
          "Tensor(c!) counts_ws) -> ()");
    m.def("segment_events(Tensor pairs, int K, Tensor offsets, int B, int nSym, Tensor ofValue, Tensor ofPresence, int lastFrameIdx, "
          "float frameDur, Tensor beginTime, int stepFrames, Tensor(a!) times, Tensor(b!) flags, Tensor(c!) lastP, Tensor(d!) nextStart) -> ()");
}

STABLE_TORCH_LIBRARY_IMPL(semicrf, CPU, m)
{
    m.impl("logz_fwd", TORCH_BOX(&logz_fwd_cpu));
// ... 79 lines not shown
```

Baseline: 1911 steps/s.

## Fold path-score gradient into persistent backward sweep via per-frame path table

The forward persistent sweep now writes a per-(t,chain) path table that encodes interval begin/end and coverage for ordered, non-overlapping paths. The backward persistent sweep streams this table into LDS next to v and applies the path gradient inline, so the separate eval_path_bwd scatter kernel can be skipped. This removes a kernel launch and a scatter pass over dScore. In exchange it adds a T×B int32 table write in the forward pass, one more LDS constant slot and loader stream in the backward sweep, and a host-side O(K) simplicity check during packing.

```diff
diff --git a/include/semicrf_hip.h b/include/semicrf_hip.h
--- a/include/semicrf_hip.h
+++ b/include/semicrf_hip.h
@@ -133,6 +133,17 @@
 int semicrf_logprob_bwd_f(const float* score, const float* noise, const float* v, const float* logZ, const float* gout,
                           int gout_stride, int T, int B, const int32_t* pairs, int64_t K, const int32_t* offsets,
                           float* dScore, float* dNoise, int flags, void* ws, size_t ws_bytes, semicrf_stream_t stream);
+
+#define SEMICRF_PTAB_COVERED (1 << 30)
+#define SEMICRF_PTAB_NONE ((1 << 30) - 1)
+int semicrf_logprob_path_table_supported(int T, int B);
+int semicrf_logprob_fwd_t(const float* score, const float* noise, int T, int B, const int32_t* pairs, int64_t K,
+                          const int32_t* offsets, float* logProb, float* logZ, float* v, int32_t* ptab, void* ws, size_t ws_bytes,
+                          semicrf_stream_t stream);
+int semicrf_logprob_bwd_t(const float* score, const float* noise, const float* v, const float* logZ, const float* gout,
+                          int gout_stride, int T, int B, const int32_t* pairs, int64_t K, const int32_t* offsets,
+                          float* dScore, float* dNoise, int flags, const int32_t* ptab, void* ws, size_t ws_bytes,
+                          semicrf_stream_t stream);
 
 int interval_score_fwd(const float* q, const float* k, const float* diag, int C, int T, int D,
                        int64_t ldq, int64_t ldk, int64_t ldd, float qscale, int length_scaling,
diff --git a/transkun_amd/CRF/NeuralSemiCRFInterval.py b/transkun_amd/CRF/NeuralSemiCRFInterval.py
--- a/transkun_amd/CRF/NeuralSemiCRFInterval.py
+++ b/transkun_amd/CRF/NeuralSemiCRFInterval.py
@@ -74,6 +74,7 @@
         pairs_d = pairs_h.to(device, non_blocking=True)
         offsets_d = offsets_h.to(device, non_blocking=True)
     pairs_d._semicrf_K = K
+    pairs_d._semicrf_simple = bool(ordered) and bool(mm.path_is_simple(pairs_h.data_ptr(), offsets_h.data_ptr(), B))
     return pairs_d, offsets_d
 
 
@@ -256,7 +257,17 @@
     return dscore, dnoise, (q if want_q else None)
 
 
-def _logprob_fwd_raw(score, noise, pairs, offsets, want_v: bool):
+PATH_FOLD = True
+PATH_ROUTES = {"folded": 0, "scatter": 0}
+
+
+def _path_table_ok(score, pairs) -> bool:
+    if not (PATH_FOLD and score.is_cuda and getattr(pairs, "_semicrf_simple", False)) or _odd_pad(score):
+        return False
+    return _lib.load().semicrf_logprob_path_table_supported(int(score.shape[0]), int(score.shape[2])) == 1
+
+
+def _logprob_fwd_raw(score, noise, pairs, offsets, want_v: bool, ptab=None):
     K = getattr(pairs, "_semicrf_K", pairs.shape[0])
     if _odd_pad(score):
         logz, v = _logz_fwd_raw(score, noise, want_v)
@@ -267,7 +278,8 @@
     logz = torch.empty(B, dtype=torch.float32, device=dev)
     v = torch.empty((T, B) if want_v else (0,), dtype=torch.float32, device=dev)
     ws = _lib.leased_workspace(_lib.OP_LOGZ_FWD, T, B, dev)
-    _lib.ops().logprob_fwd(score, noise, pairs, int(K), offsets, lp, logz, v, want_v, ws)
+    _lib.ops().logprob_fwd(score, noise, pairs, int(K), offsets, lp, logz, v, want_v, ws, ptab if ptab is not None else offsets,
+                           ptab is not None)
     return lp, logz, (v if want_v else None)
 
 
@@ -478,17 +490,21 @@
         T, B = score_c.shape[0], score_c.shape[2]
         K = getattr(pairs, "_semicrf_K", pairs.shape[0])
         _ready(pairs)
-        lp, logz, v = _logprob_fwd_raw(score_c, noise_c, pairs, offsets, need)
+        ptab = torch.empty((T, B), dtype=torch.int32, device=score_c.device) if need and _path_table_ok(score_c, pairs) else None
+        lp, logz, v = _logprob_fwd_raw(score_c, noise_c, pairs, offsets, need, ptab)
         if need:
-            ctx.save_for_backward(score_c, noise_c, v, logz, pairs, offsets)
+            ctx.save_for_backward(score_c, noise_c, v, logz, pairs, offsets, *([ptab] if ptab is not None else []))
             ctx.K = K
         ctx.in_dtypes = (score.dtype, noiseScore.dtype)
         return lp.to(score.dtype)
 
     @staticmethod
     def backward(ctx, grad_output):
-        score, noise, v, logz, pairs, offsets = ctx.saved_tensors
+        score, noise, v, logz, pairs, offsets = ctx.saved_tensors[:6]
+        ptab = ctx.saved_tensors[6] if len(ctx.saved_tensors) > 6 else None
         T, B = score.shape[0], score.shape[2]
+        folded = ptab is not None and PATH_FOLD and _lib.load().semicrf_logprob_path_table_supported(int(T), int(B)) == 1
+        PATH_ROUTES["folded" if folded else "scatter"] += 1
         if _odd_pad(score):
             g = _gout(grad_output, B)
             dscore, dnoise, _ = _logz_bwd_raw(score, noise, v, logz, -g)
@@ -498,7 +514,8 @@
             dscore, flags, pkey = _GRAD_POOL.take(T, B, score.device)
             dnoise = torch.empty_like(noise)
             ws = _lib.leased_workspace(_lib.OP_LOGZ_BWD, T, B, score.device)
-            _lib.ops().logprob_bwd(score, noise, v, logz, g, gstride, pairs, int(ctx.K), offsets, dscore, dnoise, flags, ws)
+            _lib.ops().logprob_bwd(score, noise, v, logz, g, gstride, pairs, int(ctx.K), offsets, dscore, dnoise, flags, ws,
+                                   ptab if folded else offsets, folded)
             _GRAD_POOL.give(pkey, dscore)
         return dscore.to(ctx.in_dtypes[0]), dnoise.to(ctx.in_dtypes[1]), None, None
 
diff --git a/transkun_amd/_lib.py b/transkun_amd/_lib.py
--- a/transkun_amd/_lib.py
+++ b/transkun_amd/_lib.py
@@ -55,6 +55,9 @@
     "semicrf_async_error": (ctypes.c_int, []),
     "semicrf_logz_bwd_f": (_i, [_vp, _vp, _vp, _vp, _vp, _i, _i, _vp, _vp, _vp, _i, _vp, _sz, _vp]),
     "semicrf_logprob_bwd_f": (_i, [_vp, _vp, _vp, _vp, _vp, _i, _i, _i, _vp, _i64, _vp, _vp, _vp, _i, _vp, _sz, _vp]),
+    "semicrf_logprob_path_table_supported": (_i, [_i, _i]),
+    "semicrf_logprob_fwd_t": (_i, [_vp, _vp, _i, _i, _vp, _i64, _vp, _vp, _vp, _vp, _vp, _vp, _sz, _vp]),
+    "semicrf_logprob_bwd_t": (_i, [_vp, _vp, _vp, _vp, _vp, _i, _i, _i, _vp, _i64, _vp, _vp, _vp, _i, _vp, _vp, _sz, _vp]),
     "semicrf_debug_wg_ticket": (_i, [_i, _i, _i]),
     "semicrf_debug_score_variant": (None, [_i]),
     "semicrf_logz_fwd": (_i, [_vp, _vp, _i, _i, _vp, _vp, _vp, _sz, _vp]),
diff --git a/transkun_amd/csrc/api.hip b/transkun_amd/csrc/api.hip
--- a/transkun_amd/csrc/api.hip
+++ b/transkun_amd/csrc/api.hip
@@ -159,9 +159,11 @@
 int launch_persist_logz_bwd(const float* score, const float* noise, const float* v, const float* logZ,
                             const float* gout, int T, int B, float* dScore, float* dNoise, float* q_out, void* ws,
                             hipStream_t stream, int lease, unsigned lease_tag, int gstride = 1, float gscale = 1.0f, int keep_upper = 0,
-                            float noise_add = 0.0f);
+                            float noise_add = 0.0f, const int* ptab = nullptr, int* path_folded = nullptr);
 int launch_persist_logprob_fwd(const float* score, const float* noise, int T, int B, float* u_out, float* logZ, const int* pairs,
-                               int K, const int* offsets, float* logProb, void* ws, hipStream_t stream, int lease, unsigned lease_tag);
+                               int K, const int* offsets, float* logProb, void* ws, hipStream_t stream, int lease, unsigned lease_tag,
+                               int* ptab = nullptr);
+int persist_path_fold_possible(int T, int B);
 
 static bool use_persist(int T, int B) { return g_impl.load() == 0 && persist_supported(T, B); }
 
@@ -328,7 +330,7 @@
     return SEMICRF_OK;
 }
 
-struct PathFold { const int32_t* pairs; int64_t K; const int32_t* offsets; float* logProb; int folded; };
+struct PathFold { const int32_t* pairs; int64_t K; const int32_t* offsets; float* logProb; int folded; int32_t* ptab; };
 
 static int logz_fwd_impl(const float* score, const float* noise, int T, int B, float* logZ, float* v, void* ws,
                          size_t ws_bytes, semicrf_stream_t stream, PathFold* pf)
@@ -345,7 +347,7 @@
     if (fast) {
         unsigned ltag = 0;
         const int lease = lease_acquire(ws, SEMICRF_OP_LOGZ_FWD, T, B, &ltag, st);
-        const int rc = pf ? launch_persist_logprob_fwd(score, noise, T, B, vv, logZ, pf->pairs, (int)pf->K, pf->offsets, pf->logProb, pws, st, lease, ltag)
+        const int rc = pf ? launch_persist_logprob_fwd(score, noise, T, B, vv, logZ, pf->pairs, (int)pf->K, pf->offsets, pf->logProb, pws, st, lease, ltag, pf->ptab)
                           : launch_persist_sweep(0, 0, score, noise, T, B, vv, logZ, nullptr, pws, st, lease, ltag);
         if (rc) {
             lease_failed(ws);
@@ -368,7 +370,8 @@
 
 static int logz_bwd_impl(const float* score, const float* noise, const float* v, const float* logZ,
                          const float* gout, int gstride, float gscale, int T, int B, float* dScore, float* dNoise, float* q_out,
-                         int flags, void* ws, size_t ws_bytes, semicrf_stream_t stream, float noise_add = 0.0f, int* noise_folded = nullptr)
+                         int flags, void* ws, size_t ws_bytes, semicrf_stream_t stream, float noise_add = 0.0f, int* noise_folded = nullptr,
+                         const int32_t* ptab = nullptr, int* path_folded = nullptr)
 {
     if (int rc = check_common(score, noise, T, B)) return rc;
     SEMICRF_CHECK_ARG((flags & ~SEMICRF_GRAD_UPPER_IS_ZERO) == 0, "unknown flags %d", flags);
@@ -386,7 +389,7 @@
     if (fast) {
         unsigned ltag = 0;
         const int lease = lease_acquire(ws, SEMICRF_OP_LOGZ_BWD, T, B, &ltag, st);
-        if (launch_persist_logz_bwd(score, noise, v, logZ, gout, T, B, dScore, dNoise, q, pws, st, lease, ltag, gstride, gscale, keep_upper, noise_add)) {
+        if (launch_persist_logz_bwd(score, noise, v, logZ, gout, T, B, dScore, dNoise, q, pws, st, lease, ltag, gstride, gscale, keep_upper, noise_add, ptab, path_folded)) {
             lease_failed(ws);
             set_error("persistent sweep could not be enqueued (too many chain chunks for this device)"); return SEMICRF_ELAUNCH;
         }
@@ -419,9 +422,22 @@
                         const int32_t* offsets, float* logProb, float* logZ, float* v, void* ws, size_t ws_bytes,
                         semicrf_stream_t stream)
 {
+    return semicrf_logprob_fwd_t(score, noise, T, B, pairs, K, offsets, logProb, logZ, v, nullptr, ws, ws_bytes, stream);
+}
+
+int semicrf_logprob_path_table_supported(int T, int B)
+{
+    return (T >= 1 && B >= 1 && use_persist(T, B) && persist_path_fold_possible(T, B)) ? 1 : 0;
+}
+
+int semicrf_logprob_fwd_t(const float* score, const float* noise, int T, int B, const int32_t* pairs, int64_t K,
+                          const int32_t* offsets, float* logProb, float* logZ, float* v, int32_t* ptab, void* ws, size_t ws_bytes,
+                          semicrf_stream_t stream)
+{
     SEMICRF_CHECK_ARG(offsets && logProb && logZ, "offsets/logProb/logZ must be non-NULL");
     SEMICRF_CHECK_ARG(K >= 0 && K < (1ll << 31) && (K == 0 || pairs), "bad interval count");
-    PathFold pf{pairs, K, offsets, logProb, 0};
+    SEMICRF_CHECK_ARG(ptab == nullptr || (T >= 1 && B >= 1 && use_persist(T, B)), "a path table needs the persistent sweep (T=%d, B=%d)", T, B);
+    PathFold pf{pairs, K, offsets, logProb, 0, ptab};
     if (int rc = logz_fwd_impl(score, noise, T, B, logZ, v, ws, ws_bytes, stream, &pf)) return rc;
     if (!pf.folded) launch_eval_path(score, noise, T, B, (int)K, pairs, offsets, logProb, (hipStream_t)stream, logZ);
     SEMICRF_CHECK_LAUNCH("semicrf_logprob_fwd");
@@ -439,12 +455,21 @@
                           int gout_stride, int T, int B, const int32_t* pairs, int64_t K, const int32_t* offsets, float* dScore,
                           float* dNoise, int flags, void* ws, size_t ws_bytes, semicrf_stream_t stream)
 {
+    return semicrf_logprob_bwd_t(score, noise, v, logZ, gout, gout_stride, T, B, pairs, K, offsets, dScore, dNoise, flags, nullptr, ws, ws_bytes,
+                                 stream);
+}
+
+int semicrf_logprob_bwd_t(const float* score, const float* noise, const float* v, const float* logZ, const float* gout,
+                          int gout_stride, int T, int B, const int32_t* pairs, int64_t K, const int32_t* offsets, float* dScore,
+                          float* dNoise, int flags, const int32_t* ptab, void* ws, size_t ws_bytes, semicrf_stream_t stream)
+{
     SEMICRF_CHECK_ARG(offsets, "offsets must be non-NULL");
     SEMICRF_CHECK_ARG(K >= 0 && K < (1ll << 31) && (K == 0 || pairs), "bad interval count");
-    int noise_folded = 0;
+    int noise_folded = 0, path_folded = 0;
     if (int rc = logz_bwd_impl(score, noise, v, logZ, gout, gout_stride, -1.0f, T, B, dScore, dNoise, nullptr, flags, ws, ws_bytes, stream,
-                               1.0f, &noise_folded)) return rc;
-    launch_eval_path_bwd(gout, T, B, (int)K, pairs, offsets, dScore, dNoise, (hipStream_t)stream, gout_stride, 1.0f, noise_folded);
+                               1.0f, &noise_folded, ptab, &path_folded)) return rc;
+    if (!path_folded)
+        launch_eval_path_bwd(gout, T, B, (int)K, pairs, offsets, dScore, dNoise, (hipStream_t)stream, gout_stride, 1.0f, noise_folded);
     SEMICRF_CHECK_LAUNCH("semicrf_logprob_bwd");
     return SEMICRF_OK;
 }
diff --git a/transkun_amd/csrc/pathscore.h b/transkun_amd/csrc/pathscore.h
--- a/transkun_amd/csrc/pathscore.h
+++ b/transkun_amd/csrc/pathscore.h
@@ -21,4 +21,26 @@
     return acc;
 }
 
+constexpr int PTAB_COVERED = 1 << 30;
+constexpr int PTAB_NONE = PTAB_COVERED - 1;
+
+__device__ __forceinline__ void path_table_wave(int* __restrict__ tab, int T, int B, int K, const int* __restrict__ pairs,
+                                                const int* __restrict__ offsets, int c)
+{
+    const int lane = threadIdx.x & 63;
+    const int k0 = offsets[c];
+    int k1 = offsets[c + 1];
+    if (k1 > K) k1 = K;
+    int first = k0 < k1 ? pairs[2 * k0] : T;
+    first = first < 0 ? 0 : (first > T ? T : first);
+    for (int t = lane; t < first; t += 64) tab[(size_t)t * B + c] = PTAB_NONE;
+    for (int k = k0 + lane; k < k1; k += 64) {
+        const int b = pairs[2 * k], e = pairs[2 * k + 1];
+        int hi = k + 1 < k1 ? pairs[2 * k + 2] : T;
+        hi = hi > T ? T : hi;
+        for (int t = b < 0 ? 0 : b; t < hi; ++t)
+            tab[(size_t)t * B + c] = (t == b ? (e & PTAB_NONE) : PTAB_NONE) | (t < e ? PTAB_COVERED : 0);
+    }
 }
+
+}
diff --git a/transkun_amd/csrc/persist.hip b/transkun_amd/csrc/persist.hip
--- a/transkun_amd/csrc/persist.hip
+++ b/transkun_amd/csrc/persist.hip
@@ -133,6 +133,8 @@
     float* pathOut;
     u64* pathg;
     float noiseAdd;
+    int* ptabOut;
+    const int* ptab;
     float* band;
     unsigned* bandFlags;
     int bandSpines;
@@ -164,6 +166,15 @@
     return __hip_atomic_load(p, __ATOMIC_RELAXED, __HIP_MEMORY_SCOPE_AGENT);
 }
 
+template <typename Tp>
+__device__ __forceinline__ Tp kernarg_again(size_t off)
+{
+    typedef __attribute__((address_space(4))) const char ka_t;
+    ka_t* ka = (ka_t*)__builtin_amdgcn_kernarg_segment_ptr();
+    asm volatile("" : "+s"(ka));
+    return *(__attribute__((address_space(4))) const Tp*)(ka + off);
+}
+
 template <int DIR>
 __device__ __forceinline__ int frame_of(int p, int T) { return DIR == 0 ? p : T - 1 - p; }
 
@@ -236,7 +247,7 @@
 #endif
 constexpr int NRBUF = SEMICRF_NRBUF;
 constexpr int TILE_BYTES = PB * PB * RS * 4;
-constexpr int NCONST = 3;
+constexpr int NCONST = 4;
 constexpr int LDS_TILES = 0;
 constexpr int LDS_CONST = LDS_TILES + NRBUF * RING * TILE_BYTES;
 constexpr int LDS_FAR = LDS_CONST + NRBUF * NCONST * 256;
@@ -337,6 +348,7 @@
     const float* const score = P.score;
     const float* const noise = P.noise;
     const float* const vfwd = P.vfwd;
+    const float* const tabw = P.ptab ? (const float*)P.ptab : P.vfwd;
     const int lane = threadIdx.x & 63;
     const int cbase = P.c0 + sg * GS;
     const size_t last4 = (size_t)T * T * Bs - 4;
@@ -347,7 +359,7 @@
     int* const cons = ready + NRBUF;
     int* const nready = cons + RING;
     const int* const fcons = nready + NNSLOT;
-    constexpr int NL = RING * 4 + 2 + (GRAD ? 1 : 0) + NNEAR * 4 + ((GRAD && NNEAR > 0) ? 1 : 0);
+    constexpr int NL = RING * 4 + 2 + (GRAD ? 2 : 0) + NNEAR * 4 + ((GRAD && NNEAR > 0) ? 1 : 0);
     constexpr int LDEPTH = 3 * NL <= 63 ? 3 : 2;
     static_assert(2 * NL <= 63, "loader pipeline");
 
@@ -405,8 +417,10 @@
         __builtin_amdgcn_global_load_lds((gbl_void_t*)(score + ((size_t)frow * T + frow) * Bs + cc), (lds_void_t*)cb, 4, 0, 0);
         __builtin_amdgcn_global_load_lds((gbl_void_t*)(noise + (size_t)gap_of<DIR>(prow_c >= 1 ? prow_c : 1, T) * Bs + cc),
                                          (lds_void_t*)(cb + 256), 4, 0, 0);
-        if (GRAD)
+        if (GRAD) {
             __builtin_amdgcn_global_load_lds((gbl_void_t*)(vfwd + (size_t)frow * Bs + cc), (lds_void_t*)(cb + 512), 4, 0, 0);
+            __builtin_amdgcn_global_load_lds((gbl_void_t*)(tabw + (size_t)frow * Bs + cc), (lds_void_t*)(cb + 768), 4, 0, 0);
+        }
         if (NNEAR > 0) {
             char* const nb = lds + LDS_NEAR + (kr % NNSLOT) * NEAR_SLOT_BYTES;
             if (fromband) {
@@ -678,6 +692,7 @@
     const float4* const far = (const float4*)(lds + LDS_FAR);
     float gz = 0.f, lzc = 0.f;
     float nadd = 0.f;
+    const bool fold = GRAD && P.ptab != nullptr;
     if (GRAD && cvalid) {
         const float go = P.gout[(size_t)c * P.gstride];
         gz = go * P.gscale; lzc = P.logZ[c]; nadd = P.noiseAdd * go;
@@ -714,6 +729,8 @@
         for (int i = 0; i < RING; ++i) X[i] = read_tile(i);
         const float* cst = (const float*)(lds + LDS_CONST + slot * NCONST * 256) + lane;
         const float dcell = cst[0], nzl = cst[64], vfl = cst[128];
+        const int pte = fold ? __float_as_int(cst[192]) : PTAB_NONE;
+        const bool pdiag = (pte & PTAB_NONE) == frow, pgap = (pte & PTAB_COVERED) != 0;
         const float s1own = *(const float*)(lds + LDS_TILES + (slot * RING + RING - 1) * TILE_BYTES +
                                             ((((r > 0 ? r - 1 : 0) * PB) + r) * RS + ch) * 4);
         const float s1 = r == 0 ? X[RING - 2].v[PB - 1] : s1own;
@@ -797,8 +814,11 @@
                         float p = fmaf(X.v[u], LOG2E, uq[q]);
                         if (GRAD && ringBand && rvalid && j < prow) grad_store(j, gz * fexp2(p + arow));
                         if (last && u == PB - 1 && r == 0) {
-                            if (GRAD && rvalid)
-                                dNoise[(size_t)gap_of<DIR>(prow, T) * Bs + c] = gz * fexp2(uq[q] + nz * LOG2E + arow) + nadd;
+                            if (GRAD && rvalid) {
+                                float nv = gz * fexp2(uq[q] + nz * LOG2E + arow) + nadd;
+                                if (pgap) nv = nv - nadd;
+                                dNoise[(size_t)gap_of<DIR>(prow, T) * Bs + c] = nv;
+                            }
                             p = uq[q] + wl;
                         }
                         t[u] = p;
@@ -881,7 +901,11 @@
                     });
                 }
                 const float um1 = __int_as_float(__builtin_amdgcn_update_dpp(0, __float_as_int(mine), 0x111, 0xf, 0xf, false));
-                if (rvalid && r >= 1) dNoise[(size_t)gap_of<DIR>(prow, T) * Bs + c] = gz * fexp2(um1 + nz * LOG2E + arow) + nadd;
+                if (rvalid && r >= 1) {
+                    float nv = gz * fexp2(um1 + nz * LOG2E + arow) + nadd;
+                    if (pgap) nv = nv - nadd;
+                    dNoise[(size_t)gap_of<DIR>(prow, T) * Bs + c] = nv;
+                }
             }
         } else {
             float best = aM;
@@ -930,8 +954,11 @@
                 }
                 pathOut[c] = ok ? __uint_as_float((unsigned)gr) - mine * sc : __uint_as_float(0x7fc00000u);
             }
-            if (GRAD)
-                dScore[((size_t)frow * T + frow) * Bs + c] = gz * fexp2(arow + mine + draw - 2.0f * sp);
+            if (GRAD) {
+                float dv = gz * fexp2(arow + mine + draw - 2.0f * sp);
+                if (pdiag) dv = dv + nadd;
+                dScore[((size_t)frow * T + frow) * Bs + c] = dv;
+            }
             if (MODE == 1) code[(size_t)c * T + frow] = (mykey + 1) | (sp > 0.0f ? 0x40000000 : 0);
         }
         if (SEMICRF_PANEL_PROBES && trace) ts[k] = __builtin_amdgcn_s_memrealtime();
@@ -1095,6 +1122,7 @@
     const float* const logZp = P.logZ;
     const float* const goutp = P.gout;
     float* const dScore = P.dScore;
+    constexpr bool PFOLD = GRAD && DIR == 1;
     const int lane = threadIdx.x & 63;
     const int slot = lane >> 3, q8 = lane & 7;
     const size_t Bs = (size_t)B;
@@ -1168,6 +1196,14 @@
                 }
             }
         }
+        int ptab_words[4] = {PTAB_NONE, PTAB_NONE, PTAB_NONE, PTAB_NONE};
+        const int* const ptab = PFOLD ? kernarg_again<const int*>(offsetof(SweepParams, ptab)) : nullptr;
+        if (PFOLD && ptab != nullptr) {
+            const int prow = pbase + (slot & 3) < T ? pbase + (slot & 3) : T - 1;
+            const int* const pr = ptab + (size_t)frame_of<DIR>(prow, T) * Bs;
+#pragma unroll
+            for (int i = 0; i < 4; ++i) ptab_words[i] = pr[c + i < c1 ? c + i : c1 - 1];
+        }
         PanelGeom G;
         geom_of(tk, G);
         char* const stage0 = lds + wslot * (PNS * PSTAGE_BYTES);
@@ -1188,6 +1224,17 @@
                 issued += 10;
                 if (i == 0) mark0 = issued; else if (i == 1) mark1 = issued; else mark2 = issued;
             }
+
+        bool pathfix = false;
+        if (PFOLD && ptab != nullptr) {
+            bool hit = false;
+#pragma unroll
+            for (int i = 0; i < 4; ++i) {
+                const int pj = T - 1 - (ptab_words[i] & PTAB_NONE);
+                hit = hit | ((unsigned)(pj - m0 * PB) < (unsigned)((m1 - m0) * PB));
+            }
+            pathfix = __any(hit);
+        }
 
         for (int m = m0, s = 0; m < m1; ++m, s = (s + 1 == PNS ? 0 : s + 1)) {
             char* const stage = stage0 + s * PSTAGE_BYTES;
@@ -1403,6 +1450,31 @@
         }
         if (SEMICRF_PANEL_PROBES && (dbg & 16u) && g == 0 && m1 == q + 1 && lane == 0 && k < 64)
             P.ts[256 + 64 * q4 + k] = __builtin_amdgcn_s_memrealtime();
+        if (PFOLD && pathfix) {
+            asm volatile("s_waitcnt vmcnt(0)" ::: "memory");
+            const int* const ptab2 = kernarg_again<const int*>(offsetof(SweepParams, ptab));
+            const float* const gout2 = kernarg_again<const float*>(offsetof(SweepParams, gout));
+            float* const dScore2 = kernarg_again<float*>(offsetof(SweepParams, dScore));
+            const int gstride2 = kernarg_again<int>(offsetof(SweepParams, gstride));
+            const float wpath = kernarg_again<float>(offsetof(SweepParams, noiseAdd));
+            int f0, f1;
+            part_tiles(k - FAR0, part, f0, f1);
+#pragma nounroll
+            for (int n = 0; n < 16; ++n) {
+                const int prow = pbase + (n >> 2), ci = c + (n & 3);
+                if (prow >= T) break;
+                const int fb = frame_of<DIR>(prow, T);
+                const int pend = ptab2[(size_t)fb * Bs + (ci < c1 ? ci : c1 - 1)] & PTAB_NONE;
+                const int pj = T - 1 - pend;
+                if (ci < c1 && (unsigned)(pj - f0 * PB) < (unsigned)((f1 - f0) * PB) && (pj & 7) == (lane >> 3)) {
+                    float* const cell = dScore2 + ((size_t)pend * T + fb) * Bs + ci;
+                    const float mv = __hip_atomic_load(cell, __ATOMIC_RELAXED, __HIP_MEMORY_SCOPE_AGENT);
+                    const float nv = mv + wpath * gout2[(size_t)ci * gstride2];
+                    if (grad_nt) __builtin_nontemporal_store(nv, cell);
+                    else *cell = nv;
+                }
+            }
+        }
         if (tr) tsp[3] = __builtin_amdgcn_s_memrealtime();
         ++tn;
     }
@@ -1451,6 +1523,7 @@
     unsigned* const ctrl = P.ctrl;
     const float* __restrict__ score = P.score;
     float* const dScore = P.dScore;
+    const int* __restrict__ ptab = P.ptab;
     const int lane = threadIdx.x & 63;
     const int q8 = lane & 7, pjsub = (lane >> 3) & 1, pisub = lane >> 4;
     const int nG = P.nPanelGroups;
@@ -1478,14 +1551,20 @@
         const int cl = c < c1 ? c : c0;
         const bool v0 = c < c1, v1 = c + 1 < c1, v2 = c + 2 < c1, v3 = c + 3 < c1;
         float gz[4], ar[4];
+        float gp[4];
+        int pjp[4];
         {
             const int fr = frame_of<DIR>(pic, T);
 #pragma unroll
             for (int i = 0; i < 4; ++i) {
                 const bool ok = c + i < c1;
                 const float lz = ok ? P.logZ[c + i] : 0.f;
-                gz[i] = ok ? P.gout[(size_t)(c + i) * P.gstride] * P.gscale : 0.f;
+                const float go = ok ? P.gout[(size_t)(c + i) * P.gstride] : 0.f;
+                gz[i] = ok ? go * P.gscale : 0.f;
                 ar[i] = ok ? (P.vfwd[(size_t)fr * Bs + c + i] - lz) * LOG2E : 0.f;
+                const int pend = (DIR == 1 && ok && rowok && ptab) ? (ptab[(size_t)fr * Bs + c + i] & PTAB_NONE) : PTAB_NONE;
+                pjp[i] = pend != PTAB_NONE ? T - 1 - pend : -1;
+                gp[i] = P.noiseAdd * go;
             }
         }
         v4u x[8], uu[8];
@@ -1525,6 +1604,13 @@
             gv.y = __float_as_uint(gz[1] * fexp2(fmaf(__uint_as_float(x[e].y), LOG2E, __uint_as_float(uu[e].y)) + ar[1]));
             gv.z = __float_as_uint(gz[2] * fexp2(fmaf(__uint_as_float(x[e].z), LOG2E, __uint_as_float(uu[e].z)) + ar[2]));
             gv.w = __float_as_uint(gz[3] * fexp2(fmaf(__uint_as_float(x[e].w), LOG2E, __uint_as_float(uu[e].w)) + ar[3]));
+            {
+                const int pj = m * PB + 2 * e + pjsub;
+                if (pj == pjp[0]) gv.x = __float_as_uint(__uint_as_float(gv.x) + gp[0]);
+                if (pj == pjp[1]) gv.y = __float_as_uint(__uint_as_float(gv.y) + gp[1]);
+                if (pj == pjp[2]) gv.z = __float_as_uint(__uint_as_float(gv.z) + gp[2]);
+                if (pj == pjp[3]) gv.w = __float_as_uint(__uint_as_float(gv.w) + gp[3]);
+            }
             float* const dst = dScore + off[e];
 #if defined(SEMICRF_BAND_ABL) && SEMICRF_BAND_ABL == 1
             asm volatile("" ::"v"(gv));
@@ -1556,6 +1642,7 @@
         const double r = path_score_wave(P.score, P.noise, P.T, P.B, P.pathK, P.pathPairs, P.pathOffsets, c);
         __builtin_amdgcn_wave_barrier();
         store_granule(P.pathg + c, make_granule(P.tag, (float)r));
+        if (P.ptabOut) path_table_wave(P.ptabOut, P.T, P.B, P.pathK, P.pathPairs, P.pathOffsets, c);
     }
 }
 
@@ -1880,8 +1967,10 @@
     const float* vfwd; const float* logZ; const float* gout; float* dScore; float* dNoise; int gstride; float gscale;
     int keep_upper;
     float noise_add;
+    const int* ptab;
+    int* path_folded;
 };
-struct PathArgs { const int* pairs; const int* offsets; int K; float* out; };
+struct PathArgs { const int* pairs; const int* offsets; int K; float* out; int* ptab; };
 
 template <int MODE, int DIR, bool GRAD>
 static void launch_one(const SweepParams& P, int grid, hipStream_t stream)
@@ -1902,6 +1991,7 @@
 {
     SweepParams P;
     P.pathPairs = nullptr; P.pathOffsets = nullptr; P.pathK = 0; P.pathOut = nullptr; P.pathg = nullptr; P.pathSpine = 0; P.noiseAdd = 0.0f;
+    P.ptabOut = nullptr; P.ptab = nullptr;
     P.vfwd = nullptr; P.logZ = nullptr; P.gout = nullptr; P.dScore = nullptr; P.dNoise = nullptr; P.gstride = 1; P.gscale = 1.0f;
     if (grad) {
         P.vfwd = grad->vfwd; P.logZ = grad->logZ; P.gout = grad->gout; P.dScore = grad->dScore; P.dNoise = grad->dNoise;
@@ -1929,6 +2019,7 @@
     const bool band_ok = band_in_sweep(T, B);
     if (path && mode == 0 && dir == 0 && !grad) {
         P.pathPairs = path->pairs ? path->pairs : path->offsets; P.pathOffsets = path->offsets; P.pathK = path->K; P.pathOut = path->out;
+        P.ptabOut = path->ptab;
         P.pathg = (u64*)(w + ug_off + 2 * ug_bytes);
     }
     P.u_out = u_out; P.last_out = last_out; P.code = code;
@@ -1993,6 +2084,8 @@
             if (bw > NT / 64 - pw - zw) bw = NT / 64 - pw - zw;
         }
         P.bandWaves = bw;
+        P.ptab = (grad && grad->ptab && bw > 0 && nchunks == 1 && NNEAR == 0) ? grad->ptab : nullptr;
+        if (grad && grad->path_folded) *grad->path_folded = P.ptab != nullptr ? 1 : 0;
         P.gradLazyShort = nb < 256 ? 1 : 0;
         P.nfarw = (!grad && nb <= SEMICRF_NFARW2_MAXB && T >= SEMICRF_NFARW2_MINT && NFARW >= 2) ? 2 : 1;
         if (knobs.nfarw >= 1 && knobs.nfarw <= NFARW) P.nfarw = knobs.nfarw;
@@ -2027,18 +2120,27 @@
 }
 
 int launch_persist_logprob_fwd(const float* score, const float* noise, int T, int B, float* u_out, float* logZ, const int* pairs,
-                               int K, const int* offsets, float* logProb, void* ws, hipStream_t stream, int lease, unsigned lease_tag)
-{
-    const PathArgs pa{pairs, offsets, K, logProb};
+                               int K, const int* offsets, float* logProb, void* ws, hipStream_t stream, int lease, unsigned lease_tag, int* ptab)
+{
+    const PathArgs pa{pairs, offsets, K, logProb, ptab};
     return launch_persist_sweep_impl(0, 0, score, noise, T, B, u_out, logZ, nullptr, ws, stream, nullptr, lease, lease_tag, &pa);
 }
 
 int launch_persist_logz_bwd(const float* score, const float* noise, const float* v, const float* logZ,
                             const float* gout, int T, int B, float* dScore, float* dNoise, float* q_out, void* ws,
-                            hipStream_t stream, int lease, unsigned lease_tag, int gstride, float gscale, int keep_upper, float noise_add)
-{
-    GradArgs ga{v, logZ, gout, dScore, dNoise, gstride, gscale, keep_upper, noise_add};
+                            hipStream_t stream, int lease, unsigned lease_tag, int gstride, float gscale, int keep_upper, float noise_add,
+                            const int* ptab, int* path_folded)
+{
+    if (path_folded) *path_folded = 0;
+    GradArgs ga{v, logZ, gout, dScore, dNoise, gstride, gscale, keep_upper, noise_add, ptab, path_folded};
     return launch_persist_sweep_impl(0, 1, score, noise, T, B, q_out, nullptr, nullptr, ws, stream, &ga, lease, lease_tag);
+}
+
+int persist_path_fold_possible(int T, int B)
+{
+    const int ncu = device_cus();
+    const int nSpine = (B + GS - 1) / GS, maxSpine = ncu / 2 > 0 ? ncu / 2 : 1;
+    return NNEAR == 0 && B % 2 == 0 && (T + PB - 1) / PB > FAR0 && nSpine <= maxSpine && ncu - (nSpine + SPH - 1) / SPH > 0;
 }
 
 int persist_wg_ticket(int nSpine, int grid, int b) { return wg_ticket(nSpine, grid, b); }
diff --git a/transkun_amd/csrc/pymarshal.c b/transkun_amd/csrc/pymarshal.c
--- a/transkun_amd/csrc/pymarshal.c
+++ b/transkun_amd/csrc/pymarshal.c
@@ -127,6 +127,21 @@
     return PyLong_FromLongLong(k);
 }
 
+static PyObject* m_path_is_simple(PyObject* self, PyObject* args)
+{
+    unsigned long long pa, oa;
+    long long B;
+    if (!PyArg_ParseTuple(args, "KKL", &pa, &oa, &B)) return NULL;
+    const int32_t* pairs = (const int32_t*)(uintptr_t)pa;
+    const int32_t* off = (const int32_t*)(uintptr_t)oa;
+    for (long long c = 0; c < B; ++c)
+        for (long long k = off[c]; k < off[c + 1]; ++k) {
+            if (pairs[2 * k] > pairs[2 * k + 1]) Py_RETURN_FALSE;
+            if (k > off[c] && (pairs[2 * k] <= pairs[2 * k - 2] || pairs[2 * k] < pairs[2 * k - 1])) Py_RETURN_FALSE;
+        }
+    Py_RETURN_TRUE;
+}
+
 
 #include <descrobject.h>
 #include <structmember.h>
@@ -544,6 +559,7 @@
     {"unpack", m_unpack, METH_VARARGS, "packed int32 pairs/offsets (host addresses) -> list of lists of (begin, end)"},
     {"pack_into", m_pack_into, METH_VARARGS, "list of lists of (begin, end) -> packed int32 buffers; returns K (ordered: begin <= end required)"},
     {"count", m_count, METH_O, "total number of intervals"},
+    {"path_is_simple", m_path_is_simple, METH_VARARGS, "packed int32 pairs/offsets (host addresses), B -> can the path be a path table"},
     {"tm_new", m_tm_new, METH_VARARGS, "event merger for n_files recordings of P symbols"},
     {"tm_add", m_tm_add, METH_VARARGS, "merge the packed events of one step (rows of 7 doubles at a host address)"},
     {"tm_finish", m_tm_finish, METH_VARARGS, "the final Note list of one recording"},
diff --git a/transkun_amd/csrc/torch_ops.cpp b/transkun_amd/csrc/torch_ops.cpp
--- a/transkun_amd/csrc/torch_ops.cpp
+++ b/transkun_amd/csrc/torch_ops.cpp
@@ -331,27 +331,29 @@
 }
 
 void logprob_fwd(Tensor score, Tensor noise, Tensor pairs, int64_t K, Tensor offsets, Tensor logProb, Tensor logZ, Tensor v, bool want_v,
-                 Tensor ws)
+                 Tensor ws, Tensor ptab, bool has_ptab)
 {
     Ctx c(score); c.same(score, noise, pairs, offsets, logProb, logZ, v, ws);
+    if (has_ptab) c.same(score, ptab);
     const Dims d = crf_dims(score, noise);
     STD_TORCH_CHECK(K >= 0, "semicrf: negative interval count");
-    check(semicrf_logprob_fwd(cfp(score), cfp(noise), d.T, d.B, i32(pairs, 2 * K, "pairs"), K, i32(offsets, d.B + 1, "offsets"),
-                              f32w(logProb, d.B, "logProb"), f32w(logZ, d.B, "logZ"), want_v ? f32w(v, (int64_t)d.T * d.B, "v") : nullptr,
-                              bytes(ws, "ws"), (size_t)ws.numel(), c.stream),
+    check(semicrf_logprob_fwd_t(cfp(score), cfp(noise), d.T, d.B, i32(pairs, 2 * K, "pairs"), K, i32(offsets, d.B + 1, "offsets"),
+                                f32w(logProb, d.B, "logProb"), f32w(logZ, d.B, "logZ"), want_v ? f32w(v, (int64_t)d.T * d.B, "v") : nullptr,
+                                has_ptab ? i32(ptab, (int64_t)d.T * d.B, "ptab") : nullptr, bytes(ws, "ws"), (size_t)ws.numel(), c.stream),
           "semicrf_logprob_fwd");
 }
 void logprob_bwd(Tensor score, Tensor noise, Tensor v, Tensor logZ, Tensor gout, int64_t gstride, Tensor pairs, int64_t K, Tensor offsets,
-                 Tensor dScore, Tensor dNoise, int64_t flags, Tensor ws)
+                 Tensor dScore, Tensor dNoise, int64_t flags, Tensor ws, Tensor ptab, bool has_ptab)
 {
     Ctx c(score); c.same(score, noise, v, logZ, gout, pairs, offsets, dScore, dNoise, ws);
+    if (has_ptab) c.same(score, ptab);
     const Dims d = crf_dims(score, noise);
     const int64_t TB = (int64_t)d.T * d.B;
     STD_TORCH_CHECK(K >= 0 && (gstride == 0 || gstride == 1), "semicrf: bad interval count / gout stride");
-    check(semicrf_logprob_bwd_f(cfp(score), cfp(noise), f32(v, TB, "v"), f32(logZ, d.B, "logZ"), f32(gout, gstride ? d.B : 1, "gout"),
+    check(semicrf_logprob_bwd_t(cfp(score), cfp(noise), f32(v, TB, "v"), f32(logZ, d.B, "logZ"), f32(gout, gstride ? d.B : 1, "gout"),
                                 (int)gstride, d.T, d.B, i32(pairs, 2 * K, "pairs"), K, i32(offsets, d.B + 1, "offsets"),
-                                f32w(dScore, TB * d.T, "dScore"), f32w(dNoise, TB - d.B, "dNoise"), (int)flags, bytes(ws, "ws"),
-                                (size_t)ws.numel(), c.stream),
+                                f32w(dScore, TB * d.T, "dScore"), f32w(dNoise, TB - d.B, "dNoise"), (int)flags,
+                                has_ptab ? i32(ptab, TB, "ptab") : nullptr, bytes(ws, "ws"), (size_t)ws.numel(), c.stream),
           "semicrf_logprob_bwd");
 }
 
@@ -578,8 +580,9 @@
 }
 
 void logprob_fwd_cpu(Tensor score, Tensor noise, Tensor pairs, int64_t K, Tensor offsets, Tensor logProb, Tensor logZ, Tensor v, bool want_v,
-                     Tensor ws)
-{
+                     Tensor ws, Tensor ptab, bool has_ptab)
+{
+    STD_TORCH_CHECK(!has_ptab, "semicrf: the path table belongs to the GPU sweeps");
     logz_fwd_cpu(score, noise, logZ, v, want_v, ws);
     eval_path_cpu(score, noise, pairs, K, offsets, logProb, ws);
     float* lp = (float*)logProb.data_ptr();
@@ -587,8 +590,9 @@
     for (int64_t c = 0; c < score.size(2); ++c) lp[c] -= lz[c];
 }
 void logprob_bwd_cpu(Tensor score, Tensor noise, Tensor v, Tensor logZ, Tensor gout, int64_t gstride, Tensor pairs, int64_t K, Tensor offsets,
-                     Tensor dScore, Tensor dNoise, int64_t flags, Tensor ws)
-{
+                     Tensor dScore, Tensor dNoise, int64_t flags, Tensor ws, Tensor ptab, bool has_ptab)
+{
+    STD_TORCH_CHECK(!has_ptab, "semicrf: the path table belongs to the GPU sweeps");
     all_cpu(score, noise, v, logZ, gout, pairs, offsets, dScore, dNoise);
     const Dims d = crf_dims(score, noise);
     const int64_t TB = (int64_t)d.T * d.B;
@@ -1141,9 +1145,9 @@
     m.def("eval_path_bwd(Tensor gout, int T, int B, Tensor pairs, int K, Tensor offsets, Tensor(a!) dScore, bool has_ds, Tensor(b!) dNoise, "
           "bool has_dn) -> ()");
     m.def("logprob_fwd(Tensor score, Tensor noise, Tensor pairs, int K, Tensor offsets, Tensor(a!) logProb, Tensor(b!) logZ, Tensor(c!) v, "
-          "bool want_v, Tensor(d!) ws) -> ()");
+          "bool want_v, Tensor(d!) ws, Tensor(e!) ptab, bool has_ptab) -> ()");
     m.def("logprob_bwd(Tensor score, Tensor noise, Tensor v, Tensor logZ, Tensor gout, int gstride, Tensor pairs, int K, Tensor offsets, "
-          "Tensor(a!) dScore, Tensor(b!) dNoise, int flags, Tensor(c!) ws) -> ()");
+          "Tensor(a!) dScore, Tensor(b!) dNoise, int flags, Tensor(c!) ws, Tensor ptab, bool has_ptab) -> ()");
     m.def("interval_score_fwd(Tensor q, Tensor k, Tensor diag, Tensor rowc, int C, int T, int D, int ldq, int ldk, int ldd, int ldrc, "
           "float qscale, int mode, int full, int group, int pitch, Tensor(a!) S, Tensor(b!) noise) -> ()");
     m.def("interval_score_bwd_ws(Tensor dS, Tensor q, Tensor k, int C, int T, int D, int ldq, int ldk, float qscale, int mode, int group, "
```

Measured after the change: 1951 steps/s (median of 6 runs). 1.02x the previous value.
